# CIawevy/FreeFine

Hardware: AMD Instinct MI355X
Metric: edited images/sec/GPU @512px 50-step DDIM (higher is better)
Workload: dtype bf16x3

## Files before the change

freefine_amd/_lib.py:

```python
import ctypes as C
import os

_HERE = os.path.dirname(os.path.abspath(__file__))
LIB_PATH = os.environ.get("FREEFINE_HIP_LIB") or os.path.join(_HERE, "libfreefine_hip.so")

FFN_F32, FFN_BF16, FFN_BF16X3, FFN_FP8 = 0, 1, 2, 3
IG_OUT_SILU, IG_OUT_F32, IG_GEGLU, IG_OUT_TRANSPOSED, IG_OUT_PAIR, IG_OUT_GELU, IG_OUT_RELU, IG_OUT_KV64 = 1, 2, 4, 8, 16, 32, 64, 128
IG_OUT_QGELU = 256
ELT_RELU, ELT_ADD, ELT_GELU = 0, 1, 2
ATT_MAXP, ATT_MAXB = 4, 16
ATT_HEAD_RULE, ATT_UNIFORM_SEL1, ATT_UNIFORM_SEL0, ATT_CAUSAL = 1, 2, 4, 8
NORM_SILU, NORM_OUT_PAIR = 1, 2
IMGPREP_MAX_SIDE = 4096
IMGPREP_MAX_TAPS = 2 * 3 * IMGPREP_MAX_SIDE + 1
BOX_NMS_MAX = 16384
KEEP_NONE, KEEP_SUM_LT128, KEEP_GT128 = 0, 1, 2
CHAIN_MAXL, CHAIN_MAXW = 8, 1024
CONV_RELU = 1
POOL_MAX, POOL_AVG_VALID = 0, 1


class IgemmDesc(C.Structure):
    _fields_ = [
        ("A", C.c_void_p), ("W", C.c_void_p), ("out", C.c_void_p),
        ("bias", C.c_void_p), ("rowbias", C.c_void_p), ("residual", C.c_void_p),
        ("M", C.c_int), ("N", C.c_int), ("K", C.c_int), ("Kpad", C.c_int),
        ("lda", C.c_int), ("ldo", C.c_int), ("ldr", C.c_int), ("ldrb", C.c_int),
        ("rows_per_batch", C.c_int),
        ("Hin", C.c_int), ("Win", C.c_int), ("Cin", C.c_int), ("Hout", C.c_int), ("Wout", C.c_int),
        ("stride", C.c_int), ("pad", C.c_int), ("upsample", C.c_int),
        ("flags", C.c_int), ("alpha", C.c_float), ("conv", C.c_int),
        ("splitk", C.c_int), ("ws", C.c_void_p), ("ws_bytes", C.c_long),
        ("a_lo", C.c_int), ("x3", C.c_int), ("f8", C.c_int), ("kv64_from", C.c_int),
    ]


class AttnEntry(C.Structure):
    _fields_ = [
        ("q_row", C.c_int), ("kv_row", C.c_int),
        ("w_const", C.c_float), ("w_slope", C.c_float),
        ("wq", C.c_void_p), ("kmask", C.c_void_p), ("qsel", C.c_void_p),
        ("flags", C.c_int), ("hr_row", C.c_int),
    ]


class AttnDesc(C.Structure):
    _fields_ = [
        ("q", C.c_void_p), ("k", C.c_void_p), ("vt", C.c_void_p), ("out", C.c_void_p), ("w_dev", C.c_void_p),
        ("Bo", C.c_int), ("S", C.c_int), ("Sk", C.c_int), ("heads", C.c_int), ("D", C.c_int),
        ("ldq", C.c_int), ("ldk", C.c_int), ("ldvt", C.c_int), ("ldo", C.c_int),
        ("scale", C.c_float), ("npass", C.c_int), ("out_pair", C.c_int), ("kv_pair", C.c_int),
        ("e", AttnEntry * (ATT_MAXP * ATT_MAXB)),
    ]


class CtrlStepDesc(C.Structure):
    _fields_ = [
        ("eps", C.c_void_p), ("x", C.c_void_p), ("noise", C.c_void_p), ("m", C.c_void_p), ("om", C.c_void_p),
        ("x_prev", C.c_void_p), ("pred_x0", C.c_void_p),
        ("c_bt", C.c_float), ("c_at", C.c_float), ("c_ap", C.c_float), ("c_dir", C.c_float),
        ("c_dirm", C.c_float * 8), ("stdv", C.c_float * 8), ("row_masked", C.c_int * 8),
        ("rows", C.c_int), ("CHW", C.c_int), ("HW", C.c_int),
    ]


class SplatXform(C.Structure):
    _fields_ = [("center", C.c_float * 3), ("translate", C.c_float * 3), ("rotate", C.c_float * 9), ("scale", C.c_float * 3),
                ("tan_half_fov", C.c_float)]


class PackDesc(C.Structure):
    _fields_ = [
        ("src", C.c_void_p), ("dst", C.c_void_p), ("src_row", C.c_int * 16),
        ("B", C.c_int), ("Cl", C.c_int), ("CP", C.c_int), ("HW", C.c_int),
    ]


class DiftDesc(C.Structure):
    _fields_ = [
        ("src", C.c_void_p), ("tgt", C.c_void_p), ("kps", C.c_void_p), ("ws", C.c_void_p), ("out_rc", C.c_void_p), ("out_cos", C.c_void_p),
        ("ws_bytes", C.c_long), ("es", C.c_long),
        ("dtype", C.c_int), ("E", C.c_int), ("C", C.c_int), ("ld", C.c_int), ("h", C.c_int), ("w", C.c_int), ("H", C.c_int), ("W", C.c_int), ("K", C.c_int),
    ]


class ResizePilDesc(C.Structure):
    _fields_ = [
        ("src", C.c_void_p), ("dst", C.c_void_p), ("scratch", C.c_void_p), ("m1", C.c_void_p), ("m2", C.c_void_p),
        ("hbounds", C.c_void_p), ("hcoef", C.c_void_p), ("vbounds", C.c_void_p), ("vcoef", C.c_void_p),
        ("B", C.c_int), ("H", C.c_int), ("W", C.c_int), ("C", C.c_int), ("oh", C.c_int), ("ow", C.c_int), ("hksize", C.c_int), ("vksize", C.c_int),
        ("y0", C.c_int), ("x0", C.c_int), ("ch", C.c_int), ("cw", C.c_int), ("rule", C.c_int),
    ]


class CoarseEditDesc(C.Structure):
    _fields_ = [
        ("src_img", C.c_void_p), ("src_mask", C.c_void_p), ("bg", C.c_void_p), ("hole_img", C.c_void_p), ("hole_mask", C.c_void_p), ("inv", C.c_void_p),
        ("final_img", C.c_void_p), ("tmask", C.c_void_p), ("trans_hole", C.c_void_p),
        ("B", C.c_int), ("H", C.c_int), ("W", C.c_int), ("mask_c", C.c_int), ("hole_mask_c", C.c_int),
    ]


class Conv2dDesc(C.Structure):
    _fields_ = [
        ("x", C.c_void_p), ("w", C.c_void_p), ("bias", C.c_void_p), ("out", C.c_void_p),
        ("B", C.c_int), ("Hin", C.c_int), ("Win", C.c_int), ("Cin", C.c_int), ("N", C.c_int),
        ("KH", C.c_int), ("KW", C.c_int), ("stride", C.c_int), ("pad_h", C.c_int), ("pad_w", C.c_int),
        ("ldx", C.c_int), ("ldo", C.c_int), ("Kpad", C.c_int), ("flags", C.c_int),
    ]


_vp, _i, _f, _l = C.c_void_p, C.c_int, C.c_float, C.c_long
SYMBOLS = {
    "ffn_version": (_i, []),
    "ffn_last_error": (C.c_char_p, []),
    "ffn_device_info": (_i, [_i, C.c_char_p, _i]),
    "ffn_graph_launch": (_i, [_vp, _vp]),
    "ffn_igemm": (_i, [_vp, _i, C.POINTER(IgemmDesc)]),
    "ffn_conv3x3_n4": (_i, [_vp, _i, _vp, _vp, _vp, _vp, _i, _i, _i, _i]),
    "ffn_split_pair": (_i, [_vp, _vp, _vp, _l, _i, _i]),
    "ffn_groupnorm_f8": (_i, [_vp, _vp, _vp, _vp, _vp, _i, _i, _i, _i, _i, _f, _i, _f, _vp, _vp, _vp]),
    "ffn_attn": (_i, [_vp, _i, C.POINTER(AttnDesc)]),
    "ffn_attn_kernel_name": (_i, [_i, C.POINTER(AttnDesc), C.c_char_p, _i]),
    "ffn_igemm_tune": (_i, [_vp, _i, C.POINTER(IgemmDesc)]),
    "ffn_igemm_tune_entry_ints": (_i, []),
    "ffn_igemm_tune_export": (_i, [C.POINTER(C.c_int), _i]),
    "ffn_igemm_tune_import": (_i, [C.POINTER(C.c_int), _i]),
    "ffn_igemm_tune_stamp": (_i, []),
    "ffn_igemm_tune_clear": (_i, []),
    "ffn_igemm_tune_enable": (_i, [_i]),
    "ffn_igemm_num_configs": (_i, []),
    "ffn_igemm_force_config": (_i, [_i]),
    "ffn_igemm_kernel_name": (_i, [_i, C.POINTER(IgemmDesc), C.c_char_p, _i]),
    "ffn_attn_presplit": (_i, [_vp, _vp, _vp, _vp, _vp, _i, _i, _i, _i, _i]),
    "ffn_attn_variant": (_i, [_i, _i, C.POINTER(C.c_int), C.POINTER(C.c_int)]),
    "ffn_gn_nchunk": (_i, [_i]),
    "ffn_gn_fused": (_i, [_i, _i, _i, _i]),
    "ffn_gn_stats": (_i, [_vp, _i, _vp, _vp, _vp, _i, _i, _i, _i, _f, _vp, _vp, _vp]),
    "ffn_gn_apply": (_i, [_vp, _i, _vp, _vp, _vp, _vp, _i, _i, _i, _i]),
    "ffn_groupnorm": (_i, [_vp, _i, _vp, _vp, _vp, _vp, _i, _i, _i, _i, _f, _i, _vp, _vp, _vp]),
    "ffn_groupnorm_pair_raw": (_i, [_vp, _vp, _vp, _vp, _vp, _vp, _i, _i, _i, _i, _f, _i, _vp, _vp, _vp]),
    "ffn_layernorm": (_i, [_vp, _i, _vp, _vp, _vp, _vp, _i, _i, _f]),
    "ffn_layernorm_pair": (_i, [_vp, _vp, _vp, _vp, _vp, _i, _i, _f]),
    "ffn_softmax_rows": (_i, [_vp, _i, _vp, _vp, _l, _i, _f]),
    "ffn_pool_layernorm": (_i, [_vp, _i, _vp, _vp, _vp, _vp, _vp, _i, _i, _i, _f, _i]),
    "ffn_cosine_rows": (_i, [_vp, _vp, _vp, _vp, _i, _i, _i]),
    "ffn_cfg_masked": (_i, [_vp, _vp, _vp, _vp, _f, _vp, _l, _i]),
    "ffn_ddim_inv_step": (_i, [_vp, _vp, _vp, _f, _f, _f, _f, _vp, _vp, _l]),
    "ffn_ddim_ctrl_step": (_i, [_vp, C.POINTER(CtrlStepDesc)]),
    "ffn_pack_nchw": (_i, [_vp, _i, C.POINTER(PackDesc)]),
    "ffn_nhwc_to_nchw_f32": (_i, [_vp, _vp, _vp, _i, _i, _i, _i]),
    "ffn_concat": (_i, [_vp, _i, _vp, _vp, _vp, _l, _i, _i]),
    "ffn_timestep_embed": (_i, [_vp, _i, _vp, _vp, _vp, _i, _i, _i]),
    "ffn_transpose": (_i, [_vp, _i, _vp, _vp, _i, _i, _i, _i, _i]),
    "ffn_cast": (_i, [_vp, _i, _i, _vp, _vp, _l]),
    "ffn_eltwise": (_i, [_vp, _i, _i, _vp, _vp, _vp, _l]),
    "ffn_resize_bilinear": (_i, [_vp, _i, _vp, _vp, _i, _i, _i, _i, _i, _i, _i]),
    "ffn_splat_lift": (_i, [_vp, _vp, _vp, _vp, _i, _i, _i, _f, _f]),
    "ffn_splat_project": (_i, [_vp, _vp, _vp, _i, C.POINTER(SplatXform)]),
    "ffn_splat_bin": (_i, [_vp, _i, _vp, _i, _f, _i, _i, _vp, _vp, _vp]),
    "ffn_splat_render": (_i, [_vp, _vp, _vp, _vp, _vp, _f, _i, _i, _i, _vp, _vp, _vp]),
    "ffn_splat_ids": (_i, [_vp, _vp, _vp, _vp, _f, _i, _i, _i, _vp]),
    "ffn_splat_correspond": (_i, [_vp, _vp, _vp, _i, _i, _i, _vp, _i, _vp, _vp]),
    "ffn_geo_project": (_i, [_vp, _vp, C.POINTER(C.c_float), _f, _i, _i, _vp, _vp]),
    "ffn_splat_composite": (_i, [_vp, _vp, _vp, _vp, _vp, _f, _f, _i, _i, _i, _i, _i, _vp]),
    "ffn_mesh_cover": (_i, [_vp, _vp, _vp, _i, _i, _vp]),
    "ffn_embed_tokens": (_i, [_vp, _i, _vp, _vp, _vp, _vp, _l, _i, _i, _i]),
    "ffn_embed_tokens_ln": (_i, [_vp, _i, _vp, _vp, _vp, _vp, _vp, _vp, _l, _i, _i, _i, _f]),
    "ffn_affine_chain": (_i, [_vp, _vp, _vp, _vp, _i, _i, C.POINTER(C.c_int), _i, _f, _f]),
    "ffn_dift_match": (_i, [_vp, C.POINTER(DiftDesc)]),
    "ffn_dift_workspace_bytes": (_l, [_i, _i, _i, _i]),
    "ffn_sift_base": (_i, [_vp, _vp, _vp, _i, _i, _i]),
    "ffn_gauss_blur_f32": (_i, [_vp, _vp, _vp, _vp, _i, _i, _vp, _i]),
    "ffn_decimate2_f32": (_i, [_vp, _vp, _vp, _i, _i]),
    "ffn_sift_extrema": (_i, [_vp, _vp, _vp, _i, _i, _vp, _i, _vp, C.POINTER(C.c_int)]),
    "ffn_sift_refine_orient": (_i, [_vp, _vp, _vp, _i, _i, _i, _vp, _i, _vp]),
    "ffn_sift_describe": (_i, [_vp, _vp, _i, _i, _i, _vp, _i, _vp, _vp]),
    "ffn_knn2_u8": (_i, [_vp, _vp, _i, _vp, _i, _vp, _vp]),
    "ffn_resize_pil_bilinear_u8": (_i, [_vp, _vp, _vp, _vp, _i, _i, _i, _i, _i, _vp, _vp, _i, _vp, _vp, _i]),
    "ffn_resize_pil_u8": (_i, [_vp, C.POINTER(ResizePilDesc)]),
    "ffn_resize_taps8_u8": (_i, [_vp, _vp, _vp, _i, _i, _i, _i, _i, _i, _vp, _vp, _vp, _vp]),
    "ffn_resize_gather_u8": (_i, [_vp, _vp, _vp, _i, _i, _i, _i, _i, _i, _vp, _vp, _i]),
    "ffn_dilate_u8": (_i, [_vp, _vp, _vp, _vp, _i, _i, _i, _i, _i]),
    "ffn_mask_bbox_u8": (_i, [_vp, _vp, _vp, _i, _i, _i, _i]),
    "ffn_coarse_edit_2d": (_i, [_vp, C.POINTER(CoarseEditDesc)]),
    "ffn_vit_patch_rows": (_i, [_vp, _i, _vp, _vp, _vp, _i, _i, _i, _i, _i]),
    "ffn_vit_patch_rows_pair": (_i, [_vp, _vp, _vp, _vp, _i, _i, _i, _i, _i]),
    "ffn_sam_patch_rows": (_i, [_vp, _i, _vp, _vp, _i, _i, _i, _i, _i, _i, C.POINTER(C.c_float), C.POINTER(C.c_float)]),
    "ffn_sam_patch_rows_pair": (_i, [_vp, _vp, _vp, _i, _i, _i, _i, _i, _i, C.POINTER(C.c_float), C.POINTER(C.c_float)]),
    "ffn_hyper_masks": (_i, [_vp, _vp, _vp, _vp, _i, _i, _i, _i]),
    "ffn_upsample_bicubic": (_i, [_vp, _vp, _vp, _vp, _i, _i, _i, _i, _i]),
    "ffn_upsample_bicubic_stats": (_i, [_vp, _vp, _vp, _vp, _i, _i, _i, _i, _i, _f]),
    "ffn_box_nms": (_i, [_vp, _vp, _vp, _i, _f]),
    "ffn_image_to_nhwc": (_i, [_vp, _i, _vp, _vp, _l, _i]),
    "ffn_nhwc_to_image": (_i, [_vp, _i, _vp, _vp, _i, _i, _i]),
    "ffn_conv2d": (_i, [_vp, _i, C.POINTER(Conv2dDesc)]),
    "ffn_pool2d": (_i, [_vp, _i, _vp, _vp, _i, _i, _i, _i, _i, _i, _i, _i, _i]),
    "ffn_mean_hw": (_i, [_vp, _vp, _vp, _i, _i, _i, _i]),
    "ffn_fid_prep": (_i, [_vp, _vp, _vp, _vp, _i, _i, _i]),
}

_lib = None


class FreeFineHipError(RuntimeError):
    pass


def load():
    global _lib
    if _lib is None:
        if not os.path.exists(LIB_PATH):
            raise FreeFineHipError(
                f"{LIB_PATH} not found: build it with `python -c 'import __graft_entry__ as g; g.build()'` "
                "(hipcc --offload-arch=gfx950). There is no CPU fallback for the product path.")
        import torch
        lib = C.CDLL(LIB_PATH)
        for name, (res, args) in SYMBOLS.items():
            fn = getattr(lib, name)
            fn.restype = res
            fn.argtypes = args
        _lib = lib
    return _lib

# ... 6 lines not shown
```

freefine_amd/csrc/capi.hip:

```cpp
#include <stdlib.h>
#include <string.h>

#include "capi_common.h"
#include "conv_small.h"
#include "elementwise.h"
#include "norms.h"

__thread char g_err[512] = "";

extern "C" int ffn_version(void) { return 16; }
extern "C" const char* ffn_last_error(void) { return g_err; }
extern "C" int ffn_device_info(int device, char* name, int name_len) {
    hipDeviceProp_t prop;
    hipError_t e = hipGetDeviceProperties(&prop, device);
    if (e != hipSuccess) return fail(FFN_EHIP, "hipGetDeviceProperties: %s", hipGetErrorString(e));
    if (name && name_len > 0) {
        strncpy(name, prop.gcnArchName, name_len - 1);
        name[name_len - 1] = 0;
    }
    return prop.multiProcessorCount;
}

extern "C" int ffn_graph_launch(void* stream, void* graph_exec) {
    REQUIRE(graph_exec, "graph_launch: null graph");
    hipError_t e = hipGraphLaunch(reinterpret_cast<hipGraphExec_t>(graph_exec), reinterpret_cast<hipStream_t>(stream));
    if (e != hipSuccess) return fail(FFN_EHIP, "hipGraphLaunch: %s", hipGetErrorString(e));
    return FFN_OK;
}

extern "C" int ffn_split_pair(void* stream, const float* src, void* dst, long rows, int C, int ld_src) {
    REQUIRE(src && dst && rows > 0 && C > 0 && C % 4 == 0 && ld_src >= C && ld_src % 4 == 0, "split_pair: bad arguments (C=%d, ld_src=%d)", C, ld_src);
    REQUIRE(aligned16(src) && aligned16(dst), "split_pair: pointers must be 16-byte aligned");
    if (C % 8 == 0) LAUNCH(split_pair8_kernel, dim3(grid_for(rows * (C / 8))), dim3(256), 0, reinterpret_cast<hipStream_t>(stream), src, (bf16*)dst, rows, C, ld_src);
    else LAUNCH(split_pair_kernel, dim3(grid_for(rows * (C / 4))), dim3(256), 0, reinterpret_cast<hipStream_t>(stream), src, (bf16*)dst, rows, C, ld_src);
    return check_launch("split_pair");
}
extern "C" int ffn_conv3x3_n4(void* stream, int dtype, const void* x, const float* w, const float* bias, float* out, int B, int H, int W, int Cin) {
    REQUIRE(dtype == FFN_F32 || dtype == FFN_BF16, "conv3x3_n4: fp32 or bf16 activations");
    REQUIRE(x && w && out && aligned16(x) && aligned16(w) && aligned16(out) && (!bias || aligned16(bias)), "conv3x3_n4: null / unaligned pointer");
    REQUIRE(B > 0 && H > 0 && W > 0 && Cin > 0 && Cin % 16 == 0 && Cin <= 448, "conv3x3_n4: B=%d H=%d W=%d Cin=%d (Cin %% 16 == 0, <= 448)", B, H, W, Cin);
    hipStream_t s = reinterpret_cast<hipStream_t>(stream);
    const long npix = (long)B * H * W;
    const int lds = 36 * Cin * 4;
    dim3 grid((unsigned)((npix + 63) / 64));
    int rc;
    if (dtype == FFN_F32) {
        if ((rc = set_lds(conv3x3_n4_kernel<float>, lds))) return rc;
        LAUNCH(conv3x3_n4_kernel<float>, grid, dim3(256), lds, s, (const float*)x, w, bias, out, B, H, W, Cin);
    } else {
        if ((rc = set_lds(conv3x3_n4_kernel<bf16>, lds))) return rc;
        LAUNCH(conv3x3_n4_kernel<bf16>, grid, dim3(256), lds, s, (const bf16*)x, w, bias, out, B, H, W, Cin);
    }
    return check_launch("conv3x3_n4");
}

extern "C" int ffn_eltwise(void* stream, int dtype, int op, const void* a, const void* b, void* y, long n) {
    REQUIRE(dtype == FFN_F32 || dtype == FFN_BF16, "eltwise: bad dtype %d", dtype);
    REQUIRE(op == FFN_ELT_RELU || op == FFN_ELT_ADD || op == FFN_ELT_GELU, "eltwise: bad op %d", op);
    REQUIRE(a && y && (op != FFN_ELT_ADD || b), "eltwise: null operand");
    REQUIRE(n > 0 && n % 4 == 0, "eltwise: n=%ld must be a positive multiple of 4", n);
    hipStream_t s = reinterpret_cast<hipStream_t>(stream);
    const long n4 = n / 4;
    const int grid = grid_for(n4);
    if (dtype == FFN_F32) {
        if (op == FFN_ELT_RELU) LAUNCH((eltwise_kernel<float, FFN_ELT_RELU>), dim3(grid), dim3(256), 0, s, (const float*)a, (const float*)b, (float*)y, n4);
        else if (op == FFN_ELT_GELU) LAUNCH((eltwise_kernel<float, FFN_ELT_GELU>), dim3(grid), dim3(256), 0, s, (const float*)a, (const float*)b, (float*)y, n4);
        else LAUNCH((eltwise_kernel<float, FFN_ELT_ADD>), dim3(grid), dim3(256), 0, s, (const float*)a, (const float*)b, (float*)y, n4);
    } else {
        if (op == FFN_ELT_RELU) LAUNCH((eltwise_kernel<bf16, FFN_ELT_RELU>), dim3(grid), dim3(256), 0, s, (const bf16*)a, (const bf16*)b, (bf16*)y, n4);
        else if (op == FFN_ELT_GELU) LAUNCH((eltwise_kernel<bf16, FFN_ELT_GELU>), dim3(grid), dim3(256), 0, s, (const bf16*)a, (const bf16*)b, (bf16*)y, n4);
        else LAUNCH((eltwise_kernel<bf16, FFN_ELT_ADD>), dim3(grid), dim3(256), 0, s, (const bf16*)a, (const bf16*)b, (bf16*)y, n4);
    }
    return check_launch("eltwise");
}
extern "C" int ffn_resize_bilinear(void* stream, int dtype, const void* x, void* y, int B, int Hin, int Win, int Hout, int Wout, int C, int relu) {
    REQUIRE(dtype == FFN_F32 || dtype == FFN_BF16, "resize_bilinear: bad dtype %d", dtype);
    REQUIRE(x && y, "resize_bilinear: null operand");
    REQUIRE(B > 0 && Hin > 0 && Win > 0 && Hout > 0 && Wout > 0 && C > 0 && C % 4 == 0, "resize_bilinear: bad shape (C=%d must be a multiple of 4)", C);
    REQUIRE((long)B * Hout * Wout * C < (1l << 40) && (long)Hin * Win < (1l << 31), "resize_bilinear: problem too large");
    hipStream_t s = reinterpret_cast<hipStream_t>(stream);
    const long n4 = (long)B * Hout * Wout * (C / 4);
    const int grid = grid_for(n4);
    if (dtype == FFN_F32) {
        if (relu) LAUNCH((resize_bilinear_kernel<float, true>), dim3(grid), dim3(256), 0, s, (const float*)x, (float*)y, n4, Hin, Win, Hout, Wout, C);
        else LAUNCH((resize_bilinear_kernel<float, false>), dim3(grid), dim3(256), 0, s, (const float*)x, (float*)y, n4, Hin, Win, Hout, Wout, C);
    } else {
        if (relu) LAUNCH((resize_bilinear_kernel<bf16, true>), dim3(grid), dim3(256), 0, s, (const bf16*)x, (bf16*)y, n4, Hin, Win, Hout, Wout, C);
        else LAUNCH((resize_bilinear_kernel<bf16, false>), dim3(grid), dim3(256), 0, s, (const bf16*)x, (bf16*)y, n4, Hin, Win, Hout, Wout, C);
    }
    return check_launch("resize_bilinear");
}

extern "C" int ffn_gn_nchunk(int HW) {
    int n = HW / 128;
    if (n < 1) n = 1;
    if (n > 256) n = 256;
    return n;
}
extern "C" int ffn_gn_fused(int B, int HW, int C, int G) {
    const long slice = (long)HW * (C / (G > 0 ? G : 1));
    if (slice > 131072) return 0;
    if (HW <= 64) return 1;
    if (HW <= 256) return B <= 32 ? 1 : 0;
    return (HW <= 1024 && (long)B * HW * C <= 3000000l) ? 1 : 0;
}
extern "C" int ffn_groupnorm(void* stream, int dtype, const void* x, void* y, const float* gamma, const float* beta, int B, int HW, int C,
                             int G, float eps, int silu, float* partial_ws, float* scale, float* shift) {
    REQUIRE(dtype == FFN_F32 || dtype == FFN_BF16, "groupnorm: bad dtype");
    REQUIRE(x && y && gamma && beta && C % G == 0 && (C / G) % 2 == 0, "groupnorm: bad arguments (C=%d, G=%d)", C, G);
    hipStream_t s = reinterpret_cast<hipStream_t>(stream);
    const bool fused = ffn_gn_fused(B, HW, C, G) != 0;
    const bool pair = silu & FFN_NORM_OUT_PAIR;
    REQUIRE(!pair || (dtype == FFN_F32 && C % 4 == 0), "groupnorm: pair output needs fp32 input and C %% 4 == 0");
    silu &= FFN_NORM_SILU;
    if (fused && pair) {
        dim3 grid(G, B);
        if (silu) LAUNCH((gn_fused_kernel<float, true, true>), grid, dim3(1024), 0, s, (const float*)x, (float*)y, gamma, beta, HW, C, G, eps);
        else LAUNCH((gn_fused_kernel<float, false, true>), grid, dim3(1024), 0, s, (const float*)x, (float*)y, gamma, beta, HW, C, G, eps);
        return check_launch("gn_fused(pair)");
    }
    if (fused) {
        dim3 grid(G, B);
        if (dtype == FFN_F32) {
            if (silu) LAUNCH((gn_fused_kernel<float, true>), grid, dim3(1024), 0, s, (const float*)x, (float*)y, gamma, beta, HW, C, G, eps);
            else LAUNCH((gn_fused_kernel<float, false>), grid, dim3(1024), 0, s, (const float*)x, (float*)y, gamma, beta, HW, C, G, eps);
        } else {
            if (silu) LAUNCH((gn_fused_kernel<bf16, true>), grid, dim3(1024), 0, s, (const bf16*)x, (bf16*)y, gamma, beta, HW, C, G, eps);
            else LAUNCH((gn_fused_kernel<bf16, false>), grid, dim3(1024), 0, s, (const bf16*)x, (bf16*)y, gamma, beta, HW, C, G, eps);
        }
        return check_launch("gn_fused");
    }
    REQUIRE(partial_ws && scale && shift, "groupnorm: workspace required beyond 32x32 positions");
    int rc = ffn_gn_stats(stream, dtype, x, gamma, beta, B, HW, C, G, eps, partial_ws, scale, shift);
    if (rc) return rc;
    return ffn_gn_apply(stream, dtype, x, y, scale, shift, B, HW, C, silu | (pair ? FFN_NORM_OUT_PAIR : 0));
}
extern "C" int ffn_groupnorm_pair_raw(void* stream, const void* x, void* y, void* yraw, const float* gamma, const float* beta, int B, int HW, int C, int G,
                                      float eps, int silu, float* partial_ws, float* scale, float* shift) {
    REQUIRE(x && y && yraw && gamma && beta && partial_ws && scale && shift, "groupnorm_pair_raw: null pointer (the workspace is always needed)");
    REQUIRE(C % 8 == 0 && C % G == 0 && (C / G) % 2 == 0 && aligned16(x) && aligned16(y) && aligned16(yraw), "groupnorm_pair_raw: bad arguments (C=%d, G=%d)", C, G);
    REQUIRE(y != yraw && yraw != x && y != x, "groupnorm_pair_raw: x, y and yraw must be distinct buffers");
    int rc = ffn_gn_stats(stream, FFN_F32, x, gamma, beta, B, HW, C, G, eps, partial_ws, scale, shift);
    if (rc) return rc;
    hipStream_t s = reinterpret_cast<hipStream_t>(stream);
    const long n8 = (long)B * HW * (C / 8);
    if (silu & FFN_NORM_SILU) LAUNCH((gn_apply_pair8_kernel<true, true>), dim3(grid_for(n8)), dim3(256), 0, s, (const float*)x, (bf16*)y, scale, shift, n8, HW, C, (bf16*)yraw);
    else LAUNCH((gn_apply_pair8_kernel<false, true>), dim3(grid_for(n8)), dim3(256), 0, s, (const float*)x, (bf16*)y, scale, shift, n8, HW, C, (bf16*)yraw);
    return check_launch("gn_apply(pair + raw pair)");
}
extern "C" int ffn_groupnorm_f8(void* stream, const void* x, void* y, const float* gamma, const float* beta, int B, int HW, int C, int Cp, int G,
                                float eps, int silu, float qscale, float* partial_ws, float* scale, float* shift) {
    REQUIRE(x && y && gamma && beta && partial_ws && scale && shift, "groupnorm_f8: null pointer (the workspace is always needed)");
    REQUIRE(C % 16 == 0 && C % G == 0 && Cp >= C && Cp % 16 == 0 && aligned16(x) && aligned16(y) && qscale > 0.f, "groupnorm_f8: bad arguments (C=%d, Cp=%d)", C, Cp);
    int rc = ffn_gn_stats(stream, FFN_BF16, x, gamma, beta, B, HW, C, G, eps, partial_ws, scale, shift);
    if (rc) return rc;
    hipStream_t s = reinterpret_cast<hipStream_t>(stream);
    const long nch = (long)B * HW * (Cp / 16);
    if (silu & FFN_NORM_SILU) LAUNCH(gn_apply_f8_kernel<true>, dim3(grid_for(nch)), dim3(256), 0, s, (const bf16*)x, (uint8_t*)y, scale, shift, nch, HW, C, Cp, qscale);
    else LAUNCH(gn_apply_f8_kernel<false>, dim3(grid_for(nch)), dim3(256), 0, s, (const bf16*)x, (uint8_t*)y, scale, shift, nch, HW, C, Cp, qscale);
    return check_launch("gn_apply_f8");
}
extern "C" int ffn_gn_stats(void* stream, int dtype, const void* x, const float* gamma, const float* beta, int B, int HW, int C,
                            int G, float eps, float* partial_ws, float* scale, float* shift) {
    REQUIRE(dtype == FFN_F32 || dtype == FFN_BF16, "gn_stats: bad dtype");
    const int epc = dtype == FFN_F32 ? 4 : 8;
    REQUIRE(x && gamma && beta && partial_ws && scale && shift, "gn_stats: null pointer");
    REQUIRE(C % epc == 0 && C % G == 0 && aligned16(x), "gn_stats: C=%d must be a multiple of %d and of G=%d", C, epc, G);
    hipStream_t s = reinterpret_cast<hipStream_t>(stream);
    const int nchunk = ffn_gn_nchunk(HW);
    const int ppc = (HW + nchunk - 1) / nchunk;
    const int cols_ = C / epc < 256 ? C / epc : 256;
    const int lds = (256 / cols_ > 0 ? 256 / cols_ : 1) * cols_ * 2 * epc * (int)sizeof(float);
    if (dtype == FFN_F32)
        LAUNCH(gn_partial_kernel<float>, dim3(nchunk, B), dim3(256), lds, s, (const float*)x, partial_ws, HW, C, ppc);
    else
        LAUNCH(gn_partial_kernel<bf16>, dim3(nchunk, B), dim3(256), lds, s, (const bf16*)x, partial_ws, HW, C, ppc);
    if (int rc = check_launch("gn_partial")) return rc;
    LAUNCH(gn_finalize_kernel, dim3(G, B), dim3(64), 0, s, partial_ws, gamma, beta, scale, shift, HW, C, G, nchunk, ppc, eps);
    return check_launch("gn_stats");
}
extern "C" int ffn_gn_apply(void* stream, int dtype, const void* x, void* y, const float* scale, const float* shift, int B, int HW,
                            int C, int silu) {
    REQUIRE(dtype == FFN_F32 || dtype == FFN_BF16, "gn_apply: bad dtype");
    const int epc = dtype == FFN_F32 ? 4 : 8;
    REQUIRE(x && y && scale && shift && C % epc == 0 && aligned16(x) && aligned16(y), "gn_apply: bad arguments");
    hipStream_t s = reinterpret_cast<hipStream_t>(stream);
    const long nch = (long)B * HW * (C / epc);
    const int grid = grid_for(nch);
    if (silu & FFN_NORM_OUT_PAIR) {
        REQUIRE(dtype == FFN_F32, "gn_apply: pair output needs fp32 input");
        if (C % 8 == 0) {
            const long n8 = (long)B * HW * (C / 8);
            if (silu & FFN_NORM_SILU) LAUNCH(gn_apply_pair8_kernel<true>, dim3(grid_for(n8)), dim3(256), 0, s, (const float*)x, (bf16*)y, scale, shift, n8, HW, C);
            else LAUNCH(gn_apply_pair8_kernel<false>, dim3(grid_for(n8)), dim3(256), 0, s, (const float*)x, (bf16*)y, scale, shift, n8, HW, C);
            return check_launch("gn_apply(pair, 8 wide)");
        }
        if (silu & FFN_NORM_SILU) LAUNCH((gn_apply_kernel<float, true, true>), dim3(grid), dim3(256), 0, s, (const float*)x, (float*)y, scale, shift, nch, HW, C);
        else LAUNCH((gn_apply_kernel<float, false, true>), dim3(grid), dim3(256), 0, s, (const float*)x, (float*)y, scale, shift, nch, HW, C);
        return check_launch("gn_apply(pair)");
    }
    if (dtype == FFN_F32) {
        if (silu) LAUNCH((gn_apply_kernel<float, true>), dim3(grid), dim3(256), 0, s, (const float*)x, (float*)y, scale, shift, nch, HW, C);
        else LAUNCH((gn_apply_kernel<float, false>), dim3(grid), dim3(256), 0, s, (const float*)x, (float*)y, scale, shift, nch, HW, C);
    } else {
        if (silu) LAUNCH((gn_apply_kernel<bf16, true>), dim3(grid), dim3(256), 0, s, (const bf16*)x, (bf16*)y, scale, shift, nch, HW, C);
        else LAUNCH((gn_apply_kernel<bf16, false>), dim3(grid), dim3(256), 0, s, (const bf16*)x, (bf16*)y, scale, shift, nch, HW, C);
    }
    return check_launch("gn_apply");
}
extern "C" int ffn_layernorm(void* stream, int dtype, const void* x, void* y, const float* gamma, const float* beta, int M, int C,
                             float eps) {
    REQUIRE(dtype == FFN_F32 || dtype == FFN_BF16, "layernorm: bad dtype");
    const int epc = dtype == FFN_F32 ? 4 : 8;
    REQUIRE(x && y && gamma && beta && C % epc == 0 && aligned16(x) && aligned16(y), "layernorm: bad arguments");
    const int cch = C / epc;
    REQUIRE(cch <= 64 * 6, "layernorm: C=%d too large", C);
    hipStream_t s = reinterpret_cast<hipStream_t>(stream);
    const int grid = (M + 3) / 4;
    if (dtype == FFN_F32) {
        if (cch <= 128) LAUNCH((layernorm_kernel<float, 2>), dim3(grid), dim3(256), 0, s, (const float*)x, (float*)y, gamma, beta, M, C, eps);
        else LAUNCH((layernorm_kernel<float, 6>), dim3(grid), dim3(256), 0, s, (const float*)x, (float*)y, gamma, beta, M, C, eps);
    } else {
        if (cch <= 128) LAUNCH((layernorm_kernel<bf16, 2>), dim3(grid), dim3(256), 0, s, (const bf16*)x, (bf16*)y, gamma, beta, M, C, eps);
        else LAUNCH((layernorm_kernel<bf16, 6>), dim3(grid), dim3(256), 0, s, (const bf16*)x, (bf16*)y, gamma, beta, M, C, eps);
    }
    return check_launch("layernorm");
}
extern "C" int ffn_layernorm_pair(void* stream, const float* x, void* y, const float* gamma, const float* beta, int M, int C, float eps) {
    REQUIRE(x && y && gamma && beta && C % 4 == 0 && aligned16(x) && aligned16(y), "layernorm_pair: bad arguments");
    const int cch = C / 4;
    REQUIRE(cch <= 64 * 6, "layernorm_pair: C=%d too large", C);
    hipStream_t s = reinterpret_cast<hipStream_t>(stream);
    const int grid = (M + 3) / 4;
    if (cch <= 128) LAUNCH((layernorm_kernel<float, 2, true>), dim3(grid), dim3(256), 0, s, x, (float*)y, gamma, beta, M, C, eps);
    else LAUNCH((layernorm_kernel<float, 6, true>), dim3(grid), dim3(256), 0, s, x, (float*)y, gamma, beta, M, C, eps);
    return check_launch("layernorm(pair)");
}
extern "C" int ffn_softmax_rows(void* stream, int dtype, const void* x, void* y, long M, int N, float scale) {
    REQUIRE(dtype == FFN_F32 || dtype == FFN_BF16, "softmax_rows: bad dtype");
    REQUIRE(x && y && M > 0 && N > 0, "softmax_rows: bad arguments");
    hipStream_t s = reinterpret_cast<hipStream_t>(stream);
    if (dtype == FFN_F32) LAUNCH(softmax_rows_kernel<float>, dim3((unsigned)M), dim3(256), 0, s, (const float*)x, (float*)y, N, scale);
    else LAUNCH(softmax_rows_kernel<bf16>, dim3((unsigned)M), dim3(256), 0, s, (const bf16*)x, (bf16*)y, N, scale);
    return check_launch("softmax_rows");
}

extern "C" int ffn_cfg_masked(void* stream, const float* eps_u, const float* eps_c, const float* mask, float cfg, float* eps, long n,
                              int HW) {
    REQUIRE(eps_u && eps_c && eps && n > 0 && HW > 0, "cfg_masked: bad arguments");
    LAUNCH(cfg_masked_kernel, dim3(grid_for(n)), dim3(256), 0, reinterpret_cast<hipStream_t>(stream), eps_u, eps_c, mask, cfg, eps, n, HW);
    return check_launch("cfg_masked");
}
extern "C" int ffn_ddim_inv_step(void* stream, const float* eps, const float* x, float c_bt, float c_at, float c_an, float c_bn,
                                 float* x_next, float* pred_x0, long n) {
    REQUIRE(eps && x && x_next && n > 0, "ddim_inv_step: bad arguments");
    LAUNCH(ddim_inv_step_kernel, dim3(grid_for(n)), dim3(256), 0, reinterpret_cast<hipStream_t>(stream), eps, x, c_bt, c_at, c_an, c_bn, x_next, pred_x0, n);
    return check_launch("ddim_inv_step");
}
extern "C" int ffn_ddim_ctrl_step(void* stream, const ffn_ctrl_step_desc* d) {
    REQUIRE(d && d->eps && d->x && d->x_prev && d->m && d->om, "ddim_ctrl_step: null pointer");
    REQUIRE(d->rows > 0 && d->rows <= 8 && d->CHW > 0 && d->HW > 0 && d->CHW % d->HW == 0, "ddim_ctrl_step: bad shape");
    LAUNCH(ddim_ctrl_step_kernel, dim3(grid_for((long)d->rows * d->CHW)), dim3(256), 0, reinterpret_cast<hipStream_t>(stream), *d);
// ... 75 lines not shown
```

freefine_amd/csrc/capi_igemm.hip:

```cpp
#include <math.h>
#include <stdlib.h>
#include <string.h>
#include <initializer_list>

#include "capi_common.h"
#include "igemm.h"
#include "igemm_p8.h"

static bool can_split(const ffn_igemm_desc& d) {
    return d.ws && d.splitk != 1 && !(d.flags & (FFN_IG_GEGLU | FFN_IG_OUT_TRANSPOSED | FFN_IG_OUT_KV64));
}
static void igemm_rule_for(int dtype, const ffn_igemm_desc& d, int* bm, int* bn, int* splitk) {
    const long t128 = (long)((d.M + 127) / 128) * ((d.N + 127) / 128);
    const long t12864 = (long)((d.M + 127) / 128) * ((d.N + 63) / 64);
    *splitk = 1;
    if (!d.conv && !(d.flags & FFN_IG_GEGLU) && d.M >= 128 && (!can_split(d) || t12864 >= 128)) {
        *bm = 128; *bn = 64;
    } else if (d.N > 64 && (t128 >= 256 || (can_split(d) && d.M > 512 && d.N >= 128))) {
        *bm = 128; *bn = 128;
    } else if (t12864 >= 256 || d.M >= 4096 || (can_split(d) && d.M >= 96 && d.N >= 64)) {
        *bm = 128; *bn = 64;
    } else { *bm = 64; *bn = 64; }
    if (can_split(d)) {
        const int kstage = dtype == FFN_F32 ? 32 : 64;
        const int nk = (d.K + kstage - 1) / kstage;
        const long tiles = (long)((d.M + *bm - 1) / *bm) * ((d.N + *bn - 1) / *bn);
        int s = d.splitk > 1 ? d.splitk : (tiles >= 224 ? 1 : (int)((448 + tiles - 1) / tiles));
        if (d.splitk <= 1 && s > nk / 6) s = nk / 6;
        const long per = (long)d.M * d.N * 4;
        if ((long)s * per > d.ws_bytes) s = (int)(d.ws_bytes / per);
        if (s > nk) s = nk;
        if (s < 1) s = 1;
        *splitk = s;
    }
}

enum { CFG_64x64, CFG_128x64, CFG_128x128_8, CFG_128x128_16, CFG_256x128, CFG_256x256, CFG_128x320, CFG_128x160, CFG_192x320, CFG_H_128x320, CFG_H_256x128, CFG_H_256x256, CFG_H_128x128, CFG_PP_256x320, CFG_PP_256x256, CFG_PP_192x320, CFG_PP_192x256, CFG_PP_256x128, CFG_COUNT };
struct IgCfgInfo { int bm, bn, nwm, nwn; };
static const IgCfgInfo kCfg[CFG_COUNT] = {{64, 64, 2, 2}, {128, 64, 4, 2}, {128, 128, 2, 4}, {128, 128, 4, 4},
                                          {256, 128, 4, 4}, {256, 256, 4, 4}, {128, 320, 4, 4}, {128, 160, 4, 2}, {192, 320, 3, 4},
                                          {128, 320, 4, 4}, {256, 128, 4, 4}, {256, 256, 4, 4}, {128, 128, 4, 4},
                                          {256, 320, 2, 4}, {256, 256, 2, 4}, {192, 320, 2, 4}, {192, 256, 2, 4},
                                          {256, 128, 2, 4}};
struct IgChoice { int cfg, splitk; };
struct TunedEntry { IgChoice ch; bool validated; };

static bool is_halo_cfg(int cfg) { return cfg == CFG_H_128x320 || cfg == CFG_H_256x128 || cfg == CFG_H_256x256 || cfg == CFG_H_128x128; }
static bool is_pp_cfg(int cfg) { return cfg >= CFG_PP_256x320 && cfg <= CFG_PP_256x128; }
static bool pp_ok(const ffn_igemm_desc& d, int bm, int bn, int splitk = 1) {
    const long lim = (1l << 31) - 4096;
    const int nkt = d.x3 ? d.K / 96 : d.K / 64;
    if (bn == 128 && (bm != 256 || !d.x3 || d.conv != 1 || splitk > 1 || d.N % 256 == 0 || d.N % 320 == 0 || (d.flags & (FFN_IG_GEGLU | FFN_IG_OUT_PAIR | FFN_IG_OUT_KV64 | FFN_IG_OUT_TRANSPOSED)))) return false;
    if (d.x3) {
        if (d.x3 != 2 || d.K % 96 != 0 || d.a_lo != 32) return false;
    } else if (d.K % 64 != 0) return false;
    if (nkt < 2 || d.N % bn != 0 || d.M < bm) return false;
    const int osz = d.x3 ? 4 : 2;
    if (splitk > 1) {
        if (!can_split(d) || nkt % splitk != 0 || nkt / splitk < 2 || (long)splitk * d.M * d.N * 4 > d.ws_bytes || (long)splitk * d.M * d.N * 4 >= lim) return false;
    } else {
        const int act_ok = (!d.residual && !d.x3 && !d.f8 && !(d.flags & FFN_IG_GEGLU)) ? (FFN_IG_OUT_GELU | FFN_IG_OUT_RELU) : 0;
        if ((d.alpha != 1.0f && !d.f8) || (d.flags & ~(FFN_IG_GEGLU | act_ok | (d.x3 ? (FFN_IG_OUT_F32 | FFN_IG_OUT_PAIR | FFN_IG_OUT_KV64) : 0)))) return false;
        if (d.f8 && (!d.conv || (d.flags & FFN_IG_GEGLU))) return false;
        if (d.x3 && (d.flags & FFN_IG_GEGLU) && !(d.flags & FFN_IG_OUT_PAIR)) return false;
        if ((d.flags & FFN_IG_OUT_PAIR) && !(d.flags & FFN_IG_GEGLU) && (d.N % 32 != 0 || (d.ldo / 2) % 32 != 0 || (d.flags & FFN_IG_OUT_TRANSPOSED))) return false;
        if ((d.flags & FFN_IG_GEGLU) && bn != 256) return false;
        if (d.rowbias && d.rows_per_batch < 128) return false;
    }
    long a_bytes;
    if (d.conv) {
        const int pix = d.x3 ? d.lda : d.Cin;
        const int cpt = d.x3 ? d.Cin / 32 : d.Cin / 64;
        if (d.Cin % (d.x3 ? 32 : 64) != 0 || d.K != (d.conv == 2 ? 4 : 9) * (d.x3 ? 3 : 1) * d.Cin) return false;
        if (d.x3 && d.lda != 2 * d.Cin) return false;
        if (d.conv == 2 && (d.f8 || d.stride != 1 || d.upsample)) return false;
        if ((long)cpt * 9 * cpt >= 65536) return false;
        a_bytes = (long)(d.M / (d.Hout * d.Wout)) * d.Hin * d.Win * pix * 2;
        if (2 * d.Hin + 2 >= 32768 || 2 * d.Win + 2 >= 32768) return false;
        if (a_bytes + 256l * pix * 2 >= lim) return false;
    } else {
        a_bytes = (long)d.M * d.lda * 2;
        if (a_bytes + 256l * d.lda * 2 >= lim) return false;
    }
    if ((long)d.N * d.Kpad * 2 >= lim || (long)(d.M + 256) * d.ldo * ((d.flags & FFN_IG_OUT_PAIR) ? 2 : osz) >= lim) return false;
    if (d.residual && (long)(d.M + 256) * d.ldr * osz >= lim) return false;
    return true;
}
static int halo_bytes_for(const ffn_igemm_desc& d, int bm) {
    if (!d.conv || d.stride != 1 || d.upsample || d.pad != 1 || d.Hin != d.Hout || d.Win != d.Wout) return 0;
    if (d.Cin % 64 != 0 || d.Cin > 30000 || d.K != 9 * d.Cin || d.M % bm != 0) return 0;
    const int H = d.Hin, W = d.Win;
    int tw, tr;
    if (W <= bm) {
        if (bm % W != 0 || (H * W) % bm != 0) return 0;
        tw = W; tr = bm / W;
    } else {
        if (W % bm != 0) return 0;
        tw = bm; tr = 1;
    }
    const int nq = ((tr + 2) * (tw + 2) + 7) / 8;
    if (nq > 4 * 16) return 0;
    return nq * 8 * 128;
}
static bool x3_cfg(int cfg) { return cfg == CFG_64x64 || cfg == CFG_128x64 || cfg == CFG_128x128_8 || is_pp_cfg(cfg); }
static ffn_igemm_desc x3_view(const ffn_igemm_desc& d) {
    ffn_igemm_desc v = d;
    v.x3 = d.x3 == 2 ? 2 : 1;
    v.f8 = 0;
    v.K = 3 * d.K;
    v.flags |= FFN_IG_OUT_F32;
    return v;
}
static ffn_igemm_desc f8_view(const ffn_igemm_desc& d) {
    ffn_igemm_desc v = d;
    v.f8 = 1;
    v.x3 = 0;
    v.K = d.K / 2;
    v.Cin = d.Cin / 2;
    v.Kpad = d.Kpad / 2;
    v.lda = d.lda / 2;
    return v;
}
static ffn_igemm_desc igemm_view(int dtype, const ffn_igemm_desc& d) {
    if (dtype == FFN_BF16X3) return x3_view(d);
    if (dtype == FFN_FP8) return f8_view(d);
    ffn_igemm_desc v = d;
    v.x3 = v.f8 = 0;
    return v;
}
static int pp_tile_height(const ffn_igemm_desc& d, int bn, std::initializer_list<int> heights, int min_fill4, bool trans = false) {
    long best = -1;
    int bh = 0;
    for (int h : heights) {
        if (trans ? d.M < h : !pp_ok(d, h, bn)) continue;
        const long tiles = (long)((d.M + h - 1) / h) * (d.N / bn);
        if (tiles * 4 < (long)device_cus() * min_fill4) continue;
        const long cost = ((tiles + device_cus() - 1) / device_cus()) * h;
        if (best < 0 || cost < best) { best = cost; bh = h; }
    }
    return bh;
}
static int pp_cfg(int bm, int bn) {
    for (int cfg = CFG_PP_256x320; cfg <= CFG_PP_256x128; ++cfg)
        if (kCfg[cfg].bm == bm && kCfg[cfg].bn == bn) return cfg;
    return -1;
}
static bool conv2_tile(const ffn_igemm_desc& d, int* bm, int* bn) {
    for (int n : {320, 256})
        for (int h : {256, 192})
            if (pp_tile_height(d, n, {h}, 0)) { *bm = h; *bn = n; return true; }
    return false;
}
static bool pp_trans_tile(const ffn_igemm_desc& d, int* bm, int* bn) {
    const long lim = (1l << 31) - 4096;
    *bn = d.N % 320 == 0 ? 320 : (d.N % 256 == 0 ? 256 : 0);
    if (!*bn || d.alpha != 1.0f || d.rows_per_batch % 16 != 0 || d.M % 4 != 0) return false;
    if (d.x3) {
        if (d.x3 != 2 || d.K % 96 != 0 || d.K < 192 || d.a_lo != 32) return false;
    } else if (d.K % 64 != 0 || d.K < 128) return false;
    if ((long)(d.M + 256) * d.lda * 2 >= lim || (long)d.N * d.Kpad * 2 >= lim) return false;
    if ((long)((d.M + d.rows_per_batch - 1) / d.rows_per_batch) * d.N * d.ldo * (d.x3 ? 4 : 2) >= lim) return false;
    return (*bm = pp_tile_height(d, *bn, {256, 192}, 0, true)) != 0;
}
static IgChoice rule_choice(int dtype, const ffn_igemm_desc& d) {
    int bm, bn, sk;
    igemm_rule_for(dtype, d, &bm, &bn, &sk);
    const int kstage = dtype == FFN_F32 ? 32 : 64;
    const int nk = ((d.K + kstage - 1) / kstage + sk - 1) / sk;
    int cfg = CFG_64x64;
    if (bm == 128 && bn == 64) cfg = CFG_128x64;
    if (bm == 128 && bn == 128) cfg = (!d.conv && nk <= 24 && !d.x3 && !d.f8) ? CFG_128x128_16 : CFG_128x128_8;
    return IgChoice{cfg, sk};
}
static IgChoice heuristic_choice(const ffn_igemm_desc& d) {
    int bm, bn;
    if (d.conv == 2 && conv2_tile(d, &bm, &bn)) return IgChoice{pp_cfg(bm, bn), 1};
    if (d.splitk <= 1) {
        for (int n : {320, 256})
            if ((bm = pp_tile_height(d, n, {256, 192}, 3))) return IgChoice{pp_cfg(bm, n), 1};
        if (pp_tile_height(d, 128, {256}, 3)) return IgChoice{CFG_PP_256x128, 1};
    }
    return rule_choice(FFN_BF16, d);
}

struct TuneKey {
    int M, N, K, conv, Cin, Hin, Win, stride, upsample, flags, lda, splitk, ptrs, wslabs, rpb, alpha1, ldo, pad, Hout, Wout, Kpad, ldr, dtype;
    bool operator==(const TuneKey& o) const { return memcmp(this, &o, sizeof(TuneKey)) == 0; }
};
struct TuneKeyHash {
    size_t operator()(const TuneKey& k) const {
        const int* p = reinterpret_cast<const int*>(&k);
        size_t h = 1469598103934665603ull;
        for (size_t i = 0; i < sizeof(TuneKey) / sizeof(int); ++i) h = (h ^ (size_t)(unsigned)p[i]) * 1099511628211ull;
        return h;
    }
};
static TuneKey tune_key(const ffn_igemm_desc& d) {
    TuneKey k;
    memset(&k, 0, sizeof(k));
    k.M = d.M; k.N = d.N; k.K = d.K; k.conv = d.conv; k.flags = d.flags; k.lda = d.lda; k.splitk = d.splitk;
    if (d.conv) { k.Cin = d.Cin; k.Hin = d.Hin; k.Win = d.Win; k.stride = d.stride; k.upsample = d.upsample; k.pad = d.pad; k.Hout = d.Hout; k.Wout = d.Wout; }
    k.Kpad = d.Kpad;
    k.ldr = d.residual ? d.ldr : 0;
    k.dtype = d.x3 ? (FFN_BF16X3 | (d.x3 << 8)) : (d.f8 ? FFN_FP8 : FFN_BF16);
    k.ptrs = (d.bias ? 1 : 0) | (d.rowbias ? 2 : 0) | (d.residual ? 4 : 0) | (d.ws && d.ws_bytes > 0 ? 8 : 0);
    const long per = (long)d.M * d.N * 4;
    k.wslabs = d.ws ? (int)(d.ws_bytes / per > 1024 ? 1024 : d.ws_bytes / per) : 0;
    k.rpb = d.rows_per_batch;
    k.alpha1 = d.alpha == 1.0f;
    k.ldo = d.ldo;
    return k;
}
static std::mutex g_tune_mu;
static std::unordered_map<TuneKey, TunedEntry, TuneKeyHash> g_tuned;
static int g_tune_runtime = 1;
static bool tune_enabled() {
    static const bool on = [] { const char* e = getenv("FFN_IGEMM_TUNE"); return !(e && atoi(e) == 0); }();
    return on && g_tune_runtime;
}
static constexpr int kPpSplitBelow = 160;
static int candidates_for(const ffn_igemm_desc& d, IgChoice* out, int cap) {
    int n = 0;
    const IgChoice h = heuristic_choice(d);
    out[n++] = h;
    const int nk = (d.K + 63) / 64;
    const long per = (long)d.M * d.N * 4;
    for (int cfg = 0; cfg < CFG_COUNT; ++cfg) {
        const IgCfgInfo& c = kCfg[cfg];
        if ((d.x3 || d.f8) && !x3_cfg(cfg)) continue;
        if (d.conv == 2 && !is_pp_cfg(cfg)) continue;
        if ((cfg == CFG_128x320 || cfg == CFG_128x160 || cfg == CFG_192x320) && (d.flags & FFN_IG_GEGLU)) continue;
        if (is_halo_cfg(cfg)) {
            const int hb = halo_bytes_for(d, c.bm);
            if (hb <= 0 || d.splitk > 1 || 2 * hb + 2 * c.bn * 128 > 160 * 1024) continue;
            if ((cfg == CFG_H_128x320) && (d.flags & FFN_IG_GEGLU)) continue;
        }
        const bool halo = is_halo_cfg(cfg) || is_pp_cfg(cfg);
        if (is_pp_cfg(cfg)) {
            const long pt = (long)((d.M + c.bm - 1) / c.bm) * (d.N / (c.bn > 0 ? c.bn : 1));
            if (d.splitk <= 1 && pp_ok(d, c.bm, c.bn) && n < cap) out[n++] = IgChoice{cfg, 1};
            if (cfg != CFG_PP_256x128 && d.splitk != 1 && pt > 0 && pt < kPpSplitBelow && d.N % c.bn == 0) {
                const int nkt = d.x3 ? d.K / 96 : d.K / 64;
                int added = 0;
                for (int sgo = (int)((384 + pt - 1) / pt); sgo >= 2 && added < 2; --sgo) {
                    if (d.splitk > 1 && sgo != d.splitk) continue;
                    if (nkt % sgo != 0 || nkt / sgo < 2 || !pp_ok(d, c.bm, c.bn, sgo)) continue;
                    if (n < cap) out[n++] = IgChoice{cfg, sgo};
                    ++added;
                }
            }
            continue;
        }
        if (c.bm > 64 && c.bm >= 2 * d.M) continue;
        if (c.bn > 64 && c.bn >= 2 * d.N) continue;
        if (cfg == CFG_64x64 && (long)d.M * d.N > (1l << 22)) continue;
        const long tiles = (long)((d.M + c.bm - 1) / c.bm) * ((d.N + c.bn - 1) / c.bn);
        int splits[3] = {1, 0, 0};
        if (d.splitk > 1) {
            int sf = (can_split(d) && !halo) ? d.splitk : 1;
            if ((long)sf * per > d.ws_bytes) sf = (int)(d.ws_bytes / per);
            if (sf > nk) sf = nk;
            splits[0] = sf >= 2 ? sf : 1;
        } else if (can_split(d) && !halo) {
            for (int t = 0; t < 2; ++t) {
                int sgo = (int)(((t ? 512 : 256) + tiles / 2) / tiles);
                if (sgo > nk / 4) sgo = nk / 4;
                if ((long)sgo * per > d.ws_bytes) sgo = (int)(d.ws_bytes / per);
                if (sgo >= 2) splits[1 + t] = sgo;
            }
            if (splits[2] == splits[1]) splits[2] = 0;
        }
        for (int t = 0; t < 3 && n < cap; ++t) {
            if (!splits[t]) continue;
            bool dup = false;
            for (int j = 0; j < n; ++j) dup |= out[j].cfg == cfg && out[j].splitk == splits[t];
            if (!dup) out[n++] = IgChoice{cfg, splits[t]};
        }
    }
    return n;
}
static int g_force_cfg = -1;
extern "C" int ffn_igemm_num_configs(void) { return CFG_COUNT; }
extern "C" int ffn_igemm_force_config(int cfg) {
    const int prev = g_force_cfg;
    g_force_cfg = (cfg >= 0 && cfg < CFG_COUNT) ? cfg : -1;
    return prev;
}
static bool known_choice(const ffn_igemm_desc& d, IgChoice* ch) {
    IgChoice cand[40];
    if (g_force_cfg >= 0) {
        *ch = heuristic_choice(d);
        for (int i = candidates_for(d, cand, 40) - 1; i >= 0; --i)
            if (cand[i].cfg == g_force_cfg) *ch = cand[i];
        return true;
    }
    std::lock_guard<std::mutex> lk(g_tune_mu);
    auto it = g_tuned.find(tune_key(d));
    if (it == g_tuned.end()) return false;
    if (!it->second.validated) {
        const int nc = candidates_for(d, cand, 40);
        bool ok = false;
        for (int i = 0; i < nc; ++i) ok |= cand[i].cfg == it->second.ch.cfg && cand[i].splitk == it->second.ch.splitk;
        if (!ok) return g_tuned.erase(it), false;
        it->second.validated = true;
    }
    *ch = it->second.ch;
    return true;
}

enum IgKind { IG_RING, IG_HALO, IG_PP, IG_PP_TRANS };
struct IgemmPlan {
    IgKind kind;
    bool f32;
    int bm, bn, amode, nwm, nwn;
    bool swap, fastk, x3, f8;
    bool res, geglu, split;
    int splitk, halo_bytes, lds;
    bool reduce_f32;
    dim3 grid, block;
};
static int igemm_plan(int dtype, const ffn_igemm_desc& d, const IgChoice* ch, IgemmPlan* p) {
    *p = IgemmPlan{};
    p->f32 = dtype == FFN_F32;
    p->x3 = d.x3 != 0;
    p->f8 = d.f8 != 0;
    p->amode = d.conv ? AMODE_CONV3 : AMODE_DENSE;
    p->swap = !(d.flags & FFN_IG_OUT_TRANSPOSED);
    p->reduce_f32 = p->f32 || p->x3;
    p->splitk = 1;
    p->block = dim3(512);
    const bool tuned = ch != nullptr;
    IgChoice rule;
    if (!tuned && !p->f32 && pp_trans_tile(d, &p->bm, &p->bn)) {
        p->kind = IG_PP_TRANS;
    } else {
        if (!tuned) ch = &(rule = rule_choice(p->f32 ? FFN_F32 : FFN_BF16, d));
        REQUIRE(ch->cfg >= 0 && ch->cfg < CFG_COUNT, "igemm: bad configuration %d", ch->cfg);
        REQUIRE(!(p->x3 || p->f8) || x3_cfg(ch->cfg), "igemm: configuration %d is not built for split-bf16 / fp8 problems", ch->cfg);
        const IgCfgInfo& c = kCfg[ch->cfg];
        p->kind = is_halo_cfg(ch->cfg) ? IG_HALO : (is_pp_cfg(ch->cfg) ? IG_PP : IG_RING);
        p->bm = c.bm; p->bn = c.bn; p->nwm = c.nwm; p->nwn = c.nwn;
        p->splitk = ch->splitk;
        p->block = dim3(64 * c.nwm * c.nwn);
        if (!tuned && p->x3) p->nwm = p->nwn = 2, p->block = dim3(256);
    }
    const int ntm = (d.M + p->bm - 1) / p->bm, ntn = (d.N + p->bn - 1) / p->bn;
    switch (p->kind) {
    case IG_RING: {
        p->fastk = tuned && !p->x3 && !p->f8 && (d.conv ? d.Cin % 64 == 0 : d.K % 64 == 0) && (long)d.K * 2 + 256 <= (long)sizeof(g_zero_page);
        p->lds = 2 * (p->bm + p->bn) * 128;
        int gx = ntm * ntn;
        if (tuned || p->x3) {
            int per_cu = (160 * 1024) / p->lds;
            if (per_cu > 2048 / (int)p->block.x) per_cu = 2048 / (int)p->block.x;
            const int cap = (device_cus() * per_cu) / p->splitk;
            if (gx > cap && cap >= 8) gx = cap;
        }
        p->grid = dim3(gx, p->splitk);
        break;
    }
    case IG_HALO:
        p->halo_bytes = halo_bytes_for(d, p->bm);
        REQUIRE(p->halo_bytes > 0 && p->splitk == 1 && !p->x3 && !p->f8, "igemm: halo kernel not applicable");
        p->lds = 2 * p->halo_bytes + 2 * p->bn * 128;
        p->grid = dim3((d.M / p->bm) * ntn);
        break;
    case IG_PP:
        REQUIRE(pp_ok(d, p->bm, p->bn, p->splitk), "igemm: ping-pong kernel not applicable");
        p->split = p->splitk > 1;
        p->res = !p->split && d.residual;
        p->geglu = !p->split && !d.conv && (d.flags & FFN_IG_GEGLU);
        [[fallthrough]];
    case IG_PP_TRANS: {
        p->lds = 2 * (p->bm + p->bn) * 128 + 12288;
        const int nt = ntm * (d.N / p->bn) * p->splitk;
        p->grid = dim3(nt < device_cus() ? nt : device_cus());
        break;
    }
    }
    return FFN_OK;
}
template <typename K, typename... A>
static int igemm_launch(const IgemmPlan& p, K kern, hipStream_t s, A... args) {
    static const char* const what[] = {"igemm", "igemm(halo)", "igemm(ping-pong)", "igemm(ping-pong, transposed)"};
    if (int rc = set_lds(kern, p.lds)) return rc;
    LAUNCH(kern, p.grid, p.block, p.lds, s, args...);
    return check_launch(what[p.kind]);
}
template <typename T, int AMODE, bool SWAP, bool FASTK = false, bool X3 = false, bool F8 = false>
static int launch_ring(const IgemmPlan& p, hipStream_t s, const ffn_igemm_desc& d) {
#define FFN_RING(BM_, BN_, WM_, WN_) \
    if (p.bm == BM_ && p.bn == BN_ && p.nwm == WM_ && p.nwn == WN_) return igemm_launch(p, igemm_glds_kernel<T, BM_, BN_, AMODE, SWAP, 2, WM_, WN_, FASTK, X3, F8>, s, d)
    if constexpr (X3 && !SWAP) {
        FFN_RING(64, 64, 2, 2);
        FFN_RING(128, 64, 2, 2);
        FFN_RING(128, 128, 2, 2);
    } else {
        FFN_RING(64, 64, 2, 2);
        FFN_RING(128, 64, 4, 2);
        FFN_RING(128, 128, 2, 4);
        if constexpr (!X3 && !F8) FFN_RING(128, 128, 4, 4);
        if constexpr (sizeof(T) == 2 && SWAP && !X3 && !F8) {
            FFN_RING(256, 128, 4, 4);
            FFN_RING(256, 256, 4, 4);
            FFN_RING(128, 320, 4, 4);
            FFN_RING(128, 160, 4, 2);
            FFN_RING(192, 320, 3, 4);
        }
    }
#undef FFN_RING
    return fail(FFN_EINVAL, "igemm: no %d x %d tile on %d x %d waves for this problem", p.bm, p.bn, p.nwm, p.nwn);
}
template <int AMODE, bool X3 = false, bool F8 = false>
static int launch_pp(const IgemmPlan& p, hipStream_t s, const ffn_igemm_desc& d) {
    const bool trans = p.kind == IG_PP_TRANS;
#define FFN_PP(BM_, BN_, RES_, GEGLU_, SPLIT_, TRANS_)                                                                       \
    if (p.bm == BM_ && p.bn == BN_ && p.res == RES_ && p.geglu == GEGLU_ && p.split == SPLIT_ && trans == TRANS_) \
        return igemm_launch(p, igemm_pp_kernel<BM_, BN_, AMODE, RES_, GEGLU_, SPLIT_, TRANS_, X3, F8>, s, d, p.splitk)
#define FFN_PP_TILE(BM_, BN_)                                                                   \
    FFN_PP(BM_, BN_, false, false, false, false);                                               \
    FFN_PP(BM_, BN_, true, false, false, false);                                                \
    FFN_PP(BM_, BN_, false, false, true, false);                                                \
    if constexpr (AMODE == AMODE_DENSE && !F8) {                                                \
        FFN_PP(BM_, BN_, false, false, false, true);                                            \
        if constexpr (BN_ == 256) FFN_PP(BM_, BN_, false, true, false, false);                  \
    }
    FFN_PP_TILE(256, 320)
    FFN_PP_TILE(256, 256)
    FFN_PP_TILE(192, 320)
    FFN_PP_TILE(192, 256)
    if constexpr (X3 && AMODE == AMODE_CONV3) {
        FFN_PP(256, 128, false, false, false, false);
        FFN_PP(256, 128, true, false, false, false);
    }
#undef FFN_PP_TILE
#undef FFN_PP
    return fail(FFN_EINVAL, "igemm: no %d x %d ping-pong tile of this form", p.bm, p.bn);
}
static int igemm_run(hipStream_t s, int dtype, const ffn_igemm_desc& d, const IgChoice* ch) {
    IgemmPlan p;
    int rc = igemm_plan(dtype, d, ch, &p);
    if (rc) return rc;
    const bool conv = p.amode == AMODE_CONV3;
    switch (p.kind) {
    case IG_RING:
        if (p.f32) rc = conv ? launch_ring<float, AMODE_CONV3, true>(p, s, d) : (p.swap ? launch_ring<float, AMODE_DENSE, true>(p, s, d) : launch_ring<float, AMODE_DENSE, false>(p, s, d));
        else if (!p.swap) rc = p.x3 ? launch_ring<bf16, AMODE_DENSE, false, false, true>(p, s, d) : launch_ring<bf16, AMODE_DENSE, false>(p, s, d);
        else if (p.x3) rc = conv ? launch_ring<bf16, AMODE_CONV3, true, false, true>(p, s, d) : launch_ring<bf16, AMODE_DENSE, true, false, true>(p, s, d);
        else if (p.f8) rc = launch_ring<bf16, AMODE_CONV3, true, false, false, true>(p, s, d);
        else if (p.fastk) rc = conv ? launch_ring<bf16, AMODE_CONV3, true, true>(p, s, d) : launch_ring<bf16, AMODE_DENSE, true, true>(p, s, d);
        else rc = conv ? launch_ring<bf16, AMODE_CONV3, true>(p, s, d) : launch_ring<bf16, AMODE_DENSE, true>(p, s, d);
        break;
    case IG_HALO:
#define FFN_HALO(BM_, BN_) \
    if (p.bm == BM_ && p.bn == BN_) rc = igemm_launch(p, igemm_halo_kernel<bf16, BM_, BN_, 4, 4>, s, d, p.halo_bytes)
        FFN_HALO(128, 320);
        FFN_HALO(256, 128);
        FFN_HALO(256, 256);
        FFN_HALO(128, 128);
#undef FFN_HALO
        break;
    case IG_PP:
    case IG_PP_TRANS:
        if (p.x3) rc = conv ? launch_pp<AMODE_CONV3, true>(p, s, d) : launch_pp<AMODE_DENSE, true>(p, s, d);
        else if (p.f8) rc = launch_pp<AMODE_CONV3, false, true>(p, s, d);
        else rc = conv ? launch_pp<AMODE_CONV3>(p, s, d) : launch_pp<AMODE_DENSE>(p, s, d);
        break;
    }
    if (rc || p.splitk == 1) return rc;
    const dim3 grid(grid_for((long)d.M * (d.N / 4)));
    if (p.reduce_f32) LAUNCH(igemm_splitk_reduce_kernel<float>, grid, dim3(256), 0, s, d, p.splitk);
    else LAUNCH(igemm_splitk_reduce_kernel<bf16>, grid, dim3(256), 0, s, d, p.splitk);
    return check_launch("igemm_splitk_reduce");
}
static int igemm_tune_now(hipStream_t s, int dtype, const ffn_igemm_desc& d) {
    std::lock_guard<std::mutex> lk(g_tune_mu);
    IgChoice cand[40];
    const int nc = candidates_for(d, cand, 40);
    hipEvent_t e0, e1;
    if (hipEventCreate(&e0) != hipSuccess || hipEventCreate(&e1) != hipSuccess) return igemm_run(s, dtype, d, &cand[0]);
    IgChoice best = cand[0];
    float best_ms = 1e30f;
    const int reps = 3;
    for (int i = 0; i < nc; ++i) {
        int rc = igemm_run(s, dtype, d, &cand[i]);
        if (rc) continue;
        float ms = 1e30f;
        for (int round = 0; round < 2 && !rc; ++round) {
            (void)hipEventRecord(e0, s);
            for (int r = 0; r < reps && !rc; ++r) rc = igemm_run(s, dtype, d, &cand[i]);
            (void)hipEventRecord(e1, s);
            if (rc || hipEventSynchronize(e1) != hipSuccess) { rc = rc ? rc : FFN_EHIP; break; }
            float t = 0.f;
            (void)hipEventElapsedTime(&t, e0, e1);
            if (t < ms) ms = t;
        }
        if (rc) continue;
        if (ms < best_ms) { best_ms = ms; best = cand[i]; }
// ... 30 lines not shown
        if (buf && n < max_entries) {
            int* e = buf + (long)n * kTuneEntryInts;
            e[0] = kTuneStamp;
            memcpy(e + 1, &kv.first, sizeof(TuneKey));
            e[kTuneEntryInts - 2] = kv.second.ch.cfg;
            e[kTuneEntryInts - 1] = kv.second.ch.splitk;
        }
        ++n;
    }
    return n;
}
extern "C" int ffn_igemm_tune_import(const int* buf, int n_entries) {
    REQUIRE(buf || n_entries == 0, "igemm_tune_import: null buffer");
    std::lock_guard<std::mutex> lk(g_tune_mu);
    int n = 0;
    for (int i = 0; i < n_entries; ++i) {
        const int* e = buf + (long)i * kTuneEntryInts;
        if (e[0] != kTuneStamp) continue;
        TuneKey k;
        memcpy(&k, e + 1, sizeof(TuneKey));
        const IgChoice ch{e[kTuneEntryInts - 2], e[kTuneEntryInts - 1]};
        if (ch.cfg < 0 || ch.cfg >= CFG_COUNT || ch.splitk < 1) continue;
        g_tuned[k] = TunedEntry{ch, false};
        ++n;
    }
    return n;
}
static int igemm_validate(int dtype, const ffn_igemm_desc& d) {
    REQUIRE(dtype == FFN_F32 || dtype == FFN_BF16 || dtype == FFN_BF16X3 || dtype == FFN_FP8, "igemm: bad dtype %d", dtype);
    if (dtype == FFN_FP8) {
        REQUIRE(d.conv && d.Cin > 0 && d.Cin % 16 == 0 && d.K == 9 * d.Cin && d.Kpad >= d.K && d.Kpad % 16 == 0 && d.lda == d.Cin,
                "igemm(fp8): 3x3 convolutions with Cin %% 16 == 0 only (Cin=%d, K=%d, Kpad=%d, lda=%d)", d.Cin, d.K, d.Kpad, d.lda);
        REQUIRE(d.M > 0 && d.N > 0 && d.N % 4 == 0 && d.ldo % 4 == 0 && d.rows_per_batch > 0 && d.M % (d.Hout * d.Wout) == 0, "igemm(fp8): bad shape");
        REQUIRE(!(d.flags & (FFN_IG_GEGLU | FFN_IG_OUT_TRANSPOSED | FFN_IG_OUT_PAIR | FFN_IG_OUT_F32)), "igemm(fp8): plain / SiLU / residual epilogues only");
        REQUIRE(d.stride == 1 || d.stride == 2, "igemm(fp8): stride %d", d.stride);
        int ex = 0;
        REQUIRE(d.alpha > 0.f && frexpf(d.alpha, &ex) == 0.5f, "igemm(fp8): alpha must be a power of two (the un-scaling of two power-of-two operand scales)");
        if (d.residual) REQUIRE(d.ldr % 4 == 0 && d.ldr >= d.N, "igemm(fp8): ldr=%d must be a multiple of 4 and >= N=%d", d.ldr, d.N);
        REQUIRE(d.ldo >= d.N, "igemm(fp8): ldo=%d must be >= N=%d", d.ldo, d.N);
        return FFN_OK;
    }
    const int epc = dtype == FFN_F32 ? 4 : 8;
    const int kmul = dtype == FFN_BF16X3 ? (d.x3 == 2 ? 2 : 3) : 1;
    REQUIRE(d.M > 0 && d.N > 0 && d.K > 0, "igemm: empty problem M=%d N=%d K=%d", d.M, d.N, d.K);
    REQUIRE(d.Kpad >= kmul * d.K && d.Kpad % epc == 0, "igemm: Kpad=%d (row stride of W) must be >= %d x K=%d and a multiple of %d", d.Kpad, kmul, d.K, epc);
    if (dtype == FFN_BF16X3) {
        const int plane = d.conv ? d.Cin : d.K;
        if (d.x3 == 2) {
            REQUIRE(plane % 32 == 0 && d.a_lo == 32 && d.lda >= 2 * plane, "igemm: blocked split-bf16 operands need K (conv: Cin) %% 32 == 0, a_lo = 32, lda >= 2 x that (%d, a_lo=%d, lda=%d)", plane, d.a_lo, d.lda);
        } else {
            REQUIRE(d.a_lo % 8 == 0 && d.a_lo >= plane && d.a_lo + plane <= d.lda, "igemm: split-bf16 A needs planes of %d elements: a_lo=%d, lda=%d", plane, d.a_lo, d.lda);
        }
        REQUIRE(d.lda % 8 == 0, "igemm: lda=%d must be a multiple of 8", d.lda);
        REQUIRE(d.alpha == 1.0f, "igemm: split-bf16 problems take alpha = 1");
    }
    REQUIRE(d.K % epc == 0, "igemm: K=%d must be a multiple of %d", d.K, epc);
    REQUIRE(d.rows_per_batch > 0, "igemm: rows_per_batch must be > 0");
    if (d.conv) {
        REQUIRE(d.Cin % epc == 0, "igemm: Cin=%d must be a multiple of %d", d.Cin, epc);
        if (d.conv == 2) {
            REQUIRE((dtype == FFN_BF16 || dtype == FFN_BF16X3) && d.K == 4 * d.Cin && d.stride == 1 && d.upsample == 0 && d.pad >= 0 && d.pad <= 3 && d.splitk <= 1,
                    "igemm: 2x2 convolution needs FFN_BF16 / FFN_BF16X3, K = 4*Cin, stride 1, no upsample, pad in 0..3, no forced split");
            int bm, bn;
            REQUIRE(conv2_tile(igemm_view(dtype, d), &bm, &bn), "igemm: 2x2 convolution M=%d N=%d Cin=%d fits no ping-pong tile (Cin %% 64 (split-bf16: 32), N %% 256 / 320, M >= 192)", d.M, d.N, d.Cin);
        } else {
            REQUIRE(d.conv == 1, "igemm: conv=%d", d.conv);
            REQUIRE(d.K == 9 * d.Cin, "igemm: conv K=%d != 9*Cin=%d", d.K, 9 * d.Cin);
        }
        REQUIRE(d.stride == 1 || d.stride == 2, "igemm: stride %d", d.stride);
        REQUIRE(d.upsample == 0 || d.upsample == 1, "igemm: upsample %d", d.upsample);
        REQUIRE(d.M % (d.Hout * d.Wout) == 0, "igemm: M=%d not a multiple of Hout*Wout", d.M);
    } else {
        REQUIRE(d.lda % epc == 0, "igemm: lda=%d must be a multiple of %d", d.lda, epc);
    }
    if (d.flags & FFN_IG_OUT_KV64) {
        REQUIRE(dtype == FFN_BF16X3 && !d.conv && !d.residual && !d.rowbias && d.splitk <= 1 &&
                    !(d.flags & (FFN_IG_GEGLU | FFN_IG_OUT_PAIR | FFN_IG_OUT_SILU | FFN_IG_OUT_GELU | FFN_IG_OUT_RELU | FFN_IG_OUT_QGELU)),
                "igemm: FFN_IG_OUT_KV64 needs FFN_BF16X3, dense A, the plain epilogue and no forced split-K");
        if (d.flags & FFN_IG_OUT_TRANSPOSED) REQUIRE(d.rows_per_batch % 64 == 0 && d.M % d.rows_per_batch == 0 && d.ldo >= d.rows_per_batch && d.ldo % 64 == 0,
                                                     "igemm: KV64 transposed output needs rows_per_batch %% 64 == 0, whole batches, ldo %% 64 == 0 (rows_per_batch=%d, ldo=%d)", d.rows_per_batch, d.ldo);
        else REQUIRE(d.kv64_from >= 0 && d.kv64_from < d.N && d.kv64_from % 64 == 0 && d.N % 64 == 0 && d.ldo % 4 == 0,
                     "igemm: KV64 output needs kv64_from and N %% 64 == 0 (kv64_from=%d, N=%d)", d.kv64_from, d.N);
    }
    if (d.flags & FFN_IG_OUT_TRANSPOSED) {
        REQUIRE(!d.conv, "igemm: transposed output is only supported for dense A");
        REQUIRE(d.ldo % 4 == 0, "igemm: transposed ldo=%d must be a multiple of 4", d.ldo);
        REQUIRE(!(d.flags & (FFN_IG_GEGLU | FFN_IG_OUT_F32 | FFN_IG_OUT_SILU | FFN_IG_OUT_GELU | FFN_IG_OUT_RELU | FFN_IG_OUT_QGELU)) && !d.residual && !d.rowbias,
                "igemm: transposed output supports bias only");
    } else {
        REQUIRE(d.N % 4 == 0 && d.ldo % 4 == 0, "igemm: N=%d and ldo=%d must be multiples of 4", d.N, d.ldo);
        if (d.residual) REQUIRE(d.ldr % 4 == 0, "igemm: ldr=%d must be a multiple of 4", d.ldr);
        if (d.flags & FFN_IG_OUT_PAIR) {
            const int nout = (d.flags & FFN_IG_GEGLU) ? d.N / 2 : d.N;
            REQUIRE(dtype == FFN_BF16X3 && d.ldo % 16 == 0 && d.ldo / 2 >= nout, "igemm: pair output needs FFN_BF16X3, ldo %% 16 == 0, ldo/2 >= columns");
            REQUIRE(d.residual != d.out, "igemm: pair output cannot overwrite its fp32 residual");
            REQUIRE((d.ldo / 2) % 32 != 0 || nout % 32 == 0 || nout == d.ldo / 2, "igemm: blocked pair output (ldo/2 %% 32 == 0) needs whole 32-column blocks");
            REQUIRE(nout == d.ldo / 2 || (d.ldo / 2) % 32 == 0, "igemm: pair output into a wider row needs ldo/2 %% 32 == 0 (ldo=%d, columns=%d)", d.ldo, nout);
        }
        if (d.flags & FFN_IG_GEGLU) {
            REQUIRE(d.N % 64 == 0, "igemm: GEGLU needs N %% 64 == 0 (N=%d)", d.N);
            REQUIRE(!d.residual && !d.rowbias && !(d.flags & (FFN_IG_OUT_F32 | FFN_IG_OUT_SILU | FFN_IG_OUT_GELU | FFN_IG_OUT_RELU | FFN_IG_OUT_QGELU)), "igemm: GEGLU epilogue is exclusive");
        }
    }
    const int act = d.flags & (FFN_IG_OUT_SILU | FFN_IG_OUT_GELU | FFN_IG_OUT_RELU | FFN_IG_OUT_QGELU);
    REQUIRE((act & (act - 1)) == 0, "igemm: SILU / GELU / QGELU / RELU are mutually exclusive");
    REQUIRE(d.splitk >= 0, "igemm: splitk must be >= 0");
    if (!d.conv && dtype != FFN_BF16X3) REQUIRE(d.lda >= d.K, "igemm: lda=%d must be >= K=%d", d.lda, d.K);
    if (d.flags & FFN_IG_OUT_TRANSPOSED) {
        const int cols = d.rows_per_batch < d.M ? d.rows_per_batch : d.M;
        REQUIRE(d.ldo >= cols, "igemm: transposed ldo=%d must be >= the %d rows of a batch", d.ldo, cols);
    } else if (!(d.flags & FFN_IG_OUT_PAIR)) {
        const int nout = (d.flags & FFN_IG_GEGLU) ? d.N / 2 : d.N;
        REQUIRE(d.ldo >= nout, "igemm: ldo=%d must be >= the %d output columns", d.ldo, nout);
    }
    if (d.residual) REQUIRE(d.ldr >= d.N, "igemm: ldr=%d must be >= N=%d", d.ldr, d.N);
    return FFN_OK;
}
static bool tuned_family(int dtype, const ffn_igemm_desc& d) { return dtype != FFN_F32 && !(d.flags & FFN_IG_OUT_TRANSPOSED); }
extern "C" int ffn_igemm_kernel_name(int dtype, const ffn_igemm_desc* d0, char* buf, int len) {
    REQUIRE(d0 && buf && len > 0, "igemm_kernel_name: null argument");
    if (int rc = igemm_validate(dtype, *d0)) return rc;
    const ffn_igemm_desc d = igemm_view(dtype, *d0);
    const bool tuned = tuned_family(dtype, d);
    IgChoice ch;
    if (tuned && !known_choice(d, &ch)) ch = heuristic_choice(d);
    IgemmPlan p;
    if (int rc = igemm_plan(dtype, d, tuned ? &ch : nullptr, &p)) return rc;
    auto b = [](bool v) { return v ? "true" : "false"; };
    switch (p.kind) {
    case IG_RING:
        snprintf(buf, len, "void igemm_glds_kernel<%s, %d, %d, %d, %s, 2, %d, %d, %s, %s, %s>(ffn_igemm_desc)", p.f32 ? "float" : "bf16", p.bm, p.bn, p.amode,
                 b(p.swap), p.nwm, p.nwn, b(p.fastk), b(p.x3), b(p.f8));
        break;
    case IG_HALO: snprintf(buf, len, "void igemm_halo_kernel<bf16, %d, %d, %d, %d>(ffn_igemm_desc, int)", p.bm, p.bn, p.nwm, p.nwn); break;
    case IG_PP:
    case IG_PP_TRANS:
        snprintf(buf, len, "void igemm_pp_kernel<%d, %d, %d, %s, %s, %s, %s, %s, %s>(ffn_igemm_desc, int)", p.bm, p.bn, p.amode, b(p.res), b(p.geglu), b(p.split),
                 b(p.kind == IG_PP_TRANS), b(p.x3), b(p.f8));
        break;
    }
    return FFN_OK;
}
extern "C" int ffn_igemm(void* stream, int dtype, const ffn_igemm_desc* d0) {
    REQUIRE(d0, "igemm: null descriptor");
    if (int rc = igemm_validate(dtype, *d0)) return rc;
    if (dtype == FFN_FP8) {
        REQUIRE(d0->A && d0->W && d0->out && aligned16(d0->A) && aligned16(d0->W) && aligned16(d0->out), "igemm(fp8): A/W/out must be non-null and 16-byte aligned");
    } else {
        REQUIRE(d0->A && d0->W && d0->out, "igemm: null A/W/out");
        REQUIRE(aligned16(d0->A) && aligned16(d0->W) && aligned16(d0->out), "igemm: A/W/out must be 16-byte aligned");
    }
    if ((dtype == FFN_BF16X3 || dtype == FFN_F32) && d0->residual) REQUIRE(aligned16(d0->residual), "igemm: fp32 residual must be 16-byte aligned");
    if ((dtype == FFN_BF16 || dtype == FFN_FP8) && d0->residual)
        REQUIRE((reinterpret_cast<uintptr_t>(d0->residual) & 7) == 0, "igemm%s: bf16 residual must be 8-byte aligned", dtype == FFN_FP8 ? "(fp8)" : "");
    if (d0->ws) REQUIRE(aligned16(d0->ws) && d0->ws_bytes >= 0, "igemm%s: workspace must be 16-byte aligned", dtype == FFN_FP8 ? "(fp8)" : "");
    hipStream_t s = reinterpret_cast<hipStream_t>(stream);
    const ffn_igemm_desc d = igemm_view(dtype, *d0);
    if (!tuned_family(dtype, d)) return igemm_run(s, dtype, d, nullptr);
    IgChoice ch;
    if (!known_choice(d, &ch)) {
        hipStreamCaptureStatus cap = hipStreamCaptureStatusNone;
        (void)hipStreamIsCapturing(s, &cap);
        if (tune_enabled() && cap == hipStreamCaptureStatusNone && d.residual != d.out) return igemm_tune_now(s, dtype, d);
        ch = heuristic_choice(d);
    }
    return igemm_run(s, dtype, d, &ch);
}

extern "C" int ffn_igemm_tune(void* stream, int dtype, const ffn_igemm_desc* d) { return ffn_igemm(stream, dtype, d); }
```

freefine_amd/csrc/igemm_p8.h:

```cpp
#pragma once
#include <type_traits>
#include "igemm.h"

#ifndef PP_ABL
#define PP_ABL 0
#endif
#ifdef PP_STAMP
__device__ unsigned long long pp_stamp_out[8 * 64];
#define PP_STAMP_AT(k_) do { if (blockIdx.x == 7 && s >= 24 && s < 28) { const unsigned long long t_ = __builtin_amdgcn_s_memtime(); \
    if (lane == 0) *reinterpret_cast<unsigned long long*>(smem + CV + 12288 + (wave * 64 + (s - 24) * 16 + (k_)) * 8) = t_; } } while (0)
#else
#define PP_STAMP_AT(k_) do {} while (0)
#endif
#define X3_NBE(FN_, NA_) ((FN_) + 2 - ((FN_) + (NA_) + 1) / 2)
template <int N>
__device__ __forceinline__ void pp_wait_vmcnt() {
    if (PP_ABL != 2) asm volatile("s_waitcnt vmcnt(%0)" ::"n"(N) : "memory");
}
__device__ __forceinline__ void pp_barrier() {
    asm volatile("" ::: "memory");
    __builtin_amdgcn_s_barrier();
    asm volatile("" ::: "memory");
}

#ifdef PP_TRACE
__device__ unsigned long long pp_trace[256 * 64];
#endif
template <int BM, int BN, int AMODE, bool RES, bool GEGLU, bool SPLIT = false, bool TRANS = false, bool X3 = false, bool F8 = false>
__global__ __launch_bounds__(512) void igemm_pp_kernel(const IgemmParams p, int splitk = 1) {
    typedef bf16 T;
    constexpr int HM = BM / 2;
    constexpr int FM = HM / 16;
    constexpr int FH = FM / 2;
    constexpr int NA = BM / 64;
    constexpr int FN = BN / 64;
    constexpr int WN = BN / 4;
    constexpr int ABYTES = BM * 128, BBYTES = BN * 128, BUF = ABYTES + BBYTES;
    constexpr int CV = 2 * BUF;
    constexpr int NB1 = (FN + 1) / 2;
    constexpr int NST = (SPLIT || TRANS || X3) ? FH * FN : (GEGLU ? FH * FN / 2 : FH * ((FN + 1) / 2));
    constexpr int OSZ = (X3 && !GEGLU) ? 4 : 2;
    constexpr int OOB = (int)0x80000000;
    static_assert((BM == 256 || BM == 192) && (BN == 256 || BN == 320 || (BN == 128 && BM == 256 && X3 && AMODE == AMODE_CONV3 && !GEGLU && !SPLIT && !TRANS)), "tiles built for this kernel");
    static_assert(!GEGLU || FN % 2 == 0, "GEGLU pairs hidden / gate column blocks inside a wave");

    extern __shared__ __attribute__((aligned(16))) char smem[];

    const int tid = threadIdx.x;
    const int lane = tid & 63, wave = __builtin_amdgcn_readfirstlane(tid >> 6);
    const int wr = wave >> 2, wc = wave & 3;
    const int l15 = lane & 15, g = lane >> 4;
    const int lrow = lane >> 3, csrc = (lane & 7) ^ lrow;

    static_assert(!SPLIT || (!RES && !GEGLU), "split-K slabs carry raw accumulators: the epilogue runs in the reduce kernel");
    static_assert(!TRANS || (!RES && !GEGLU && !SPLIT && AMODE == AMODE_DENSE), "transposed output: dense A, bias only");
    static_assert(!F8 || (!X3 && !TRANS && !GEGLU), "fp8 operands: plain / residual / split-K epilogues");
    const int ntn = p.N / BN;
    const int ntm = (p.M + BM - 1) / BM;
    const int nsl = SPLIT ? splitk : 1;
    const int ntiles = ntm * ntn * nsl;
    const int G = gridDim.x;
    const int nk = (X3 ? p.K / 96 : p.K / 64) / nsl;
    const int first = __builtin_amdgcn_readfirstlane(xcd_remap(blockIdx.x, G));
    const int my_tiles = (ntiles - first + G - 1) / G;
    const int S = my_tiles * nk;

    const int PIX = X3 ? p.lda * 2 : p.Cin * 2;
    const long a_bytes = AMODE == AMODE_DENSE ? (long)p.M * p.lda * 2 : (long)(p.M / (p.Hout * p.Wout)) * p.Hin * p.Win * PIX;
    const __amdgpu_buffer_rsrc_t rsrcA = __builtin_amdgcn_make_buffer_rsrc(const_cast<void*>(p.A), 0, (int)a_bytes, 0x00020000);
    const __amdgpu_buffer_rsrc_t rsrcB = __builtin_amdgcn_make_buffer_rsrc(const_cast<void*>(p.W), 0, (int)((long)p.N * p.Kpad * 2), 0x00020000);
    const __amdgpu_buffer_rsrc_t rsrcBias = __builtin_amdgcn_make_buffer_rsrc(const_cast<float*>(p.bias), 0, p.bias ? p.N * 4 : 0, 0x00020000);
    const int nbatch = (p.M + p.rows_per_batch - 1) / p.rows_per_batch;
    const __amdgpu_buffer_rsrc_t rsrcRb =
        __builtin_amdgcn_make_buffer_rsrc(const_cast<float*>(p.rowbias), 0, p.rowbias ? ((nbatch - 1) * p.ldrb + p.N) * 4 : 0, 0x00020000);
    const long o_bytes = TRANS ? (long)((p.M + p.rows_per_batch - 1) / p.rows_per_batch) * p.N * p.ldo * OSZ : (long)p.M * p.ldo * OSZ;
    const __amdgpu_buffer_rsrc_t rsrcO = __builtin_amdgcn_make_buffer_rsrc(p.out, 0, (int)o_bytes, 0x00020000);
    const __amdgpu_buffer_rsrc_t rsrcR = __builtin_amdgcn_make_buffer_rsrc(const_cast<void*>(p.residual), 0, RES ? (int)((long)p.M * p.ldr * OSZ) : 0, 0x00020000);

    int l_tile = first, l_kt = 0;
    int l_k0 = 0;
    int a_off[NA];
    int a_yx[NA];
    int b_voff;
    const int b_step = 64 * p.Kpad * 2;
    int apiece[NA];
    if constexpr (BM == 256) {
        apiece[0] = wave; apiece[1] = 16 + wave; apiece[2] = 8 + wave; apiece[3] = 24 + wave;
    } else {
        apiece[0] = wave < 6 ? wave : wave + 6;
        apiece[1] = wave < 4 ? 14 + wave : 2 + wave;
        apiece[2] = wave < 2 ? 10 + wave : 16 + wave;
    }
    const int cpt = AMODE == AMODE_DENSE ? 1 : (X3 ? p.Cin / 32 : p.Cin / 64);
    const int cpt_rcp = (65536 + cpt - 1) / cpt;
    constexpr bool TAPIN = X3 && AMODE != AMODE_DENSE;
    const int ntap = p.conv == 2 ? 4 : 9;
    auto kt_split = [&](int kt, int& tap, int& c) {
        if (TAPIN) {
            c = p.conv == 2 ? (kt >> 2) : ((kt * 7282) >> 16);
            tap = kt - c * ntap;
        } else {
            tap = (kt * cpt_rcp) >> 16;
            c = kt - tap * cpt;
        }
    };
    int ka = 0, tap_ky = 0, tap_kx = 0, tap_off = 0;
    auto k_position = [&]() {
        const int kt = l_k0 + l_kt;
        if (AMODE == AMODE_DENSE) {
            ka = kt * 128;
        } else {
            int tap, c;
// ... 191 lines not shown
                            acc[i][j][3] = fmaf(__uint_as_float(w1 & 0xffff0000u), f8_inv, c[3]);
                        } else {
                        acc[i][j][0] = c[0] + __uint_as_float(w0 << 16);
                        acc[i][j][1] = c[1] + __uint_as_float(w0 & 0xffff0000u);
                        acc[i][j][2] = c[2] + __uint_as_float(w1 << 16);
                        acc[i][j][3] = c[3] + __uint_as_float(w1 & 0xffff0000u);
                        }
                    } else {
                        acc[i][j] = c;
                    }
                }
            }
        }
    };
    const __amdgpu_buffer_rsrc_t rsrcWs = __builtin_amdgcn_make_buffer_rsrc(p.ws, 0, SPLIT ? (int)((long)nsl * p.M * p.N * 4) : 0, 0x00020000);
    auto store_rows = [&](int wtile, auto I0) {
        constexpr int i0 = decltype(I0)::value;
        const int tile = wtile / nsl;
        const int m0 = (tile / ntn) * BM + wr * HM, n0 = (tile % ntn) * BN + wc * WN;
        int ln = lane;
        asm volatile("" : "+v"(ln));
        const int pr = ln >> 2, pg = ln & 3;
        const int paddr = (pr + 16 * pg) * 4;
        auto perm = [&](unsigned v) { return (unsigned)__builtin_amdgcn_ds_bpermute(paddr, (int)v); };
        if constexpr (SPLIT) {
            const int slice = wtile - tile * nsl;
            const int voff = (pr * p.N + 4 * pg) * 4;
#pragma unroll
            for (int i = i0; i < i0 + FH; ++i) {
                const int vo = m0 + i * 16 + pr < p.M ? voff : OOB;
#pragma unroll
                for (int j = 0; j < FN; ++j) {
                    u32x4 w = __builtin_bit_cast(u32x4, acc[i][j]);
                    w[0] = perm(w[0]); w[1] = perm(w[1]); w[2] = perm(w[2]); w[3] = perm(w[3]);
                    __builtin_amdgcn_raw_buffer_store_b128(w, rsrcWs, vo, ((slice * p.M + m0 + i * 16) * p.N + n0 + j * 16) * 4, 0);
                }
            }
            return;
        }
        if constexpr (TRANS) {
            const int voff = (pr * p.ldo + 4 * pg) * OSZ;
#pragma unroll
            for (int i = i0; i < i0 + FH; ++i) {
                const int mb = m0 + i * 16;
                const int bb = mb / p.rows_per_batch, sb = mb - bb * p.rows_per_batch;
#pragma unroll
                for (int j = 0; j < FN; ++j) {
                    if constexpr (X3) {
                        u32x4 w4 = __builtin_bit_cast(u32x4, acc[i][j]);
                        w4[0] = perm(w4[0]); w4[1] = perm(w4[1]); w4[2] = perm(w4[2]); w4[3] = perm(w4[3]);
                        if (p.flags & FFN_IG_OUT_KV64) {
                            const float f0 = __uint_as_float(w4[0]), f1 = __uint_as_float(w4[1]), f2 = __uint_as_float(w4[2]), f3 = __uint_as_float(w4[3]);
                            u32x2 hi, lo;
                            hi[0] = pack_bf16x2(f0, f1);
                            hi[1] = pack_bf16x2(f2, f3);
                            lo[0] = pack_bf16x2(f0 - __uint_as_float(hi[0] << 16), f1 - __uint_as_float(hi[0] & 0xffff0000u));
                            lo[1] = pack_bf16x2(f2 - __uint_as_float(hi[1] << 16), f3 - __uint_as_float(hi[1] & 0xffff0000u));
                            const int vo2 = mb + 4 * pg < p.M ? (pr * p.ldo * 4 + 4 * pg * 2) : OOB;
                            const int so2 = (bb * p.N + n0 + j * 16) * p.ldo * 4 + (sb >> 6) * 256 + (sb & 63) * 2;
                            __builtin_amdgcn_raw_buffer_store_b64(hi, rsrcO, vo2, so2, 0);
                            __builtin_amdgcn_raw_buffer_store_b64(lo, rsrcO, vo2, so2 + 128, 0);
                            continue;
                        }
                        __builtin_amdgcn_raw_buffer_store_b128(w4, rsrcO, mb + 4 * pg < p.M ? voff : OOB, ((bb * p.N + n0 + j * 16) * p.ldo + sb) * 4, 0);
                        continue;
                    }
                    u32x2 w;
                    w[0] = perm(pack_bf16x2(acc[i][j][0], acc[i][j][1]));
                    w[1] = perm(pack_bf16x2(acc[i][j][2], acc[i][j][3]));
                    __builtin_amdgcn_raw_buffer_store_b64(w, rsrcO, mb + 4 * pg < p.M ? voff : OOB, ((bb * p.N + n0 + j * 16) * p.ldo + sb) * 2, 0);
                }
            }
            return;
        }
        if (PP_ABL == 4) {
#pragma unroll
            for (int i = i0; i < i0 + FH; ++i)
#pragma unroll
                for (int j = 0; j < FN; ++j) asm volatile("" ::"v"(acc[i][j]));
            return;
        }
        if constexpr (X3) {
            const int voff = (pr * p.ldo + 4 * pg) * 4;
#pragma unroll
            for (int i = i0; i < i0 + FH; ++i) {
                const int vo = m0 + i * 16 + pr < p.M ? voff : OOB;
                if constexpr (GEGLU) {
                    const int vo2 = m0 + i * 16 + pr < p.M ? (pr * p.ldo + 4 * pg) * 2 : OOB;
#pragma unroll
                    for (int j = 0; j + 1 < FN; j += 2) {
                        const f32x2_t g01 = (PP_ABL == 3 ? f32x2_t{acc[i][j + 1][0], acc[i][j + 1][1]} : gelu_erf26_2(f32x2_t{acc[i][j + 1][0], acc[i][j + 1][1]})) * f32x2_t{acc[i][j][0], acc[i][j][1]};
                        const f32x2_t g23 = (PP_ABL == 3 ? f32x2_t{acc[i][j + 1][2], acc[i][j + 1][3]} : gelu_erf26_2(f32x2_t{acc[i][j + 1][2], acc[i][j + 1][3]})) * f32x2_t{acc[i][j][2], acc[i][j][3]};
                        const float v[4] = {g01[0], g01[1], g23[0], g23[1]};
                        u32x2 hi, lo;
                        hi[0] = pack_bf16x2(v[0], v[1]);
                        hi[1] = pack_bf16x2(v[2], v[3]);
                        lo[0] = pack_bf16x2(v[0] - __uint_as_float(hi[0] << 16), v[1] - __uint_as_float(hi[0] & 0xffff0000u));
                        lo[1] = pack_bf16x2(v[2] - __uint_as_float(hi[1] << 16), v[3] - __uint_as_float(hi[1] & 0xffff0000u));
                        hi[0] = perm(hi[0]); hi[1] = perm(hi[1]); lo[0] = perm(lo[0]); lo[1] = perm(lo[1]);
                        const int so = ((m0 + i * 16) * p.ldo + n0 + (j / 2) * 16) * 2;
                        __builtin_amdgcn_raw_buffer_store_b64(hi, rsrcO, vo2, so, 0);
                        __builtin_amdgcn_raw_buffer_store_b64(lo, rsrcO, vo2, so + 64, 0);
                    }
                } else {
#pragma unroll
                    for (int j = 0; j < FN; ++j) {
                        u32x4 w = __builtin_bit_cast(u32x4, acc[i][j]);
                        w[0] = perm(w[0]); w[1] = perm(w[1]); w[2] = perm(w[2]); w[3] = perm(w[3]);
                        const int nf = n0 + j * 16;
                        if (p.flags & FFN_IG_OUT_PAIR) {
                            const float f0 = __uint_as_float(w[0]), f1 = __uint_as_float(w[1]), f2 = __uint_as_float(w[2]), f3 = __uint_as_float(w[3]);
                            u32x2 hi, lo;
                            hi[0] = pack_bf16x2(f0, f1);
                            hi[1] = pack_bf16x2(f2, f3);
                            lo[0] = pack_bf16x2(f0 - __uint_as_float(hi[0] << 16), f1 - __uint_as_float(hi[0] & 0xffff0000u));
                            lo[1] = pack_bf16x2(f2 - __uint_as_float(hi[1] << 16), f3 - __uint_as_float(hi[1] & 0xffff0000u));
                            const int vo2 = m0 + i * 16 + pr < p.M ? (pr * p.ldo + 4 * pg) * 2 : OOB;
                            const int so2 = (m0 + i * 16) * p.ldo * 2 + (nf >> 5) * 128 + (nf & 31) * 2;
                            __builtin_amdgcn_raw_buffer_store_b64(hi, rsrcO, vo2, so2, 0);
                            __builtin_amdgcn_raw_buffer_store_b64(lo, rsrcO, vo2, so2 + 64, 0);
                            continue;
                        }
                        if ((p.flags & FFN_IG_OUT_KV64) && nf >= p.kv64_from) {
                            const float f0 = __uint_as_float(w[0]), f1 = __uint_as_float(w[1]), f2 = __uint_as_float(w[2]), f3 = __uint_as_float(w[3]);
                            u32x2 hi, lo;
                            hi[0] = pack_bf16x2(f0, f1);
                            hi[1] = pack_bf16x2(f2, f3);
                            lo[0] = pack_bf16x2(f0 - __uint_as_float(hi[0] << 16), f1 - __uint_as_float(hi[0] & 0xffff0000u));
                            lo[1] = pack_bf16x2(f2 - __uint_as_float(hi[1] << 16), f3 - __uint_as_float(hi[1] & 0xffff0000u));
                            const int crel = nf - p.kv64_from;
                            const int vo2 = m0 + i * 16 + pr < p.M ? (pr * p.ldo * 4 + 4 * pg * 2) : OOB;
                            const int so2 = ((m0 + i * 16) * p.ldo + p.kv64_from) * 4 + (crel >> 6) * 256 + (crel & 63) * 2;
                            __builtin_amdgcn_raw_buffer_store_b64(hi, rsrcO, vo2, so2, 0);
                            __builtin_amdgcn_raw_buffer_store_b64(lo, rsrcO, vo2, so2 + 128, 0);
                            continue;
                        }
                        __builtin_amdgcn_raw_buffer_store_b128(w, rsrcO, vo, ((m0 + i * 16) * p.ldo + n0 + j * 16) * 4, 0);
                    }
                }
            }
            return;
        }
        if constexpr (GEGLU) {
            const int voff = (l15 * p.ldo + 4 * g) * 2;
#pragma unroll
            for (int i = i0; i < i0 + FH; ++i)
#pragma unroll
                for (int j = 0; j + 1 < FN; j += 2) {
                    const f32x2_t g01 = (PP_ABL == 3 ? f32x2_t{acc[i][j + 1][0], acc[i][j + 1][1]} : gelu_erf_fast2(f32x2_t{acc[i][j + 1][0], acc[i][j + 1][1]})) * f32x2_t{acc[i][j][0], acc[i][j][1]};
                    const f32x2_t g23 = (PP_ABL == 3 ? f32x2_t{acc[i][j + 1][2], acc[i][j + 1][3]} : gelu_erf_fast2(f32x2_t{acc[i][j + 1][2], acc[i][j + 1][3]})) * f32x2_t{acc[i][j][2], acc[i][j][3]};
                    u32x2 w;
                    w[0] = pack_bf16x2(g01[0], g01[1]);
                    w[1] = pack_bf16x2(g23[0], g23[1]);
                    __builtin_amdgcn_raw_buffer_store_b64(w, rsrcO, voff, ((m0 + i * 16) * p.ldo + n0 / 2 + (j / 2) * 16) * 2, 0);
                }
            return;
        }
        if constexpr (F8) {
#pragma unroll
            for (int i = i0; i < i0 + FH; ++i)
#pragma unroll
                for (int j = 0; j < FN; ++j) {
                    acc[i][j] *= p.alpha;
                    asm volatile("" : "+v"(acc[i][j]));
                }
            __builtin_amdgcn_sched_barrier(0);
// ... 234 lines not shown
                read_a(ra, a_rd0, 0);
                read_b(rb, b_rd0);
            } else if (needB) {
#pragma unroll
                for (int i = 0; i < NB1; ++i) issue_b(i, lb);
                pp_wait_vmcnt<NB1>();
            } else {
                pp_wait_vmcnt<0>();
            }
            __builtin_amdgcn_sched_barrier(0);
            pp_barrier();
            mfma_rows(I0_t{});
            __builtin_amdgcn_sched_barrier(0);
            pp_barrier();

            read_a(ra, a_rd0, FH);
            if (needB) {
#pragma unroll
                for (int i = NB1; i < FN; ++i) issue_b(i, lb);
            }
            if (p_tile >= 0) {
                init_rows(c_tile, I4_t{});
                p_tile = -1;
            }
            __builtin_amdgcn_sched_barrier(0);
            pp_barrier();
            mfma_rows(I4_t{});
            __builtin_amdgcn_sched_barrier(0);
            pp_barrier();

            read_a(ra, a_rd1, 0);
            read_b(rb, b_rd1);
            if (needA) {
                k_position();
                issue_a(0, la);
                issue_a(1, la);
            }
            __builtin_amdgcn_sched_barrier(0);
            pp_barrier();
            mfma_rows(I0_t{});
            __builtin_amdgcn_sched_barrier(0);
            pp_barrier();

            read_a(ra, a_rd1, FH);
            if (more) {
                if (needA) {
#pragma unroll
                    for (int i = 2; i < NA; ++i) issue_a(i, la);
                }
                advance();
                if (PP_ABL == 9 && c_kt < 2) {}
                else if (switched) pp_wait_vmcnt<NA - 2 + (SPLIT ? 0 : 6)>();
                else pp_wait_vmcnt<NA - 2>();
            }
            if (c_kt == nk - 1) {
#ifdef PP_TRACE
                if (tid == 0) pp_trace[blockIdx.x * 64 + 2 * ((c_tile - first) / G & 31)] = __builtin_amdgcn_s_memrealtime();
#endif
                store_rows(c_tile, I0_t{});
#ifdef PP_TRACE
                if (tid == 0) pp_trace[blockIdx.x * 64 + 2 * ((c_tile - first) / G & 31) + 1] = __builtin_amdgcn_s_memrealtime();
#endif
            }
            __builtin_amdgcn_sched_barrier(0);
            pp_barrier();
            mfma_rows(I4_t{});
            __builtin_amdgcn_sched_barrier(0);
            pp_barrier();

            buf = nb;
            if (++c_kt == nk) {
                p_tile = c_tile;
                c_kt = 0;
                c_tile += G;
            }
        }
    }
    if (p_tile >= 0) store_rows(p_tile, I4_t{});
    if (wr == 0) pp_barrier();
#ifdef PP_STAMP
    if (blockIdx.x == 7) pp_stamp_out[tid] = *reinterpret_cast<const unsigned long long*>(smem + CV + 12288 + tid * 8);
#endif
}
```

freefine_amd/csrc/norms.h:

```cpp
#pragma once
#include "common.h"
#include "layernorm_row.h"

__device__ __forceinline__ int gn_row_count(int p0, int p1, int row, int ppi) {
    return p0 + row < p1 ? (p1 - p0 - row + ppi - 1) / ppi : 0;
}
template <typename T>
__global__ __launch_bounds__(256) void gn_partial_kernel(const T* __restrict__ x, float* __restrict__ partial, int HW,
                                                         int C, int pix_per_chunk) {
    constexpr int EPC = DT<T>::EPC;
    extern __shared__ __attribute__((aligned(16))) char smem[];
    float* ls = reinterpret_cast<float*>(smem);
    const int b = blockIdx.y, chunk = blockIdx.x, nchunk = gridDim.x;
    const int cch = C / EPC;
    const int tid = threadIdx.x;
    const int p0 = chunk * pix_per_chunk;
    const int p1 = min(HW, p0 + pix_per_chunk);
    float* dst = partial + ((long)b * nchunk + chunk) * 2 * C;
    for (int cbase = 0; cbase < cch; cbase += 256) {
        const int cols = min(cch - cbase, 256);
        const int ppi = max(1, 256 / cols);
        const int cc = cbase + tid % cols, pp = tid / cols;
        const bool active = pp < ppi;
        if (active) {
// ... 2 lines not shown
            for (int e = 0; e < EPC; ++e) s[e] = ss[e] = pv[e] = 0.f;
            const T* src = x + ((long)b * HW) * C + cc * EPC;
            int px = p0 + pp;
            const int cnt = gn_row_count(p0, p1, pp, ppi), first = px;
            for (; px + 7 * ppi < p1; px += 8 * ppi) {
                u32x4 v[8];
#pragma unroll
                for (int u = 0; u < 8; ++u) v[u] = *reinterpret_cast<const u32x4*>(src + (long)(px + u * ppi) * C);
                __builtin_amdgcn_sched_barrier(0);
                if (px == first) DT<T>::unpack(v[0], pv);
#pragma unroll
                for (int u = 0; u < 8; ++u) {
                    float f[EPC];
                    DT<T>::unpack(v[u], f);
#pragma unroll
                    for (int e = 0; e < EPC; ++e) {
                        const float d = f[e] - pv[e];
                        s[e] += d;
                        ss[e] += d * d;
                    }
                }
            }
            for (; px < p1; px += ppi) {
                const u32x4 v = *reinterpret_cast<const u32x4*>(src + (long)px * C);
                float f[EPC];
                DT<T>::unpack(v, f);
                if (px == first) DT<T>::unpack(v, pv);
#pragma unroll
                for (int e = 0; e < EPC; ++e) {
                    const float d = f[e] - pv[e];
                    s[e] += d;
                    ss[e] += d * d;
                }
            }
            const float inv = cnt > 0 ? 1.0f / (float)cnt : 0.f;
#pragma unroll
            for (int e = 0; e < EPC; ++e) {
                const float m = s[e] * inv;
                ls[(pp * cols + (cc - cbase)) * 2 * EPC + 2 * e] = pv[e] + m;
                ls[(pp * cols + (cc - cbase)) * 2 * EPC + 2 * e + 1] = fmaxf(ss[e] - s[e] * m, 0.f);
            }
        }
        __syncthreads();
        const int n = max(p1 - p0, 0);
        for (int i = tid; i < cols * EPC; i += 256) {
            double sm = 0.0, sq = 0.0;
            for (int r = 0; r < ppi; ++r) {
                const double nr = (double)gn_row_count(p0, p1, r, ppi), mr = (double)ls[(r * cols * EPC + i) * 2];
                sm += nr * mr;
                sq += (double)ls[(r * cols * EPC + i) * 2 + 1] + nr * mr * mr;
            }
            const double mean = n > 0 ? sm / (double)n : 0.0;
            const double m2 = fmax(sq - sm * mean, 0.0);
            dst[(cbase * EPC + i) * 2] = (float)mean;
            dst[(cbase * EPC + i) * 2 + 1] = (float)m2;
        }
        __syncthreads();
    }
}

__global__ __launch_bounds__(64) void gn_finalize_kernel(const float* __restrict__ partial, const float* __restrict__ gamma,
                                                         const float* __restrict__ beta, float* __restrict__ scale,
                                                         float* __restrict__ shift, int HW, int C, int G, int nchunk,
                                                         int pix_per_chunk, float eps) {
    const int g = blockIdx.x, b = blockIdx.y, lane = threadIdx.x;
    const int cg = C / G;
    const double n = (double)HW * cg;
    double s = 0.0, sq = 0.0;
    for (int i = lane; i < nchunk * cg; i += 64) {
        const int ch = i / cg, c = g * cg + (i - ch * cg);
        const double ni = (double)max(min(HW, (ch + 1) * pix_per_chunk) - ch * pix_per_chunk, 0);
        const float* src = partial + (((long)b * nchunk + ch) * C + c) * 2;
        const double mi = (double)src[0];
        s += ni * mi;
        sq += (double)src[1] + ni * mi * mi;
    }
    for (int off = 32; off > 0; off >>= 1) {
        s += __shfl_xor(s, off);
        sq += __shfl_xor(sq, off);
    }
    const double mean = s / n;
    const double m2 = fmax(sq - s * mean, 0.0);
    const float rstd = (float)(1.0 / sqrt(m2 / n + (double)eps));
    for (int i = lane; i < cg; i += 64) {
        const int c = g * cg + i;
        const float sc = rstd * gamma[c];
        scale[(long)b * C + c] = sc;
        shift[(long)b * C + c] = (float)((double)beta[c] - mean * (double)sc);
    }
}

template <typename T, bool SILU, bool PAIR = false>
__global__ __launch_bounds__(256) void gn_apply_kernel(const T* __restrict__ x, T* __restrict__ y,
                                                       const float* __restrict__ scale, const float* __restrict__ shift,
                                                       long nchunks_total, int HW, int C) {
    constexpr int EPC = DT<T>::EPC;
    const int cch = C / EPC;
    for (long i = (long)blockIdx.x * 256 + threadIdx.x; i < nchunks_total; i += (long)gridDim.x * 256) {
        const long pix = i / cch;
        const int cc = (int)(i - pix * cch);
        const int b = (int)(pix / HW);
        const u32x4 v = *reinterpret_cast<const u32x4*>(x + i * EPC);
        float f[EPC];
        DT<T>::unpack(v, f);
        const float* sc = scale + (long)b * C + cc * EPC;
        const float* sh = shift + (long)b * C + cc * EPC;
#pragma unroll
        for (int e = 0; e < EPC; ++e) {
            float t = f[e] * sc[e] + sh[e];
            if (SILU) t = silu_for<T>(t);
            f[e] = t;
        }
        if constexpr (PAIR) store_pair4(reinterpret_cast<bf16*>(y), pix, C, cc * EPC, f);
        else *reinterpret_cast<u32x4*>(y + i * EPC) = DT<T>::pack(f);
    }
}

template <bool SILU, bool RAW = false>
__global__ __launch_bounds__(256) void gn_apply_pair8_kernel(const float* __restrict__ x, bf16* __restrict__ y, const float* __restrict__ scale,
                                                             const float* __restrict__ shift, long n8_total, int HW, int C, bf16* __restrict__ yraw = nullptr) {
    const int cch = C / 8;
    const int lo_off = pair_lo(C);
    for (long i = (long)blockIdx.x * 256 + threadIdx.x; i < n8_total; i += (long)gridDim.x * 256) {
        const long pix = i / cch;
        const int c = (int)(i - pix * cch) * 8;
        const int b = (int)(pix / HW);
        const f32x4 v0 = *reinterpret_cast<const f32x4*>(x + pix * C + c), v1 = *reinterpret_cast<const f32x4*>(x + pix * C + c + 4);
        const f32x4 s0 = *reinterpret_cast<const f32x4*>(scale + (long)b * C + c), s1 = *reinterpret_cast<const f32x4*>(scale + (long)b * C + c + 4);
        const f32x4 h0 = *reinterpret_cast<const f32x4*>(shift + (long)b * C + c), h1 = *reinterpret_cast<const f32x4*>(shift + (long)b * C + c + 4);
        float f[8];
#pragma unroll
        for (int e = 0; e < 4; ++e) {
            f[e] = v0[e] * s0[e] + h0[e];
            f[4 + e] = v1[e] * s1[e] + h1[e];
        }
        if (SILU) {
#pragma unroll
            for (int e = 0; e < 8; ++e) f[e] = silu_fast(f[e]);
        }
        u32x4 hi, lo;
#pragma unroll
        for (int w = 0; w < 4; ++w) {
            hi[w] = pack_bf16x2(f[2 * w], f[2 * w + 1]);
            lo[w] = pack_bf16x2(f[2 * w] - __uint_as_float(hi[w] << 16), f[2 * w + 1] - __uint_as_float(hi[w] & 0xffff0000u));
        }
        bf16* q = y + pix * 2 * C + pair_pos(c, C);
        *reinterpret_cast<u32x4*>(q) = hi;
        *reinterpret_cast<u32x4*>(q + lo_off) = lo;
        if (RAW) {
            const float r[8] = {v0[0], v0[1], v0[2], v0[3], v1[0], v1[1], v1[2], v1[3]};
#pragma unroll
            for (int w = 0; w < 4; ++w) {
                hi[w] = pack_bf16x2(r[2 * w], r[2 * w + 1]);
                lo[w] = pack_bf16x2(r[2 * w] - __uint_as_float(hi[w] << 16), r[2 * w + 1] - __uint_as_float(hi[w] & 0xffff0000u));
            }
            bf16* qr = yraw + pix * 2 * C + pair_pos(c, C);
            *reinterpret_cast<u32x4*>(qr) = hi;
            *reinterpret_cast<u32x4*>(qr + lo_off) = lo;
        }
    }
}

template <bool SILU>
__global__ __launch_bounds__(256) void gn_apply_f8_kernel(const bf16* __restrict__ x, uint8_t* __restrict__ y, const float* __restrict__ scale,
                                                          const float* __restrict__ shift, long nchunks_total, int HW, int C, int Cp, float qs) {
    const int cch = Cp / 16;
// ... 131 lines not shown
```

freefine_amd/ops.py:

```python
import ctypes as CT
import math

import os
import threading

import torch

from . import _lib as L


def _dt(t):
    if t.dtype == torch.float32:
        return L.FFN_F32
    if t.dtype == torch.bfloat16:
        return L.FFN_BF16
    raise TypeError(f"unsupported dtype {t.dtype}")


def epc(dtype):
    return 4 if dtype == torch.float32 else 8


def kstage(dtype):
    return 8 * epc(dtype)
# ... 183 lines not shown
                           lambda: lib.ffn_igemm(_stream(), dcode, CT.byref(d))), "ffn_igemm(conv 2x2)")
    if out is None:
        out = torch.empty(B, 4 * Hin * Win, cout, dtype=odt, device=x.device)
    out.view(B, Hin, 2, Win, 2, cout).copy_(y.view(B, Hin, Win, 2, 2, cout).permute(0, 1, 3, 2, 4, 5))
    return out


F8_ACT_SCALE = 16.0


def pack_conv3x3_f8(w, cin_pad=None):
    cout, cin = w.shape[:2]
    cp = cin_pad or (cin + 127) // 128 * 128
    w2 = torch.zeros(cout, 3, 3, cp, dtype=torch.float32, device=w.device)
    w2[..., :cin] = w.permute(0, 2, 3, 1).float()
    amax = float(w2.abs().max())
    k = math.floor(math.log2(448.0 / amax)) if amax > 0 else 0
    ws = 2.0 ** k
    q = (w2 * ws).clamp(-448.0, 448.0).to(torch.float8_e4m3fn).reshape(cout, 9 * cp).contiguous().view(torch.uint8)
    q._ffn_f8 = (cp, 1.0 / (ws * F8_ACT_SCALE))
    return q


def is_f8(w):
    return getattr(w, "_ffn_f8", None) is not None


def groupnorm_f8(x, gamma, beta, G, eps, Cp, silu=False, ws=None):
    lib = L.load()
    B, HW, Cc = x.shape
    assert x.dtype == torch.bfloat16
    out = torch.empty(B, HW, Cp, dtype=torch.uint8, device=x.device)
    out._ffn_f8_act = Cc
    partial, scale, shift = ws if ws is not None else gn_workspace(B, HW, Cc, x.device)
    call = lambda: lib.ffn_groupnorm_f8(_stream(), x.data_ptr(), out.data_ptr(), gamma.data_ptr(), beta.data_ptr(), B, HW, Cc, Cp, G, eps,
                                        L.NORM_SILU if silu else 0, F8_ACT_SCALE, partial.data_ptr(), scale.data_ptr(), shift.data_ptr())
    L.check(_timed("gn_partial+gn_finalize+gn_apply_f8", 0.0, x.numel() * 2.0 + out.numel(), call), "ffn_groupnorm_f8")
    return out


def pack_geglu(w, b, dtype, x3=False):
    f2, k = w.shape
    f = f2 // 2
    assert f % 16 == 0
    idx = torch.arange(f, device=w.device).reshape(f // 16, 16)
    order = torch.stack([idx, idx + f], dim=1).reshape(-1)
    wp = pack_linear(w[order], dtype, x3)
    bp = None if b is None else b[order].float().contiguous()
    return wp, bp


def _mark_pair(t, C):
    t._ffn_pair = C
    return t


def pair_width(x):
    return getattr(x, "_ffn_pair", None)


def split_pair(x, K=None):
    lib = L.load()
    assert x.dtype == torch.float32 and x.stride(-1) == 1
    K = K if K is not None else x.shape[-1]
    rows = x.numel() // x.shape[-1]
    ld = x.stride(-2) if x.ndim > 1 else x.shape[-1]
    out = torch.empty(*x.shape[:-1], 2 * K, dtype=torch.bfloat16, device=x.device)
    L.check(_timed("split_pair_kernel", 0.0, 8.0 * rows * K, lambda: lib.ffn_split_pair(_stream(), x.data_ptr(), out.data_ptr(), rows, K, ld)),
            "ffn_split_pair")
    return _mark_pair(out, K)


_WS = {}
WS_BYTES = 96 << 20


def _workspace(device):
    key = (device, torch.cuda.current_stream().cuda_stream)
    ws = _WS.get(key)
    if ws is None:
        ws = _WS[key] = torch.empty(WS_BYTES // 4, dtype=torch.float32, device=device)
    return ws

_TLS = threading.local()


def _invariant():
    return getattr(_TLS, "batch_invariant", False)


class batch_invariant:

    def __enter__(self):
        self.prev, _TLS.batch_invariant = _invariant(), True

    def __exit__(self, *exc):
        _TLS.batch_invariant = self.prev


def linear(x, w, bias=None, *, K=None, out=None, residual=None, rowbias=None, rows_per_batch=None, silu=False,
           geglu=False, out_f32=False, transposed_ld=None, alpha=1.0, splitk=0, out_pair=False, gelu=False, relu=False, kv64_from=None, qgelu=False):
    lib = L.load()
    K = K if K is not None else x.shape[-1]
    M = x.numel() // x.shape[-1]
    N = w.shape[0]
    d = L.IgemmDesc()
    x3 = is_x3(w)
    if x3 and pair_width(x) is not None:
        K = pair_width(x)
        M = x.numel() // x.shape[-1]
        xa = x
    else:
        xa = split_pair(x, K) if x3 else x
    dcode = L.FFN_BF16X3 if x3 else _dt(x)
    d.A, d.W = xa.data_ptr(), w.data_ptr()
    d.bias, d.rowbias, d.residual = _p(bias), _p(rowbias), _p(residual)
    d.M, d.N, d.K, d.Kpad = M, N, K, w.stride(0)
    d.lda = xa.stride(-2) if xa.ndim > 1 else xa.shape[-1]
    d.x3 = int(w._ffn_x3) if x3 else 0
    d.a_lo = (32 if d.x3 == 2 else K) if x3 else 0
    odt = torch.float32 if x3 else x.dtype
    d.rows_per_batch = rows_per_batch or M
    d.ldrb = rowbias.stride(0) if rowbias is not None else 0
    flags = 0
    n_out = N
    if silu:
        flags |= L.IG_OUT_SILU
    if gelu:
        flags |= L.IG_OUT_GELU
    if relu:
        flags |= L.IG_OUT_RELU
    if qgelu:
        flags |= L.IG_OUT_QGELU
    if geglu:
        flags |= L.IG_GEGLU
        n_out = N // 2
    if out_f32:
        flags |= L.IG_OUT_F32
    if transposed_ld is not None:
        flags |= L.IG_OUT_TRANSPOSED
        nb = M // d.rows_per_batch
        if out is None:
            alloc = torch.zeros if transposed_ld > d.rows_per_batch else torch.empty
            out = alloc(nb, N, transposed_ld, dtype=odt, device=x.device)
        d.ldo = transposed_ld
    elif out_pair:
        assert x3 and out is None
        flags |= L.IG_OUT_PAIR
        out = _mark_pair(torch.empty(*x.shape[:-1], 2 * n_out, dtype=torch.bfloat16, device=x.device), n_out)
        d.ldo = 2 * n_out
    else:
        if out is None:
            out = torch.empty(*x.shape[:-1], n_out, dtype=torch.float32 if out_f32 else odt, device=x.device)
        d.ldo = out.stride(-2) if out.ndim > 1 else n_out
    assert xa.stride(-1) == 1 and out.stride(-1) == 1 and (residual is None or residual.stride(-1) == 1), "linear: x, out and residual need contiguous columns"
    d.ldr = (residual.stride(-2) if residual.ndim > 1 else residual.shape[-1]) if residual is not None else 0
    d.out = out.data_ptr()
    if kv64_from is not None:
        assert x3 and residual is None and rowbias is None and not (silu or gelu or relu or qgelu or geglu or out_pair)
        flags |= L.IG_OUT_KV64
        d.kv64_from = int(kv64_from)
        splitk = 1
    d.flags, d.alpha, d.conv = flags, alpha, 0
    if splitk == 0 and _invariant():
        splitk = 1
    d.splitk, d.ws, d.ws_bytes = splitk, _workspace(x.device).data_ptr(), WS_BYTES
    if _PROF is None:
        L.check(lib.ffn_igemm(_stream(), dcode, CT.byref(d)), "ffn_igemm")
    else:
        esz = x.element_size()
        L.check(_timed(_igemm_name(lib, dcode, d), 2.0 * M * N * K, esz * (M * K + N * K + M * n_out),
                       lambda: lib.ffn_igemm(_stream(), dcode, CT.byref(d))), "ffn_igemm")
    return out


def conv3x3(x, w, bias, B, Hin, Win, Cin, *, stride=1, pad=1, upsample=False, out=None, residual=None, rowbias=None,
            rowbias_ld=None, out_f32=False, Hout=None, Wout=None, splitk=0, relu=False):
    lib = L.load()
    He, We = (Hin * 2, Win * 2) if upsample else (Hin, Win)
    if Hout is None:
        Hout = (He + 2 * pad - 3) // stride + 1
        Wout = (We + 2 * pad - 3) // stride + 1
    N = w.shape[0]
    d = L.IgemmDesc()
    x3 = is_x3(w)
    f8 = is_f8(w)
    if f8:
        assert x.dtype == torch.uint8 and x.shape[-1] == w._ffn_f8[0] and out_f32 is False
        Cin = x.shape[-1]
        xa = x
    elif x3 and pair_width(x) is not None:
        assert pair_width(x) == Cin
        xa = x
    else:
        xa = split_pair(x, Cin) if x3 else x
    dcode = L.FFN_FP8 if f8 else (L.FFN_BF16X3 if x3 else _dt(x))
    odt = torch.float32 if x3 else (torch.bfloat16 if f8 else x.dtype)
    d.A, d.W = xa.data_ptr(), w.data_ptr()
    d.bias, d.rowbias, d.residual = _p(bias), _p(rowbias), _p(residual)
    d.M, d.N, d.K, d.Kpad = B * Hout * Wout, N, 9 * Cin, w.shape[1]
    d.lda = 2 * Cin if x3 else Cin
    d.x3 = int(w._ffn_x3) if x3 else 0
    d.a_lo = (32 if d.x3 == 2 else Cin) if x3 else 0
    d.rows_per_batch = Hout * Wout
    d.ldrb = (rowbias_ld or rowbias.stride(0)) if rowbias is not None else 0
    if out is None:
        out = torch.empty(B, Hout * Wout, N, dtype=torch.float32 if out_f32 else odt, device=x.device)
    assert xa.is_contiguous(), "conv3x3: x must be contiguous (a column view of a wider buffer has no pixel stride the kernels could follow)"
    assert out.stride(-1) == 1 and (residual is None or residual.stride(-1) == 1), "conv3x3: out and residual need contiguous columns"
    d.out, d.ldo = out.data_ptr(), out.stride(-2)
    d.ldr = residual.stride(-2) if residual is not None else 0
    d.Hin, d.Win, d.Cin, d.Hout, d.Wout = Hin, Win, Cin, Hout, Wout
    d.stride, d.pad, d.upsample = stride, pad, 1 if upsample else 0
    d.flags, d.alpha, d.conv = (L.IG_OUT_F32 if out_f32 else 0) | (L.IG_OUT_RELU if relu else 0), (w._ffn_f8[1] if f8 else 1.0), 1
    if splitk == 0 and _invariant():
        splitk = 1
    d.splitk, d.ws, d.ws_bytes = splitk, _workspace(x.device).data_ptr(), WS_BYTES
    if _PROF is None:
        L.check(lib.ffn_igemm(_stream(), dcode, CT.byref(d)), "ffn_igemm(conv)")
    else:
        esz = x.element_size()
        k_real = 9 * getattr(x, "_ffn_f8_act", Cin)
        L.check(_timed(_igemm_name(lib, dcode, d), 2.0 * d.M * N * k_real, esz * (x.numel() + N * d.K + d.M * N),
                       lambda: lib.ffn_igemm(_stream(), dcode, CT.byref(d))), "ffn_igemm(conv)")
    return out


class AttnEntrySpec:
    __slots__ = ("q_row", "kv_row", "w_const", "w_slope", "wq", "kmask", "qsel", "flags", "hr_row")

    def __init__(self, q_row, kv_row, w_const=1.0, w_slope=0.0, wq=None, kmask=None, qsel=None, flags=0, hr_row=None):
        self.q_row, self.kv_row, self.w_const, self.w_slope = q_row, kv_row, w_const, w_slope
        self.wq, self.kmask, self.qsel, self.flags, self.hr_row = wq, kmask, qsel, flags, hr_row

    def remap(self, row_map, logical_row):
        return AttnEntrySpec(row_map[self.q_row], row_map[self.kv_row], self.w_const, self.w_slope, self.wq, self.kmask, self.qsel,
                             self.flags, logical_row if self.hr_row is None else self.hr_row)

    def pinned(self, logical_row):
        return self if self.hr_row is not None else AttnEntrySpec(self.q_row, self.kv_row, self.w_const, self.w_slope, self.wq, self.kmask, self.qsel,
                                                                  self.flags, logical_row)

    def renumber(self, ren, kv_ren=None):
        kv_ren = ren if kv_ren is None else kv_ren
        if self.q_row not in ren or self.kv_row not in kv_ren:
            raise ValueError(f"attention term (q row {self.q_row}, kv row {self.kv_row}) reaches outside the rows of this phase {sorted(ren)} / {sorted(kv_ren)}")
        return AttnEntrySpec(ren[self.q_row], kv_ren[self.kv_row], self.w_const, self.w_slope, self.wq, self.kmask, self.qsel, self.flags, self.hr_row)

    def shifted(self, base, logical_row, kv_base=None):
        return AttnEntrySpec(self.q_row + base, self.kv_row + (base if kv_base is None else kv_base), self.w_const, self.w_slope, self.wq,
                             self.kmask, self.qsel, self.flags, logical_row if self.hr_row is None else self.hr_row)


def _set_entries(d, passes, b0, nb, ptr=_p):
    for p, rows in enumerate(passes):
        for b in range(nb):
            sp = rows[b0 + b]
            e = d.e[p * L.ATT_MAXB + b]
            if sp is None:
                e.w_const = e.w_slope = 0.0
                continue
            e.q_row, e.kv_row, e.w_const, e.w_slope = sp.q_row, sp.kv_row, sp.w_const, sp.w_slope
            e.wq, e.kmask, e.qsel, e.flags = ptr(sp.wq), ptr(sp.kmask), ptr(sp.qsel), sp.flags
            hr = sp.hr_row if sp.hr_row is not None else (b0 + b if b0 else None)
            e.hr_row = 0 if hr is None else hr + 1


def _takes_kv_images(lib, d):
    probe = L.AttnDesc.from_buffer_copy(d)
    probe.kv_pair = 1
    return lib.ffn_attn_kernel_name(L.FFN_BF16X3, CT.byref(probe), CT.create_string_buffer(160), 160) == 0


def kv_images_ok(Dh, S, Sk, passes=None, nbytes=0):
    if not (_ATTN_PRESPLIT and nbytes < 2 ** 31 - 65536):
        return False
    lib = L.load()
    passes = passes or [[AttnEntrySpec(0, 0)]]
    Bo = len(passes[0])
    for b0 in range(0, Bo, L.ATT_MAXB):
        nb = min(L.ATT_MAXB, Bo - b0)
        d = L.AttnDesc()
        d.Bo, d.S, d.Sk, d.heads, d.D, d.npass = nb, S, Sk, 1, Dh, len(passes)
        d.ldq = d.ldk = d.ldo = Dh
        d.ldvt = Sk
        d.w_dev = 1
        _set_entries(d, passes, b0, nb, lambda t: 0 if t is None else 1)
        if not _takes_kv_images(lib, d):
            return False
    return True


_CUS = {}


def attn_row_split(Bo, wg_per_row, maxb, cus):
    best_n, best = min(maxb, Bo), None
    for n in range(min(maxb, Bo), 0, -1):
        full, rest = divmod(Bo, n)
        rounds = full * -(-n * wg_per_row // cus) + (-(-rest * wg_per_row // cus) if rest else 0)
        if best is None or rounds < best:
            best_n, best = n, rounds
    return best_n


def attention(q, k, vt, heads, scale, passes=None, *, Sk=None, out=None, w_dev=None, Bo=None, C=None, x3=False, out_pair=False, kv_images=False, causal=False):
    lib = L.load()
    Bq, S, _ = q.shape
    Cq = C if C is not None else q.shape[2]
    Sk = Sk if Sk is not None else k.shape[1]
    Dh = Cq // heads
    if passes is None:
        passes = [[AttnEntrySpec(b, b) for b in range(Bq)]]
    if causal:
        passes = [[None if sp is None else AttnEntrySpec(sp.q_row, sp.kv_row, sp.w_const, sp.w_slope, sp.wq, sp.kmask, sp.qsel, sp.flags | L.ATT_CAUSAL, sp.hr_row)
                   for sp in rows] for rows in passes]
    Bo = Bo if Bo is not None else len(passes[0])
    out_pair = bool(out_pair and x3 and q.dtype == torch.float32 and Dh <= 64 and out is None and Cq % 8 == 0)
    if out_pair:
        out = _mark_pair(torch.empty(Bo, S, 2 * Cq, dtype=torch.bfloat16, device=q.device), Cq)
    if out is None:
        out = torch.empty(Bo, S, Cq, dtype=q.dtype, device=q.device)
    for rows in passes:
        assert len(rows) == Bo
    esz = q.element_size()
    dcode = L.FFN_BF16X3 if (x3 and q.dtype == torch.float32) else _dt(q)
    descs = []
    chunk = L.ATT_MAXB
    if Bo > 1 and Dh == 64 and S >= 128 and Sk % 64 == 0 and q.is_cuda:
        di = q.device.index if q.device.index is not None else torch.cuda.current_device()
        if di not in _CUS:
            _CUS[di] = torch.cuda.get_device_properties(di).multi_processor_count
        chunk = attn_row_split(Bo, heads * -(-S // 256), L.ATT_MAXB, _CUS[di])
    for b0 in range(0, Bo, chunk):
        nb = min(chunk, Bo - b0)
        d = L.AttnDesc()
        d.q, d.k, d.vt, d.w_dev = q.data_ptr(), k.data_ptr(), vt.data_ptr(), _p(w_dev)
        d.out = out.data_ptr() + b0 * S * Cq * esz
        d.Bo, d.S, d.Sk, d.heads, d.D = nb, S, Sk, heads, Dh
        d.ldq, d.ldk, d.ldvt, d.ldo = q.stride(1), k.stride(1), vt.stride(1), (2 * Cq if out_pair else Cq)
        d.out_pair = 1 if out_pair else 0
        d.scale, d.npass = scale, len(passes)
        d.kv_pair = 1 if kv_images else 0
        _set_entries(d, passes, b0, nb)
        descs.append((b0, nb, d))
    if kv_images:
        assert dcode == L.FFN_BF16X3 and kv_images_ok(Dh, S, Sk)
    elif dcode == L.FFN_BF16X3 and _ATTN_PRESPLIT and k.stride(2) == 1 and vt.stride(2) == 1 and k.stride(0) == Sk * k.stride(1) \
            and vt.stride(0) == heads * Dh * vt.stride(1) and k.shape[0] * Sk * heads * Dh * 4 < 2 ** 31 - 65536:
        if all(_takes_kv_images(lib, d) for _, _, d in descs):
            Bk = k.shape[0]
            kp = torch.empty(Bk, Sk, 2 * heads * Dh, dtype=torch.bfloat16, device=q.device)
            vp = torch.empty(Bk, heads * Dh, 2 * Sk, dtype=torch.bfloat16, device=q.device)
            L.check(_timed("attn_presplit_kernel", 0.0, 16.0 * Bk * Sk * heads * Dh,
                           lambda: lib.ffn_attn_presplit(_stream(), k.data_ptr(), vt.data_ptr(), kp.data_ptr(), vp.data_ptr(), Bk, Sk, heads, k.stride(1), vt.stride(1))),
                    "ffn_attn_presplit")
            for _, _, d in descs:
                d.k, d.vt, d.kv_pair = kp.data_ptr(), vp.data_ptr(), 1
                d.ldk, d.ldvt = heads * Dh, Sk
    for b0, nb, d in descs:
        if _PROF is None:
            L.check(lib.ffn_attn(_stream(), dcode, CT.byref(d)), "ffn_attn")
        else:
            nterms = sum(1 for rows in passes for sp in rows[b0:b0 + nb] if sp is not None and (sp.w_const != 0.0 or sp.w_slope != 0.0))
            nbuf = CT.create_string_buffer(160)
            lib.ffn_attn_kernel_name(dcode, CT.byref(d), nbuf, 160)
            L.check(_timed(nbuf.value.decode(), 4.0 * nterms * S * Sk * Cq,
                           esz * nterms * (S * Cq + 2 * Sk * Cq) + esz * nb * S * Cq,
                           lambda: lib.ffn_attn(_stream(), dcode, CT.byref(d))), "ffn_attn")
    return out


def gn_workspace(B, HW, C, device):
    lib = L.load()
    nchunk = lib.ffn_gn_nchunk(HW)
    return (torch.empty(B * nchunk * 2 * C, dtype=torch.float32, device=device),
            torch.empty(B, C, dtype=torch.float32, device=device), torch.empty(B, C, dtype=torch.float32, device=device))


def groupnorm(x, gamma, beta, G, eps, silu=False, out=None, ws=None, pair=False):
    lib = L.load()
    B, HW, Cc = x.shape
    if pair:
        assert x.dtype == torch.float32 and out is None
        out = _mark_pair(torch.empty(B, HW, 2 * Cc, dtype=torch.bfloat16, device=x.device), Cc)
    if out is None:
        out = torch.empty_like(x)
    nb = B
    if _invariant() and lib.ffn_gn_fused(1, HW, Cc, G) and not lib.ffn_gn_fused(B, HW, Cc, G):
        while not lib.ffn_gn_fused(nb, HW, Cc, G):
            nb = (nb + 1) // 2
    if lib.ffn_gn_fused(nb, HW, Cc, G):
        partial = scale = shift = None
    else:
        partial, scale, shift = ws if ws is not None else gn_workspace(B, HW, Cc, x.device)
    fl = (L.NORM_SILU if silu else 0) | (L.NORM_OUT_PAIR if pair else 0)
    def call():
        rc = 0
        for b0 in range(0, B, nb):
            n = min(nb, B - b0)
            rc = lib.ffn_groupnorm(_stream(), _dt(x), x.data_ptr() + b0 * HW * Cc * x.element_size(), out.data_ptr() + b0 * HW * out.shape[-1] * out.element_size(),
                                   gamma.data_ptr(), beta.data_ptr(), n, HW, Cc, G, eps, fl, _p(partial), _p(scale), _p(shift))
            if rc:
                break
        return rc
    if _PROF is None:
        L.check(call(), "ffn_groupnorm")
    else:
        name = f"gn_fused_kernel<{_tname(x)}>" if partial is None else f"gn_partial+gn_finalize+gn_apply<{_tname(x)}>"
        L.check(_timed(name, 0.0, 2.0 * x.numel() * x.element_size(), call), "ffn_groupnorm")
    return out


def groupnorm_pair_raw(x, gamma, beta, G, eps, silu=False, ws=None):
    lib = L.load()
    B, HW, Cc = x.shape
    if Cc % 8 != 0 or lib.ffn_gn_fused(1 if _invariant() else B, HW, Cc, G) or not x.is_contiguous():
        return groupnorm(x, gamma, beta, G, eps, silu=silu, pair=True, ws=ws), split_pair(x, Cc)
    assert x.dtype == torch.float32
    y = _mark_pair(torch.empty(B, HW, 2 * Cc, dtype=torch.bfloat16, device=x.device), Cc)
    yr = _mark_pair(torch.empty(B, HW, 2 * Cc, dtype=torch.bfloat16, device=x.device), Cc)
    partial, scale, shift = ws if ws is not None else gn_workspace(B, HW, Cc, x.device)
    call = lambda: lib.ffn_groupnorm_pair_raw(_stream(), x.data_ptr(), y.data_ptr(), yr.data_ptr(), gamma.data_ptr(), beta.data_ptr(), B, HW, Cc, G, eps,
                                              L.NORM_SILU if silu else 0, _p(partial), _p(scale), _p(shift))
    if _PROF is None:
        L.check(call(), "ffn_groupnorm_pair_raw")
    else:
        L.check(_timed("gn_partial+gn_finalize+gn_apply<float> (+ raw pair)", 0.0, 3.0 * x.numel() * x.element_size(), call), "ffn_groupnorm_pair_raw")
    return y, yr


def layernorm(x, gamma, beta, eps=1e-5, out=None, pair=False):
    lib = L.load()
    Cc = x.shape[-1]
    M = x.numel() // Cc
    if pair:
        assert x.dtype == torch.float32 and out is None
        out = _mark_pair(torch.empty(*x.shape[:-1], 2 * Cc, dtype=torch.bfloat16, device=x.device), Cc)
        call = lambda: lib.ffn_layernorm_pair(_stream(), x.data_ptr(), out.data_ptr(), gamma.data_ptr(), beta.data_ptr(), M, Cc, eps)
    else:
        if out is None:
            out = torch.empty_like(x)
        call = lambda: lib.ffn_layernorm(_stream(), _dt(x), x.data_ptr(), out.data_ptr(), gamma.data_ptr(), beta.data_ptr(), M, Cc, eps)
    if _PROF is None:
        L.check(call(), "ffn_layernorm")
    else:
        L.check(_timed(f"layernorm_kernel<{_tname(x)}>", 0.0, 2.0 * x.numel() * x.element_size(), call), "ffn_layernorm")
    return out


def pool_layernorm(x, ids, gamma, beta, eps=1e-5, out=None, pair=False):
    lib = L.load()
    assert x.ndim == 3 and x.is_contiguous()
    N, S, Cc = x.shape
    if ids is not None:
        assert ids.dtype == torch.int32 and tuple(ids.shape) == (N, S) and ids.is_contiguous() and ids.device == x.device
    if pair:
        assert x.dtype == torch.float32
        if out is None:
            out = torch.empty(N, 2 * Cc, dtype=torch.bfloat16, device=x.device)
        assert out.dtype == torch.bfloat16 and tuple(out.shape) == (N, 2 * Cc) and out.is_contiguous()
        out = _mark_pair(out, Cc)
    elif out is None:
        out = torch.empty(N, Cc, dtype=x.dtype, device=x.device)
    else:
        assert out.dtype == x.dtype and tuple(out.shape) == (N, Cc) and out.is_contiguous()
    L.check(_timed(f"pool_layernorm_kernel<{_tname(x)}>", 0.0, 2.0 * N * Cc * x.element_size(),
                   lambda: lib.ffn_pool_layernorm(_stream(), _dt(x), x.data_ptr(), _p(ids), out.data_ptr(), gamma.data_ptr(), beta.data_ptr(), N, S, Cc, eps,
                                                  int(pair))), "ffn_pool_layernorm")
    return out


def cosine_rows(a, b, out=None):
    lib = L.load()
    assert a.dtype == b.dtype == torch.float32 and a.ndim == b.ndim == 2 and a.is_contiguous() and b.is_contiguous() and a.device == b.device
    B, P = a.shape
    assert b.shape[1] == P
    if out is None:
        out = torch.empty(B, dtype=torch.float32, device=a.device)
    else:
        assert out.dtype == torch.float32 and tuple(out.shape) == (B,) and out.is_contiguous()
    L.check(_timed("cosine_rows_kernel", 6.0 * B * P, 4.0 * (B * P + b.shape[0] * P + B),
                   lambda: lib.ffn_cosine_rows(_stream(), a.data_ptr(), b.data_ptr(), out.data_ptr(), B, P, b.shape[0])), "ffn_cosine_rows")
    return out


def softmax_rows(x, scale=1.0, out=None):
    lib = L.load()
    N = x.shape[-1]
    M = x.numel() // N
    if out is None:
        out = torch.empty_like(x)
    L.check(_timed(f"softmax_rows_kernel<{_tname(x)}>", 0.0, 2.0 * x.numel() * x.element_size(),
                   lambda: lib.ffn_softmax_rows(_stream(), _dt(x), x.data_ptr(), out.data_ptr(), M, N, scale)), "ffn_softmax_rows")
    return out


def cfg_masked(eps_u, eps_c, mask_f, cfg, out=None):
    lib = L.load()
    if out is None:
        out = torch.empty_like(eps_u)
    HW = eps_u.shape[-1] * eps_u.shape[-2]
    L.check(_timed("cfg_masked_kernel", 0.0, 12.0 * eps_u.numel(),
                   lambda: lib.ffn_cfg_masked(_stream(), eps_u.data_ptr(), eps_c.data_ptr(), _p(mask_f), float(cfg), out.data_ptr(),
# ... 864 lines not shown
```

freefine_amd/unet.py:

```python
import ctypes as CT
import weakref

import torch

from . import _lib as L
from . import ops
from .config import UNetConfig


class _Res:
    pass


class HipUNet:
    def __init__(self, cfg: UNetConfig, state, dtype=torch.bfloat16, device="cuda:0", x3=False, fp8_conv=False):
        assert not x3 or dtype == torch.float32, "split-bf16 mode keeps fp32 activations"
        assert not fp8_conv or dtype == torch.bfloat16, "fp8 convolutions are an option of the bf16 fast mode"
        self.x3 = bool(x3)
        self.fp8_conv = bool(fp8_conv)
        self.cfg, self.dtype, self.device = cfg, dtype, torch.device(device)
        self.in_channels = cfg.in_channels
        self.hook, self.controller = "edit", None
        self._graphs = {}
        self._capture_stream = None
# ... 409 lines not shown
                if c.cur_att_layer != 0:
                    for _ in range(self.num_attention_calls):
                        c._tick()
            return hit
        fp = self._plan_all_slow(B, H, W)
        if len(self._plan_cache) > 64:
            self._plan_cache.clear()
        self._plan_cache[key] = fp
        return fp

    def _plan_all_slow(self, B, H, W):
        fps = []
        ru = self._reuse
        join_tb = self.join_block_tb(ru["join"]) if (ru is not None and ru["mode"] == "replay") else -1
        kv_from = ru["kv_from"] if (ru is not None and ru["mode"] == "replay_kv") else None
        calls = self._call_list(H, W)
        drop = ru is not None and ru["mode"] == "replay" and bool(ru.get("drop_tail"))
        for ci, (is_cross, place, S, heads) in enumerate(calls):
            self._in_phase_a = ci // 2 < join_tb
            self._kv_ext = kv_from is not None and not is_cross and ci // 2 >= kv_from
            if drop and ci == len(calls) - 1:
                self._in_phase_a = True
            plan = self._plan(is_cross, place, B, S, heads)
            if drop and ci == len(calls) - 2:
                plan = self._without_ref_queries(plan, B)
            if plan["passes"] is None:
                fps.append(0)
                continue
            rows = tuple(tuple(None if e is None else (e.q_row, e.kv_row, e.w_const, e.w_slope, e.flags, e.hr_row,
                                                       0 if e.wq is None else e.wq.data_ptr(),
                                                       0 if e.kmask is None else e.kmask.data_ptr(),
                                                       0 if e.qsel is None else e.qsel.data_ptr()) for e in r) for r in plan["passes"])
            fps.append((plan["kind"], plan["needs_cg"], rows))
        self._in_phase_a = self._kv_ext = False
        return (self.hook, tuple(fps))

    def join_block_tb(self, join):
        tb = len([t for blk in self.down if blk.attn for t in blk.attn]) + 1
        for blk in self.up[:join]:
            tb += len(blk.attn) if blk.attn else 0
        return tb

    def _capture(self, sample, text_kv, sig):
        ctrls = self._ctrls()
        state = [(c.cur_att_layer, c.cur_step) for c in ctrls]
        x_static = sample.clone()
        ru = self._reuse
        ref_in = None
        if ru is not None and ru["mode"] == "replay":
            ref_in = [t.clone() for t in ru["state"]]
            ru["state_run"] = ref_in
        if ru is not None and ru["mode"] == "replay_kv":
            ref_in = ru["static"] = []
            ru["static_bufs"] = []
        self._run(x_static, text_kv)
        if ru is not None and ru["mode"] == "replay_kv":
            ru["static_ready"] = True
        for c, st in zip(ctrls, state):
            c.cur_att_layer, c.cur_step = st
        torch.cuda.synchronize()
        graph = torch.cuda.CUDAGraph()
        if self._capture_stream is None:
            self._capture_stream = torch.cuda.Stream(device=x_static.device)
        with torch.cuda.graph(graph, stream=self._capture_stream):
            out = self._run(x_static, text_kv)
        rec = ru is not None and ru["mode"] == "record"
        g = dict(graph=graph, x=x_static, out=out, ref_in=ref_in, ref_bufs=ru.get("static_bufs") if ru is not None else None,
                 boundary=self.last_boundary if rec else None, kv=self.last_kv if rec else None, device=x_static.device.index)
        if ru is not None:
            for k in ("state_run", "static", "static_bufs", "static_ready"):
                ru.pop(k, None)
        self._graphs[sig] = g
        return g

    def _gn(self, x, gb, eps, silu):
        B, HW, C = x.shape
        return ops.groupnorm(x, gb[0], gb[1], self.cfg.norm_num_groups, eps, silu=silu, pair=self.x3)

    def _gn_conv_in(self, x, gb, w):
        if ops.is_f8(w):
            return ops.groupnorm_f8(x, gb[0], gb[1], self.cfg.norm_num_groups, self.cfg.norm_eps, w._ffn_f8[0], silu=True)
        return self._gn(x, gb, self.cfg.norm_eps, True)

    def _resblock(self, r, x, B, H, W, temb_all, out=None):
        cin = x.shape[-1]
        if r.sc is not None and self.x3 and not ops.is_f8(r.c1[0]) and ops.pair_width(x) is None and x.dtype == torch.float32:
            h, x = ops.groupnorm_pair_raw(x, r.n1[0], r.n1[1], self.cfg.norm_num_groups, self.cfg.norm_eps, silu=True)
        else:
            h = self._gn_conv_in(x, r.n1, r.c1[0])
        rb = temb_all[:, r.temb_off:r.temb_off + r.cout]
        h = ops.conv3x3(h, r.c1[0], r.c1[1], B, H, W, cin, rowbias=rb, rowbias_ld=temb_all.shape[1])
        h = self._gn_conv_in(h, r.n2, r.c2[0])
        if r.sc is not None:
            x = ops.linear(x, r.sc[0], r.sc[1], K=cin)
        return ops.conv3x3(h, r.c2[0], r.c2[1], B, H, W, r.cout, residual=x, out=out)

    def _without_ref_queries(self, plan, B):
        keep = self._reuse["idx_a_list"]
        passes = plan["passes"] if plan["passes"] is not None else [[ops.AttnEntrySpec(b, b) for b in range(B)]]
        pin = lambda e, r: e if (e is None or e.hr_row is not None) else ops.AttnEntrySpec(e.q_row, e.kv_row, e.w_const, e.w_slope, e.wq, e.kmask, e.qsel, e.flags, r)
        out = dict(plan)
        out["passes"] = [[pin(rows[r], r) for r in keep] for rows in passes]
        return out

    def _self_plan(self, t, place, B, S, drop_ref_queries=False):
        if self.controller is None:
            return dict(kind="plain", needs_cg=False, passes=[[ops.AttnEntrySpec(r, r, hr_row=r) for r in self._reuse["idx_a_list"]]]) if drop_ref_queries else None
        plan = self._plan(False, place, B, S, t.heads)
        if drop_ref_queries:
            assert plan["kind"] != "shared_kv"
            plan = self._without_ref_queries(plan, B)
        return plan

    def _attention(self, t, is_cross, place, q, k, vt, ldq_view, B, S, Sk, plan=None, kv_images=False):
        D = t.C // t.heads
        scale = D ** -0.5
        if is_cross and self.controller is not None:
            plan = self._plan(is_cross, place, B, S, t.heads)
        if plan is None:
            return ops.attention(q, k, vt, t.heads, scale, None, Sk=Sk, C=t.C, x3=self.x3, out_pair=self.x3, kv_images=kv_images)
        if plan["kind"] == "shared_kv":
            assert not kv_images
            rr = plan["ref_rows"]
            kc = k[..., :t.C] if k.shape[-1] != t.C else k
            k2 = torch.cat([kc, kc[rr]], dim=1).contiguous()
            vt2 = torch.cat([vt[..., :Sk], vt[rr][..., :Sk]], dim=2).contiguous()
            return ops.attention(q, k2, vt2, t.heads, scale, plan["passes"], Sk=2 * Sk, C=t.C, x3=self.x3, out_pair=self.x3)
        return ops.attention(q, k, vt, t.heads, scale, plan["passes"], Sk=Sk, C=t.C, w_dev=self.cg_dev if plan["needs_cg"] else None, x3=self.x3,
                             out_pair=self.x3, kv_images=kv_images)

    def _kv_buffers(self, B, S, C, ldv):
        ru = self._reuse
        i = ru["cursor"]
        ru["cursor"] = i + 1
        if ru.get("static_ready"):
            return ru["static_bufs"][i]
        k_ref, vt_ref = ru["state"][2 * i], ru["state"][2 * i + 1]
        nr = k_ref.shape[0]
        assert tuple(k_ref.shape) == (nr, S, C) and tuple(vt_ref.shape) == (nr, C, ldv), (tuple(k_ref.shape), tuple(vt_ref.shape), (S, C, ldv))
        qk = torch.empty(B + nr, S, 2 * C, dtype=self.dtype, device=self.device)
        vt = torch.empty(B + nr, C, ldv, dtype=self.dtype, device=self.device)
        qk[B:, :, C:].copy_(k_ref)
        vt[B:].copy_(vt_ref)
        if ru.get("static") is not None:
            ru["static_bufs"].append((qk, vt))
            ru["static"] += [qk[B:, :, C:], vt[B:]]
        return qk, vt

    def _transformer_block(self, t, x, B, H, W, place, kv_text, out=None, drop=None, tb=0):
        S, C = H * W, t.C
        res0 = x
        ru = self._reuse
        h = self._gn(x, t.norm, 1e-6, False)
        h = ops.linear(h, t.proj_in[0], t.proj_in[1], K=C)
        y = ops.layernorm(h, *t.ln[0], pair=self.x3)
        ldv = (S + 7) // 8 * 8
        if ru is not None and ru["mode"] == "replay_kv" and tb >= ru["kv_from"]:
            qk, vt = self._kv_buffers(B, S, C, ldv)
            ops.linear(y, t.w_qk1, None, K=C, out=qk[:B])
            ops.linear(y, t.w_v1, None, K=C, rows_per_batch=S, transposed_ld=ldv, out=vt[:B])
            self._kv_ext = True
            a = self._attention(t, False, place, qk[:B], qk[..., C:], vt, 2 * C, B, S, S, plan=self._self_plan(t, place, B, S))
            self._kv_ext = False
        else:
            plan = self._self_plan(t, place, B, S, drop_ref_queries=drop is not None)
            rec = ru is not None and ru["mode"] == "record" and ru.get("kv_from") is not None and tb >= ru["kv_from"]
            img = self.x3 and not rec and (plan is None or plan["kind"] != "shared_kv") and \
                ops.kv_images_ok(C // t.heads, S, S, None if plan is None else plan["passes"], B * max(S * 2 * C, C * ldv) * 4)
            qk = ops.linear(y, t.w_qk1, None, K=C, kv64_from=C if img else None)
            vt = ops.linear(y, t.w_v1, None, K=C, rows_per_batch=S, transposed_ld=ldv, kv64_from=0 if img else None)
            if rec:
                self.last_kv.append((qk[..., C:], vt))
            a = self._attention(t, False, place, qk, qk[..., C:], vt, 2 * C, B, S, S, plan=plan, kv_images=img)
        if drop is not None:
            idx, kv_text = drop
            h, res0, B = h.index_select(0, idx), res0.index_select(0, idx), idx.shape[0]
            self._in_phase_a = True
        h = ops.linear(a, t.o1[0], t.o1[1], K=C, residual=h)
        y = ops.layernorm(h, *t.ln[1], pair=self.x3)
        q = ops.linear(y, t.w_q2, None, K=C)
        k2, vt2 = kv_text
        a = self._attention(t, True, place, q, k2, vt2, C, B, S, k2.shape[1])
        h = ops.linear(a, t.o2[0], t.o2[1], K=C, residual=h)
        y = ops.layernorm(h, *t.ln[2], pair=self.x3)
        y = ops.linear(y, t.ff1[0], t.ff1[1], K=C, geglu=True, out_pair=self.x3)
        h = ops.linear(y, t.ff2[0], t.ff2[1], K=4 * C, residual=h, out_pair=self.x3 and C % 32 == 0)
        return ops.linear(h, t.proj_out[0], t.proj_out[1], K=C, residual=res0, out=out)

    def _run(self, sample, text_kv, stop_up=None):
        cfg = self.cfg
        B, _, H, W = sample.shape
        dt = self.dtype
        ru = self._reuse
        replay = ru is not None and ru["mode"] == "replay"
        record = ru is not None and ru["mode"] == "record"
        replay_kv = ru is not None and ru["mode"] == "replay_kv"
        BB = B
        if replay:
            sample = sample.index_select(0, ru["idx_a"])
            B = sample.shape[0]
            text_kv = list(ru["text_kv_a"][:self.join_block_tb(ru["join"])]) + list(text_kv[self.join_block_tb(ru["join"]):])
        if replay_kv:
            sample = sample.index_select(0, ru["idx_a"])
            B = sample.shape[0]
            text_kv = ru["text_kv_a"]
            ru["cursor"] = 0
        if record and ru.get("kv_from") is not None:
            self.last_kv = []
        self._in_phase_a = replay
        ti = iter(text_kv)
        tb = 0
        te = ops.timestep_embed(self.t_dev, self.freq, BB, dt, flip=cfg.flip_sin_to_cos)
        e1 = ops.linear(te, self.te1[0], self.te1[1], K=self.te1[2], silu=True)
        e2 = ops.linear(e1, self.te2[0], self.te2[1], K=self.te2[2], silu=True)
        temb_all = ops.linear(e2, self.temb_w, self.temb_b, K=self.te2[0].shape[0], out_f32=True)
        temb_full = temb_all
        temb_all = temb_all[:B]
        x = ops.pack_nchw(sample, list(range(B)), self.cin_pad, dt)
        x = ops.conv3x3(x, self.conv_in[0], self.conv_in[1], B, H, W, self.cin_pad)
        skips = [(x, H, W)]
        n = len(self.down)
        for i, blk in enumerate(self.down):
            for j, r in enumerate(blk.res):
                x = self._resblock(r, x, B, H, W, temb_all)
                if blk.attn:
                    x = self._transformer_block(blk.attn[j], x, B, H, W, "down", next(ti), tb=tb)
                    tb += 1
                skips.append((x, H, W))
            if blk.down is not None:
                C = x.shape[-1]
                x = ops.conv3x3(x, blk.down[0], blk.down[1], B, H, W, C, stride=2)
                H, W = (H + 1) // 2, (W + 1) // 2
                skips.append((x, H, W))
        x = self._resblock(self.mid.res[0], x, B, H, W, temb_all)
        x = self._transformer_block(self.mid.attn[0], x, B, H, W, "mid", next(ti), tb=tb)
        tb += 1
        def cat_dst(C1, HW):
            return ops.cat_dst((B, HW), C1, skips[-1][0].shape[-1], dt, x.device) if skips else None
        x = self._resblock(self.mid.res[1], x, B, H, W, temb_all, out=cat_dst(self.mid.res[1].cout, H * W))
        for i, blk in enumerate(self.up):
            if ru is not None and ru.get("join") is not None and i == ru["join"]:
                if record:
                    self.last_boundary = [x] + [s for s, _, _ in reversed(skips)]
                if replay:
                    state = ru.get("state_run") or ru["state"]
                    assert len(state) == 1 + len(skips), (len(state), len(skips))
                    merge = lambda a, r: torch.cat([a, r.to(a.dtype)], 0).index_select(0, ru["perm"])
                    x = merge(x, state[0])
                    skips = [(merge(s, st), sh, sw) for (s, sh, sw), st in zip(skips, reversed(state[1:]))]
                    B, temb_all = BB, temb_full
                    self._in_phase_a = False
            for j, r in enumerate(blk.res):
                s, sh, sw = skips.pop()
                assert (sh, sw) == (H, W)
                x = ops.concat(x, s)
                dst = cat_dst(r.cout, H * W) if j + 1 < len(blk.res) else None
                x = self._resblock(r, x, B, H, W, temb_all, out=None if blk.attn else dst)
                if blk.attn:
                    last = replay and bool(ru.get("drop_tail")) and blk.attn[j] is self.transformers[-1]
                    drop = (ru["idx_a"], ru["text_kv_a"][-1]) if last else None
                    x = self._transformer_block(blk.attn[j], x, B, H, W, "up", next(ti), out=dst, drop=drop, tb=tb)
                    tb += 1
                    if last:
                        assert dst is None and i == len(self.up) - 1 and j == len(blk.res) - 1, "the last transformer block closes the network"
                        B, temb_all = x.shape[0], temb_full[:x.shape[0]]
            if blk.up is not None:
                C = x.shape[-1]
                if blk.up2 is not None and stop_up is None and ops.up2x_eligible(C, C, B * H * W):
                    x = ops.conv3x3_up2x(x, blk.up2, blk.up[1], B, H, W, C, out=cat_dst(C, 4 * H * W))
                else:
                    x = ops.conv3x3(x, blk.up[0], blk.up[1], B, H, W, C, upsample=True, out=cat_dst(C, 4 * H * W))
                H, W = 2 * H, 2 * W
            if stop_up is not None and i == stop_up:
                return x, H, W
        C = x.shape[-1]
        if self.conv_out_n4 is not None:
            x = ops.groupnorm(x, self.norm_out[0], self.norm_out[1], cfg.norm_num_groups, cfg.norm_eps, silu=True)
            eps = ops.conv3x3_n4(x, self.conv_out_n4, self.conv_out[1], B, H, W, C)
        else:
            x = self._gn(x, self.norm_out, cfg.norm_eps, True)
            eps = ops.conv3x3(x, self.conv_out[0], self.conv_out[1], B, H, W, C, out_f32=True)
        eps = ops.nhwc_to_nchw_f32(eps, cfg.out_channels, H, W)
        self._in_phase_a = False
        if B != BB:
            eps = torch.zeros(BB, *eps.shape[1:], dtype=eps.dtype, device=eps.device).index_copy_(0, ru["idx_a"], eps)
        return eps
```

include/freefine_hip.h:

```cpp
#ifndef FREEFINE_HIP_H
#define FREEFINE_HIP_H
#include <stdint.h>
#ifdef __cplusplus
extern "C" {
#endif

enum { FFN_F32 = 0, FFN_BF16 = 1, FFN_BF16X3 = 2 ,
       FFN_FP8 = 3  };
enum { FFN_OK = 0, FFN_EINVAL = -22, FFN_ENOSYS = -38, FFN_EHIP = -5, FFN_ENOSPC = -28 };

int ffn_version(void);
const char* ffn_last_error(void);
int ffn_device_info(int device, char* name, int name_len);
int ffn_graph_launch(void* stream, void* graph_exec);

enum {
    FFN_IG_OUT_SILU = 1 << 0,
    FFN_IG_OUT_F32 = 1 << 1,
    FFN_IG_GEGLU = 1 << 2,
    FFN_IG_OUT_TRANSPOSED = 1 << 3,
    FFN_IG_OUT_PAIR = 1 << 4,
    FFN_IG_OUT_GELU = 1 << 5,
    FFN_IG_OUT_KV64 = 1 << 7,
    FFN_IG_OUT_RELU = 1 << 6,
    FFN_IG_OUT_QGELU = 1 << 8
};
typedef struct ffn_igemm_desc {
    const void* A;
    const void* W;
    void* out;
    const float* bias;
    const float* rowbias;
    const void* residual;
    int M, N, K, Kpad;
    int lda, ldo, ldr, ldrb;
    int rows_per_batch;
    int Hin, Win, Cin, Hout, Wout, stride, pad, upsample;
    int flags;
    float alpha;
    int conv;
    int splitk;
    void* ws;
    long ws_bytes;
    int a_lo;
    int x3;
    int f8;
    int kv64_from;
} ffn_igemm_desc;
int ffn_igemm(void* stream, int dtype, const ffn_igemm_desc* d);
int ffn_split_pair(void* stream, const float* src, void* dst, long rows, int C, int ld_src);
int ffn_conv3x3_n4(void* stream, int dtype, const void* x, const float* w, const float* bias, float* out, int B, int H, int W, int Cin);
int ffn_groupnorm_f8(void* stream, const void* x_bf16, void* y_e4m3, const float* gamma, const float* beta, int B, int HW, int C, int Cp,
                     int G, float eps, int silu, float qscale, float* partial_ws, float* scale, float* shift);
int ffn_igemm_tune(void* stream, int dtype, const ffn_igemm_desc* d);
int ffn_igemm_tune_entry_ints(void);
int ffn_igemm_tune_export(int* buf, int max_entries);
int ffn_igemm_tune_import(const int* buf, int n_entries);
int ffn_igemm_tune_clear(void);
int ffn_igemm_tune_enable(int on);
int ffn_igemm_tune_stamp(void);
int ffn_igemm_num_configs(void);
int ffn_igemm_force_config(int cfg);
int ffn_igemm_kernel_name(int dtype, const ffn_igemm_desc* d, char* buf, int len);

#define FFN_ATT_MAXP 4
#define FFN_ATT_MAXB 16
enum { FFN_ATT_HEAD_RULE = 1, FFN_ATT_UNIFORM_SEL1 = 2, FFN_ATT_UNIFORM_SEL0 = 4,
       FFN_ATT_CAUSAL = 8  };
typedef struct ffn_attn_entry {
    int q_row, kv_row;
    float w_const, w_slope;
    const float* wq;
    const uint8_t* kmask;
    const uint8_t* qsel;
    int flags;
    int hr_row;
} ffn_attn_entry;
typedef struct ffn_attn_desc {
    const void* q;
    const void* k;
    const void* vt;
    void* out;
    const float* w_dev;
    int Bo, S, Sk, heads, D;
    int ldq, ldk, ldvt, ldo;
    float scale;
    int npass;
    int out_pair;
    int kv_pair;
    ffn_attn_entry e[FFN_ATT_MAXP * FFN_ATT_MAXB];
} ffn_attn_desc;
int ffn_attn(void* stream, int dtype, const ffn_attn_desc* d);
int ffn_attn_presplit(void* stream, const float* k, const float* vt, void* k_pair, void* vt_pair, int rows, int Sk, int heads, int ldk, int ldvt);
int ffn_attn_variant(int dtype, int D, int* dp, int* qf);
int ffn_attn_kernel_name(int dtype, const ffn_attn_desc* d, char* buf, int len);

enum { FFN_ELT_RELU = 0, FFN_ELT_ADD = 1, FFN_ELT_GELU = 2 };
int ffn_eltwise(void* stream, int dtype, int op, const void* a, const void* b, void* y, long n);
int ffn_resize_bilinear(void* stream, int dtype, const void* x, void* y, int B, int Hin, int Win, int Hout, int Wout, int C, int relu);

typedef struct ffn_splat_xform {
    float center[3], translate[3], rotate[9] , scale[3];
    float tan_half_fov;
} ffn_splat_xform;
int ffn_splat_lift(void* stream, const float* depth, const int* idx, float* pts, int n, int W, int H, float fx, float fy);
int ffn_splat_project(void* stream, const float* pts, float* proj, int n, const ffn_splat_xform* x);
int ffn_splat_bin(void* stream, int fill, const float* proj, int n, float radius, int W, int H, int* counts, const int* offs, int* list);
int ffn_splat_render(void* stream, const float* proj, const float* rgb, const int* offs, const int* list, float radius, int K, int W, int H,
                     float* image, int* idx_sum, uint8_t* covered);
int ffn_splat_ids(void* stream, const float* proj, const int* offs, const int* list, float radius, int K, int W, int H, int* ids);
int ffn_splat_correspond(void* stream, const float* proj, const int* idx, int n, int W, int H, const int* ids, int K, float* map, uint8_t* visible);

int ffn_geo_project(void* stream, const float* depth, const float* pose, float focal, int H, int W, float* tcoords, float* proj);
int ffn_splat_composite(void* stream, const float* proj, const float* feat, const int* offs, const int* list, float radius, float tau, int K,
                        int C, int H, int W, int round_half, float* out);
int ffn_mesh_cover(void* stream, const float* tcoords, const uint8_t* mask, int H, int W, uint8_t* cover);

enum { FFN_NORM_SILU = 1, FFN_NORM_OUT_PAIR = 2 };
int ffn_gn_nchunk(int HW);
int ffn_gn_fused(int B, int HW, int C, int G);
int ffn_gn_stats(void* stream, int dtype, const void* x, const float* gamma, const float* beta, int B, int HW, int C, int G,
                 float eps, float* partial_ws, float* scale, float* shift);
int ffn_gn_apply(void* stream, int dtype, const void* x, void* y, const float* scale, const float* shift, int B, int HW,
                 int C, int silu);
int ffn_groupnorm(void* stream, int dtype, const void* x, void* y, const float* gamma, const float* beta, int B, int HW, int C, int G,
                  float eps, int silu, float* partial_ws, float* scale, float* shift);
int ffn_groupnorm_pair_raw(void* stream, const void* x, void* y_pair, void* yraw_pair, const float* gamma, const float* beta, int B, int HW, int C, int G,
                           float eps, int silu, float* partial_ws, float* scale, float* shift);
int ffn_layernorm(void* stream, int dtype, const void* x, void* y, const float* gamma, const float* beta, int M, int C,
                  float eps);
int ffn_layernorm_pair(void* stream, const float* x, void* y, const float* gamma, const float* beta, int M, int C, float eps);
int ffn_softmax_rows(void* stream, int dtype, const void* x, void* y, long M, int N, float scale);
int ffn_pool_layernorm(void* stream, int dtype, const void* x, const int* ids, void* y, const float* gamma, const float* beta, int N, int S, int C, float eps,
                       int pair);
int ffn_cosine_rows(void* stream, const float* a, const float* b, float* out, int B, int P, int b_rows);

int ffn_cfg_masked(void* stream, const float* eps_u, const float* eps_c, const float* mask, float cfg, float* eps, long n,
                   int HW);
int ffn_ddim_inv_step(void* stream, const float* eps, const float* x, float c_bt, float c_at, float c_an, float c_bn,
                      float* x_next, float* pred_x0, long n);
typedef struct ffn_ctrl_step_desc {
    const float* eps;
    const float* x;
    const float* noise;
    const float* m;
    const float* om;
    float* x_prev;
    float* pred_x0;
    float c_bt, c_at, c_ap, c_dir;
    float c_dirm[8], stdv[8];
    int row_masked[8];
    int rows, CHW, HW;
} ffn_ctrl_step_desc;
int ffn_ddim_ctrl_step(void* stream, const ffn_ctrl_step_desc* d);

typedef struct ffn_pack_desc {
    const float* src;
    void* dst;
    int src_row[16];
    int B, Cl, CP, HW;
} ffn_pack_desc;
int ffn_pack_nchw(void* stream, int dtype, const ffn_pack_desc* d);
int ffn_nhwc_to_nchw_f32(void* stream, const float* src, float* dst, int B, int HW, int C, int ld);
int ffn_concat(void* stream, int dtype, const void* a, const void* b, void* out, long rows, int C1, int C2);
int ffn_timestep_embed(void* stream, int dtype, const float* t_dev, const float* freq, void* out, int B, int half, int flip);
int ffn_transpose(void* stream, int dtype, const void* src, void* dst, int B, int R, int C, int ld_src, int ld_dst);
int ffn_cast(void* stream, int src_dtype, int dst_dtype, const void* src, void* dst, long n);
int ffn_embed_tokens(void* stream, int dtype, const int* ids, const float* table, const float* pos, void* out, long M, int S, int C, int V);
int ffn_embed_tokens_ln(void* stream, int dtype, const int* ids, const float* table, const float* pos, void* out, const float* gamma, const float* beta, long M,
                        int S, int C, int V, float eps);
#define FFN_CHAIN_MAXL 8
#define FFN_CHAIN_MAXW 1024
int ffn_affine_chain(void* stream, const float* x, const float* params, float* out, int B, int ldx, const int* dims, int L, float shift, float scale);
int ffn_image_to_nhwc(void* stream, int dtype, const uint8_t* img, void* dst, long npix, int CP);
int ffn_nhwc_to_image(void* stream, int dtype, const void* src, float* dst, int B, int HW, int ld);

typedef struct ffn_dift_desc {
    const void* src;
    const void* tgt;
    const int* kps;
    void* ws;
    int* out_rc;
    float* out_cos;
    long ws_bytes;
    long es;
    int dtype, E, C, ld, h, w, H, W, K;
} ffn_dift_desc;
int ffn_dift_match(void* stream, const ffn_dift_desc* d);
long ffn_dift_workspace_bytes(int C, int h, int w, int K);

#define FFN_SIFT_MAX_SIDE 16384
#define FFN_SIFT_MAX_TAPS 63
int ffn_sift_base(void* stream, const uint8_t* img, float* out, int H, int W, int C);
int ffn_gauss_blur_f32(void* stream, const float* src, float* dst, float* tmp, int H, int W, const float* taps, int T);
int ffn_decimate2_f32(void* stream, const float* src, float* dst, int H, int W);
int ffn_sift_extrema(void* stream, const float* gauss, float* dog, int h, int w, int* cand, int cap, int* counter, int* count);
int ffn_sift_refine_orient(void* stream, const float* dog, const float* gauss, int h, int w, int octave, const int* cand, int n, float* out);
int ffn_sift_describe(void* stream, const float* gauss, int h, int w, int octave, const float* kp, int n, uint8_t* desc, float* raw);
int ffn_knn2_u8(void* stream, const uint8_t* des1, int n1, const uint8_t* des2, int n2, int* idx, int* dist);

#define FFN_IMGPREP_MAX_SIDE 4096
int ffn_resize_pil_bilinear_u8(void* stream, const uint8_t* src, uint8_t* dst, uint8_t* scratch, int B, int H, int W, int oh, int ow, const int* hbounds,
                               const int* hcoef, int hksize, const int* vbounds, const int* vcoef, int vksize);
int ffn_vit_patch_rows(void* stream, int dtype, const uint8_t* src, const float* lut, void* out, int B, int H, int W, int patch, int ldo);
int ffn_vit_patch_rows_pair(void* stream, const uint8_t* src, const float* lut, void* out, int B, int H, int W, int patch, int K);

#define FFN_IMGPREP_MAX_TAPS (2 * 3 * FFN_IMGPREP_MAX_SIDE + 1)
enum { FFN_KEEP_NONE = 0, FFN_KEEP_SUM_LT128 = 1, FFN_KEEP_GT128 = 2 };
typedef struct {
    const uint8_t* src;
    uint8_t* dst;
// ... 62 lines not shown
```

Baseline: 2.022.

## Fuse GroupNorm statistics into the bf16x3 GEMM epilogue of producing convs

Adds a GNSTATS epilogue flag to the ping-pong bf16x3 implicit GEMM. Each tile writes per-column mean and M2 partials, which are reduced with DPP and bpermute, into a workspace. A new finalize kernel merges the tile partials into the GroupNorm scale and shift tables, so the following GroupNorm skips its separate statistics pass over the activation. The UNet marks the producers whose output feeds a GroupNorm. This removes one full read of each normalised activation, at the cost of extra epilogue work and register pressure, and it forbids split-K and the 128-wide tiles for those GEMMs.

Result: no change. 2.037, median of 4 (+0.8%).

```diff
diff --git a/freefine_amd/_lib.py b/freefine_amd/_lib.py
--- a/freefine_amd/_lib.py
+++ b/freefine_amd/_lib.py
@@ -7,6 +7,7 @@
 FFN_F32, FFN_BF16, FFN_BF16X3, FFN_FP8 = 0, 1, 2, 3
 IG_OUT_SILU, IG_OUT_F32, IG_GEGLU, IG_OUT_TRANSPOSED, IG_OUT_PAIR, IG_OUT_GELU, IG_OUT_RELU, IG_OUT_KV64 = 1, 2, 4, 8, 16, 32, 64, 128
 IG_OUT_QGELU = 256
+IG_OUT_GNSTATS = 512
 ELT_RELU, ELT_ADD, ELT_GELU = 0, 1, 2
 ATT_MAXP, ATT_MAXB = 4, 16
 ATT_HEAD_RULE, ATT_UNIFORM_SEL1, ATT_UNIFORM_SEL0, ATT_CAUSAL = 1, 2, 4, 8
@@ -32,6 +33,7 @@
         ("flags", C.c_int), ("alpha", C.c_float), ("conv", C.c_int),
         ("splitk", C.c_int), ("ws", C.c_void_p), ("ws_bytes", C.c_long),
         ("a_lo", C.c_int), ("x3", C.c_int), ("f8", C.c_int), ("kv64_from", C.c_int),
+        ("gn_ws", C.c_void_p), ("gn_ws_floats", C.c_long),
     ]
 
 
@@ -122,6 +124,7 @@
     "ffn_groupnorm_f8": (_i, [_vp, _vp, _vp, _vp, _vp, _i, _i, _i, _i, _i, _f, _i, _f, _vp, _vp, _vp]),
     "ffn_attn": (_i, [_vp, _i, C.POINTER(AttnDesc)]),
     "ffn_attn_kernel_name": (_i, [_i, C.POINTER(AttnDesc), C.c_char_p, _i]),
+    "ffn_igemm_gnstats_floats": (_l, [_i, C.POINTER(IgemmDesc), _i]),
     "ffn_igemm_tune": (_i, [_vp, _i, C.POINTER(IgemmDesc)]),
     "ffn_igemm_tune_entry_ints": (_i, []),
     "ffn_igemm_tune_export": (_i, [C.POINTER(C.c_int), _i]),
@@ -140,6 +143,8 @@
     "ffn_gn_apply": (_i, [_vp, _i, _vp, _vp, _vp, _vp, _i, _i, _i, _i]),
     "ffn_groupnorm": (_i, [_vp, _i, _vp, _vp, _vp, _vp, _i, _i, _i, _i, _f, _i, _vp, _vp, _vp]),
     "ffn_groupnorm_pair_raw": (_i, [_vp, _vp, _vp, _vp, _vp, _vp, _i, _i, _i, _i, _f, _i, _vp, _vp, _vp]),
+    "ffn_gn_apply_pair_raw": (_i, [_vp, _vp, _vp, _vp, _vp, _vp, _i, _i, _i, _i]),
+    "ffn_gn_finalize_tiles": (_i, [_vp, _vp, _i, _vp, _i, _vp, _vp, _i, _i, _i, _f, _vp, _vp]),
     "ffn_layernorm": (_i, [_vp, _i, _vp, _vp, _vp, _vp, _i, _i, _f]),
     "ffn_layernorm_pair": (_i, [_vp, _vp, _vp, _vp, _vp, _i, _i, _f]),
     "ffn_softmax_rows": (_i, [_vp, _i, _vp, _vp, _l, _i, _f]),
diff --git a/freefine_amd/csrc/capi.hip b/freefine_amd/csrc/capi.hip
--- a/freefine_amd/csrc/capi.hip
+++ b/freefine_amd/csrc/capi.hip
@@ -8,7 +8,7 @@
 
 __thread char g_err[512] = "";
 
-extern "C" int ffn_version(void) { return 16; }
+extern "C" int ffn_version(void) { return 17; }
 extern "C" const char* ffn_last_error(void) { return g_err; }
 extern "C" int ffn_device_info(int device, char* name, int name_len) {
     hipDeviceProp_t prop;
@@ -142,6 +142,11 @@
     REQUIRE(y != yraw && yraw != x && y != x, "groupnorm_pair_raw: x, y and yraw must be distinct buffers");
     int rc = ffn_gn_stats(stream, FFN_F32, x, gamma, beta, B, HW, C, G, eps, partial_ws, scale, shift);
     if (rc) return rc;
+    return ffn_gn_apply_pair_raw(stream, x, y, yraw, scale, shift, B, HW, C, silu);
+}
+extern "C" int ffn_gn_apply_pair_raw(void* stream, const void* x, void* y, void* yraw, const float* scale, const float* shift, int B, int HW, int C, int silu) {
+    REQUIRE(x && y && yraw && scale && shift && C % 8 == 0 && aligned16(x) && aligned16(y) && aligned16(yraw), "gn_apply_pair_raw: bad arguments (C=%d)", C);
+    REQUIRE(y != yraw && yraw != x && y != x, "gn_apply_pair_raw: x, y and yraw must be distinct buffers");
     hipStream_t s = reinterpret_cast<hipStream_t>(stream);
     const long n8 = (long)B * HW * (C / 8);
     if (silu & FFN_NORM_SILU) LAUNCH((gn_apply_pair8_kernel<true, true>), dim3(grid_for(n8)), dim3(256), 0, s, (const float*)x, (bf16*)y, scale, shift, n8, HW, C, (bf16*)yraw);
@@ -178,6 +183,14 @@
     if (int rc = check_launch("gn_partial")) return rc;
     LAUNCH(gn_finalize_kernel, dim3(G, B), dim3(64), 0, s, partial_ws, gamma, beta, scale, shift, HW, C, G, nchunk, ppc, eps);
     return check_launch("gn_stats");
+}
+extern "C" int ffn_gn_finalize_tiles(void* stream, const float* ws_a, int Ca, const float* ws_b, int Cb, const float* gamma, const float* beta, int B, int HW, int G,
+                                     float eps, float* scale, float* shift) {
+    REQUIRE(ws_a && gamma && beta && scale && shift && aligned16(ws_a), "gn_finalize_tiles: null pointer");
+    REQUIRE(B > 0 && HW >= 128 && G > 0 && Ca > 0 && Cb >= 0 && (Cb == 0) == (ws_b == nullptr) && (Ca + Cb) % G == 0 && (long)B * HW < (1l << 31),
+            "gn_finalize_tiles: bad shape (B=%d, HW=%d, Ca=%d, Cb=%d, G=%d; HW >= 128: the producer's rows_per_batch)", B, HW, Ca, Cb, G);
+    LAUNCH(gn_finalize_tiles_kernel, dim3(G, B), dim3(64), 0, reinterpret_cast<hipStream_t>(stream), ws_a, Ca, ws_b, Cb, gamma, beta, scale, shift, B, HW, G, eps);
+    return check_launch("gn_finalize_tiles");
 }
 extern "C" int ffn_gn_apply(void* stream, int dtype, const void* x, void* y, const float* scale, const float* shift, int B, int HW,
                             int C, int silu) {
diff --git a/freefine_amd/csrc/capi_igemm.hip b/freefine_amd/csrc/capi_igemm.hip
--- a/freefine_amd/csrc/capi_igemm.hip
+++ b/freefine_amd/csrc/capi_igemm.hip
@@ -8,7 +8,7 @@
 #include "igemm_p8.h"
 
 static bool can_split(const ffn_igemm_desc& d) {
-    return d.ws && d.splitk != 1 && !(d.flags & (FFN_IG_GEGLU | FFN_IG_OUT_TRANSPOSED | FFN_IG_OUT_KV64));
+    return d.ws && d.splitk != 1 && !(d.flags & (FFN_IG_GEGLU | FFN_IG_OUT_TRANSPOSED | FFN_IG_OUT_KV64 | FFN_IG_OUT_GNSTATS));
 }
 static void igemm_rule_for(int dtype, const ffn_igemm_desc& d, int* bm, int* bn, int* splitk) {
     const long t128 = (long)((d.M + 127) / 128) * ((d.N + 127) / 128);
@@ -50,7 +50,7 @@
 static bool pp_ok(const ffn_igemm_desc& d, int bm, int bn, int splitk = 1) {
     const long lim = (1l << 31) - 4096;
     const int nkt = d.x3 ? d.K / 96 : d.K / 64;
-    if (bn == 128 && (bm != 256 || !d.x3 || d.conv != 1 || splitk > 1 || d.N % 256 == 0 || d.N % 320 == 0 || (d.flags & (FFN_IG_GEGLU | FFN_IG_OUT_PAIR | FFN_IG_OUT_KV64 | FFN_IG_OUT_TRANSPOSED)))) return false;
+    if (bn == 128 && (bm != 256 || !d.x3 || d.conv != 1 || splitk > 1 || d.N % 256 == 0 || d.N % 320 == 0 || (d.flags & (FFN_IG_GEGLU | FFN_IG_OUT_PAIR | FFN_IG_OUT_KV64 | FFN_IG_OUT_TRANSPOSED | FFN_IG_OUT_GNSTATS)))) return false;
     if (d.x3) {
         if (d.x3 != 2 || d.K % 96 != 0 || d.a_lo != 32) return false;
     } else if (d.K % 64 != 0) return false;
@@ -60,12 +60,12 @@
         if (!can_split(d) || nkt % splitk != 0 || nkt / splitk < 2 || (long)splitk * d.M * d.N * 4 > d.ws_bytes || (long)splitk * d.M * d.N * 4 >= lim) return false;
     } else {
         const int act_ok = (!d.residual && !d.x3 && !d.f8 && !(d.flags & FFN_IG_GEGLU)) ? (FFN_IG_OUT_GELU | FFN_IG_OUT_RELU) : 0;
-        if ((d.alpha != 1.0f && !d.f8) || (d.flags & ~(FFN_IG_GEGLU | act_ok | (d.x3 ? (FFN_IG_OUT_F32 | FFN_IG_OUT_PAIR | FFN_IG_OUT_KV64) : 0)))) return false;
+        if ((d.alpha != 1.0f && !d.f8) || (d.flags & ~(FFN_IG_GEGLU | act_ok | (d.x3 ? (FFN_IG_OUT_F32 | FFN_IG_OUT_PAIR | FFN_IG_OUT_KV64 | FFN_IG_OUT_GNSTATS) : 0)))) return false;
         if (d.f8 && (!d.conv || (d.flags & FFN_IG_GEGLU))) return false;
         if (d.x3 && (d.flags & FFN_IG_GEGLU) && !(d.flags & FFN_IG_OUT_PAIR)) return false;
         if ((d.flags & FFN_IG_OUT_PAIR) && !(d.flags & FFN_IG_GEGLU) && (d.N % 32 != 0 || (d.ldo / 2) % 32 != 0 || (d.flags & FFN_IG_OUT_TRANSPOSED))) return false;
         if ((d.flags & FFN_IG_GEGLU) && bn != 256) return false;
-        if (d.rowbias && d.rows_per_batch < 128) return false;
+        if ((d.rowbias || (d.flags & FFN_IG_OUT_GNSTATS)) && d.rows_per_batch < 128) return false;
     }
     long a_bytes;
     if (d.conv) {
@@ -162,6 +162,12 @@
     if ((long)((d.M + d.rows_per_batch - 1) / d.rows_per_batch) * d.N * d.ldo * (d.x3 ? 4 : 2) >= lim) return false;
     return (*bm = pp_tile_height(d, *bn, {256, 192}, 0, true)) != 0;
 }
+static bool gnstats_tile(const ffn_igemm_desc& d, int* bm, int* bn, int min_fill4 = 0) {
+    if (!d.x3 || d.splitk > 1 || d.conv == 2) return false;
+    for (int n : {320, 256})
+        if ((*bm = pp_tile_height(d, n, {256, 192}, min_fill4))) { *bn = n; return true; }
+    return false;
+}
 static IgChoice rule_choice(int dtype, const ffn_igemm_desc& d) {
     int bm, bn, sk;
     igemm_rule_for(dtype, d, &bm, &bn, &sk);
@@ -175,6 +181,7 @@
 static IgChoice heuristic_choice(const ffn_igemm_desc& d) {
     int bm, bn;
     if (d.conv == 2 && conv2_tile(d, &bm, &bn)) return IgChoice{pp_cfg(bm, bn), 1};
+    if (d.flags & FFN_IG_OUT_GNSTATS) return IgChoice{gnstats_tile(d, &bm, &bn) ? pp_cfg(bm, bn) : -1, 1};
     if (d.splitk <= 1) {
         for (int n : {320, 256})
             if ((bm = pp_tile_height(d, n, {256, 192}, 3))) return IgChoice{pp_cfg(bm, n), 1};
@@ -228,7 +235,7 @@
     for (int cfg = 0; cfg < CFG_COUNT; ++cfg) {
         const IgCfgInfo& c = kCfg[cfg];
         if ((d.x3 || d.f8) && !x3_cfg(cfg)) continue;
-        if (d.conv == 2 && !is_pp_cfg(cfg)) continue;
+        if ((d.conv == 2 || (d.flags & FFN_IG_OUT_GNSTATS)) && !is_pp_cfg(cfg)) continue;
         if ((cfg == CFG_128x320 || cfg == CFG_128x160 || cfg == CFG_192x320) && (d.flags & FFN_IG_GEGLU)) continue;
         if (is_halo_cfg(cfg)) {
             const int hb = halo_bytes_for(d, c.bm);
@@ -315,6 +322,7 @@
     int bm, bn, amode, nwm, nwn;
     bool swap, fastk, x3, f8;
     bool res, geglu, split;
+    bool stats;
     int splitk, halo_bytes, lds;
     bool reduce_f32;
     dim3 grid, block;
@@ -370,6 +378,8 @@
         p->split = p->splitk > 1;
         p->res = !p->split && d.residual;
         p->geglu = !p->split && !d.conv && (d.flags & FFN_IG_GEGLU);
+        p->stats = d.flags & FFN_IG_OUT_GNSTATS;
+        REQUIRE(!p->stats || (p->x3 && !p->split && !p->geglu && p->bn != 128), "igemm: no statistics epilogue on this ping-pong tile");
         [[fallthrough]];
     case IG_PP_TRANS: {
         p->lds = 2 * (p->bm + p->bn) * 128 + 12288;
@@ -414,6 +424,19 @@
 template <int AMODE, bool X3 = false, bool F8 = false>
 static int launch_pp(const IgemmPlan& p, hipStream_t s, const ffn_igemm_desc& d) {
     const bool trans = p.kind == IG_PP_TRANS;
+    if constexpr (X3) {
+        if (p.stats) {
+#define FFN_PPS(BM_, BN_)                                                                                                          \
+    if (p.bm == BM_ && p.bn == BN_) return p.res ? igemm_launch(p, igemm_pp_gnstats_kernel<BM_, BN_, AMODE, true>, s, d, p.splitk) \
+                                                 : igemm_launch(p, igemm_pp_gnstats_kernel<BM_, BN_, AMODE, false>, s, d, p.splitk)
+            FFN_PPS(256, 320);
+            FFN_PPS(256, 256);
+            FFN_PPS(192, 320);
+            FFN_PPS(192, 256);
+#undef FFN_PPS
+            return fail(FFN_EINVAL, "igemm: no %d x %d ping-pong tile with the statistics epilogue", p.bm, p.bn);
+        }
+    }
 #define FFN_PP(BM_, BN_, RES_, GEGLU_, SPLIT_, TRANS_)                                                                       \
     if (p.bm == BM_ && p.bn == BN_ && p.res == RES_ && p.geglu == GEGLU_ && p.split == SPLIT_ && trans == TRANS_) \
         return igemm_launch(p, igemm_pp_kernel<BM_, BN_, AMODE, RES_, GEGLU_, SPLIT_, TRANS_, X3, F8>, s, d, p.splitk)
@@ -610,6 +633,15 @@
         else REQUIRE(d.kv64_from >= 0 && d.kv64_from < d.N && d.kv64_from % 64 == 0 && d.N % 64 == 0 && d.ldo % 4 == 0,
                      "igemm: KV64 output needs kv64_from and N %% 64 == 0 (kv64_from=%d, N=%d)", d.kv64_from, d.N);
     }
+    if (d.flags & FFN_IG_OUT_GNSTATS) {
+        REQUIRE(dtype == FFN_BF16X3 && d.x3 == 2 && d.splitk <= 1 && d.conv != 2 &&
+                    !(d.flags & (FFN_IG_GEGLU | FFN_IG_OUT_PAIR | FFN_IG_OUT_KV64 | FFN_IG_OUT_TRANSPOSED | FFN_IG_OUT_SILU | FFN_IG_OUT_GELU | FFN_IG_OUT_RELU | FFN_IG_OUT_QGELU)),
+                "igemm: FFN_IG_OUT_GNSTATS needs FFN_BF16X3 with blocked operands, a plain / row-bias / residual epilogue and no forced split-K");
+        REQUIRE(d.rows_per_batch >= 128, "igemm: GNSTATS needs rows_per_batch >= 128, the rows of a wave (rows_per_batch=%d): at most two images meet there", d.rows_per_batch);
+        const long need = ffn_igemm_gnstats_floats(dtype, &d, 1);
+        REQUIRE(need > 0, "igemm: GNSTATS: no unsplit ping-pong tile takes M=%d N=%d K=%d", d.M, d.N, d.K);
+        REQUIRE(d.gn_ws && aligned16(d.gn_ws) && d.gn_ws_floats >= need && d.gn_ws_floats * 4 < (1l << 31), "igemm: GNSTATS workspace of %ld floats, %ld needed (16-byte aligned)", d.gn_ws_floats, need);
+    }
     if (d.flags & FFN_IG_OUT_TRANSPOSED) {
         REQUIRE(!d.conv, "igemm: transposed output is only supported for dense A");
         REQUIRE(d.ldo % 4 == 0, "igemm: transposed ldo=%d must be a multiple of 4", d.ldo);
@@ -643,6 +675,14 @@
     }
     if (d.residual) REQUIRE(d.ldr >= d.N, "igemm: ldr=%d must be >= N=%d", d.ldr, d.N);
     return FFN_OK;
+}
+extern "C" long ffn_igemm_gnstats_floats(int dtype, const ffn_igemm_desc* d0, int any_size) {
+    if (!d0 || dtype != FFN_BF16X3 || d0->x3 != 2 || d0->M <= 0 || d0->N <= 0 || d0->rows_per_batch < 128) return 0;
+    ffn_igemm_desc d = igemm_view(dtype, *d0);
+    d.flags |= FFN_IG_OUT_GNSTATS;
+    int bm, bn;
+    if (!gnstats_tile(d, &bm, &bn, any_size ? 0 : 3)) return 0;
+    return 4 + 16l * d.N * ((d.M + 191) / 192);
 }
 static bool tuned_family(int dtype, const ffn_igemm_desc& d) { return dtype != FFN_F32 && !(d.flags & FFN_IG_OUT_TRANSPOSED); }
 extern "C" int ffn_igemm_kernel_name(int dtype, const ffn_igemm_desc* d0, char* buf, int len) {
@@ -663,6 +703,10 @@
     case IG_HALO: snprintf(buf, len, "void igemm_halo_kernel<bf16, %d, %d, %d, %d>(ffn_igemm_desc, int)", p.bm, p.bn, p.nwm, p.nwn); break;
     case IG_PP:
     case IG_PP_TRANS:
+        if (p.stats) {
+            snprintf(buf, len, "void igemm_pp_gnstats_kernel<%d, %d, %d, %s>(ffn_igemm_desc, int)", p.bm, p.bn, p.amode, b(p.res));
+            break;
+        }
         snprintf(buf, len, "void igemm_pp_kernel<%d, %d, %d, %s, %s, %s, %s, %s, %s>(ffn_igemm_desc, int)", p.bm, p.bn, p.amode, b(p.res), b(p.geglu), b(p.split),
                  b(p.kind == IG_PP_TRANS), b(p.x3), b(p.f8));
         break;
diff --git a/freefine_amd/csrc/igemm_p8.h b/freefine_amd/csrc/igemm_p8.h
--- a/freefine_amd/csrc/igemm_p8.h
+++ b/freefine_amd/csrc/igemm_p8.h
@@ -17,6 +17,13 @@
 __device__ __forceinline__ void pp_wait_vmcnt() {
     if (PP_ABL != 2) asm volatile("s_waitcnt vmcnt(%0)" ::"n"(N) : "memory");
 }
+__device__ __forceinline__ float dpp_rowsum16(float v) {
+    v += __builtin_bit_cast(float, __builtin_amdgcn_update_dpp(0, __builtin_bit_cast(int, v), 0xB1, 0xF, 0xF, true));
+    v += __builtin_bit_cast(float, __builtin_amdgcn_update_dpp(0, __builtin_bit_cast(int, v), 0x4E, 0xF, 0xF, true));
+    v += __builtin_bit_cast(float, __builtin_amdgcn_update_dpp(0, __builtin_bit_cast(int, v), 0x141, 0xF, 0xF, true));
+    v += __builtin_bit_cast(float, __builtin_amdgcn_update_dpp(0, __builtin_bit_cast(int, v), 0x140, 0xF, 0xF, true));
+    return v;
+}
 __device__ __forceinline__ void pp_barrier() {
     asm volatile("" ::: "memory");
     __builtin_amdgcn_s_barrier();
@@ -26,8 +33,8 @@
 #ifdef PP_TRACE
 __device__ unsigned long long pp_trace[256 * 64];
 #endif
-template <int BM, int BN, int AMODE, bool RES, bool GEGLU, bool SPLIT = false, bool TRANS = false, bool X3 = false, bool F8 = false>
-__global__ __launch_bounds__(512) void igemm_pp_kernel(const IgemmParams p, int splitk = 1) {
+template <int BM, int BN, int AMODE, bool RES, bool GEGLU, bool SPLIT, bool TRANS, bool X3, bool F8, bool STATS>
+__device__ __forceinline__ void igemm_pp_body(const IgemmParams& p, int splitk) {
     typedef bf16 T;
     constexpr int HM = BM / 2;
     constexpr int FM = HM / 16;
@@ -385,6 +392,45 @@
         }
         if constexpr (X3) {
             const int voff = (pr * p.ldo + 4 * pg) * 4;
+            if constexpr (STATS) {
+                {
+                    const int sl = ln & 15, sg = ln >> 4;
+                    const int E = (m0 / p.rows_per_batch + 1) * p.rows_per_batch - m0;
+                    const int r0 = i0 * 16, r1 = min(r0 + FH * 16, p.M - m0);
+                    const int q = (m0 + r0) / (FH * 16);
+                    const __amdgpu_buffer_rsrc_t rsrcGn = __builtin_amdgcn_make_buffer_rsrc(p.gn_ws, 0, (int)(p.gn_ws_floats * 4), 0x00020000);
+                    if (q == 0 && wc == 0)
+                        __builtin_amdgcn_raw_buffer_store_b128(__builtin_bit_cast(u32x4, f32x4{(float)(FH * 16), 0.f, 0.f, 0.f}), rsrcGn, ln == 0 ? 0 : OOB, 0, 0);
+#pragma unroll 1
+                    for (int slot = 0; slot < 2; ++slot) {
+                        const int lo = slot ? max(E, r0) : r0, hi = slot ? r1 : min(E, r1);
+                        if (hi <= lo) continue;
+                        const float inv_n = 1.0f / (float)(hi - lo);
+                        const int rl = r0 + sl - lo, rn = hi - lo;
+                        const int gvo = sl < 2 ? (sl * p.N + 4 * sg) * 4 : OOB;
+#pragma unroll
+                        for (int j = 0; j < FN; ++j) {
+                            f32x4 pv, sm = f32x4{0.f, 0.f, 0.f, 0.f}, m2 = f32x4{0.f, 0.f, 0.f, 0.f};
+#pragma unroll
+                            for (int r = 0; r < 4; ++r) pv[r] = __builtin_bit_cast(float, __builtin_amdgcn_ds_bpermute((ln & 48) * 4, __builtin_bit_cast(int, acc[i0][j][r])));
+#pragma unroll
+                            for (int i = 0; i < FH; ++i) sm += (acc[i0 + i][j] - pv) * ((unsigned)(rl + 16 * i) < (unsigned)rn ? 1.f : 0.f);
+#pragma unroll
+                            for (int r = 0; r < 4; ++r) sm[r] = dpp_rowsum16(sm[r]) * inv_n;
+#pragma unroll
+                            for (int i = 0; i < FH; ++i) {
+                                const f32x4 dv = ((acc[i0 + i][j] - pv) - sm) * ((unsigned)(rl + 16 * i) < (unsigned)rn ? 1.f : 0.f);
+                                m2 += dv * dv;
+                            }
+#pragma unroll
+                            for (int r = 0; r < 4; ++r) m2[r] = dpp_rowsum16(m2[r]);
+                            const f32x4 v = (sl & 1) ? m2 : pv + sm;
+                            __builtin_amdgcn_raw_buffer_store_b128(__builtin_bit_cast(u32x4, v), rsrcGn, gvo, (4 + (2 * q + slot) * 2 * p.N + n0 + j * 16) * 4, 0);
+                        }
+                    }
+                    __builtin_amdgcn_sched_barrier(0);
+                }
+            }
 #pragma unroll
             for (int i = i0; i < i0 + FH; ++i) {
                 const int vo = m0 + i * 16 + pr < p.M ? voff : OOB;
@@ -785,3 +831,11 @@
     if (blockIdx.x == 7) pp_stamp_out[tid] = *reinterpret_cast<const unsigned long long*>(smem + CV + 12288 + tid * 8);
 #endif
 }
+template <int BM, int BN, int AMODE, bool RES, bool GEGLU, bool SPLIT = false, bool TRANS = false, bool X3 = false, bool F8 = false>
+__global__ __launch_bounds__(512) void igemm_pp_kernel(const IgemmParams p, int splitk = 1) {
+    igemm_pp_body<BM, BN, AMODE, RES, GEGLU, SPLIT, TRANS, X3, F8, false>(p, splitk);
+}
+template <int BM, int BN, int AMODE, bool RES>
+__global__ __launch_bounds__(512) void igemm_pp_gnstats_kernel(const IgemmParams p, int splitk = 1) {
+    igemm_pp_body<BM, BN, AMODE, RES, false, false, false, true, false, true>(p, splitk);
+}
diff --git a/freefine_amd/csrc/norms.h b/freefine_amd/csrc/norms.h
--- a/freefine_amd/csrc/norms.h
+++ b/freefine_amd/csrc/norms.h
@@ -108,6 +108,52 @@
     const double mean = s / n;
     const double m2 = fmax(sq - s * mean, 0.0);
     const float rstd = (float)(1.0 / sqrt(m2 / n + (double)eps));
+    for (int i = lane; i < cg; i += 64) {
+        const int c = g * cg + i;
+        const float sc = rstd * gamma[c];
+        scale[(long)b * C + c] = sc;
+        shift[(long)b * C + c] = (float)((double)beta[c] - mean * (double)sc);
+    }
+}
+
+struct GnMoments { double n, mean, m2; };
+__device__ __forceinline__ GnMoments gn_merge(const GnMoments a, const GnMoments b) {
+    if (b.n == 0.0) return a;
+    if (a.n == 0.0) return b;
+    const double n = a.n + b.n, d = b.mean - a.mean;
+    return GnMoments{n, a.mean + d * (b.n / n), a.m2 + b.m2 + d * d * (a.n * b.n / n)};
+}
+__global__ __launch_bounds__(64) void gn_finalize_tiles_kernel(const float* __restrict__ wa, int Ca, const float* __restrict__ wb, int Cb, const float* __restrict__ gamma,
+                                                               const float* __restrict__ beta, float* __restrict__ scale, float* __restrict__ shift, int B, int HW, int G,
+                                                               float eps) {
+    const int g = blockIdx.x, b = blockIdx.y, lane = threadIdx.x;
+    const int C = Ca + Cb, cg = C / G, M = B * HW;
+    const int lo_b = b * HW, hi_b = lo_b + HW;
+    GnMoments acc{0.0, 0.0, 0.0};
+    for (int ci = 0; ci < cg; ++ci) {
+        const int c = g * cg + ci;
+        const bool second = c >= Ca;
+        const float* ws = second ? wb : wa;
+        const int N = second ? Cb : Ca, cc = second ? c - Ca : c;
+        const int R = (int)ws[0];
+        if (R != 48 && R != 64) {
+            acc = GnMoments{1.0, __builtin_nan(""), 0.0};
+            break;
+        }
+        for (int q = lo_b / R + lane; q * R < hi_b; q += 64) {
+            const int slot = b - ((q >> 1) * 2 * R) / HW;
+            const int lo = max(q * R, lo_b), hi = min(min((q + 1) * R, hi_b), M);
+            if (hi <= lo) continue;
+            const float* src = ws + 4 + (long)(2 * q + slot) * 2 * N + cc;
+            acc = gn_merge(acc, GnMoments{(double)(hi - lo), (double)src[0], (double)src[N]});
+        }
+    }
+    for (int off = 32; off > 0; off >>= 1) {
+        const GnMoments o{__shfl_down(acc.n, off), __shfl_down(acc.mean, off), __shfl_down(acc.m2, off)};
+        acc = gn_merge(acc, o);
+    }
+    const double mean = __shfl(acc.mean, 0), var = __shfl(acc.m2, 0) / __shfl(acc.n, 0);
+    const float rstd = (float)(1.0 / sqrt(var + (double)eps));
     for (int i = lane; i < cg; i += 64) {
         const int c = g * cg + i;
         const float sc = rstd * gamma[c];
diff --git a/freefine_amd/ops.py b/freefine_amd/ops.py
--- a/freefine_amd/ops.py
+++ b/freefine_amd/ops.py
@@ -289,6 +289,46 @@
         ws = _WS[key] = torch.empty(WS_BYTES // 4, dtype=torch.float32, device=device)
     return ws
 
+GN_EPILOGUE = os.environ.get("FFN_GN_EPILOGUE", "0") == "1"
+GN_EPILOGUE_ANY_SIZE = False
+
+
+def _gnstats_request(lib, dcode, d, want, device):
+    if not (want and GN_EPILOGUE) or _invariant():
+        return None
+    n = lib.ffn_igemm_gnstats_floats(dcode, CT.byref(d), 1 if GN_EPILOGUE_ANY_SIZE else 0)
+    if n <= 0:
+        return None
+    ws = torch.empty(n, dtype=torch.float32, device=device)
+    d.flags |= L.IG_OUT_GNSTATS
+    d.gn_ws, d.gn_ws_floats = ws.data_ptr(), n
+    return ws
+
+
+def _gnstats_attach(out, ws, d):
+    if ws is not None:
+        out._ffn_gnstats = (ws, out.data_ptr(), d.M, d.N, d.rows_per_batch)
+    elif hasattr(out, "_ffn_gnstats"):
+        del out._ffn_gnstats
+
+
+def gn_stats_of(x):
+    st = getattr(x, "_ffn_gnstats", None)
+    if st is None or not GN_EPILOGUE or x.ndim != 3 or not x.is_contiguous() or x.dtype != torch.float32:
+        return None
+    ws, ptr, M, N, rpb = st
+    B, HW, Cc = x.shape
+    return ws if (ptr, M, N, rpb) == (x.data_ptr(), B * HW, Cc, HW) else None
+
+
+def _gn_tables_from_tiles(lib, x, st, gamma, beta, G, eps, ws):
+    B, HW, Cc = x.shape
+    scale, shift = ws[1:] if ws is not None else (torch.empty(B, Cc, dtype=torch.float32, device=x.device), torch.empty(B, Cc, dtype=torch.float32, device=x.device))
+    call = lambda: lib.ffn_gn_finalize_tiles(_stream(), st.data_ptr(), Cc, 0, 0, gamma.data_ptr(), beta.data_ptr(), B, HW, G, eps, scale.data_ptr(), shift.data_ptr())
+    L.check(call() if _PROF is None else _timed("gn_finalize_tiles_kernel", 0.0, 4.0 * st.numel(), call), "ffn_gn_finalize_tiles")
+    return scale, shift
+
+
 _TLS = threading.local()
 
 
@@ -306,7 +346,7 @@
 
 
 def linear(x, w, bias=None, *, K=None, out=None, residual=None, rowbias=None, rows_per_batch=None, silu=False,
-           geglu=False, out_f32=False, transposed_ld=None, alpha=1.0, splitk=0, out_pair=False, gelu=False, relu=False, kv64_from=None, qgelu=False):
+           geglu=False, out_f32=False, transposed_ld=None, alpha=1.0, splitk=0, out_pair=False, gelu=False, relu=False, kv64_from=None, qgelu=False, gn_stats=False):
     lib = L.load()
     K = K if K is not None else x.shape[-1]
     M = x.numel() // x.shape[-1]
@@ -372,17 +412,19 @@
     if splitk == 0 and _invariant():
         splitk = 1
     d.splitk, d.ws, d.ws_bytes = splitk, _workspace(x.device).data_ptr(), WS_BYTES
+    gws = _gnstats_request(lib, dcode, d, gn_stats, x.device)
     if _PROF is None:
         L.check(lib.ffn_igemm(_stream(), dcode, CT.byref(d)), "ffn_igemm")
     else:
         esz = x.element_size()
         L.check(_timed(_igemm_name(lib, dcode, d), 2.0 * M * N * K, esz * (M * K + N * K + M * n_out),
                        lambda: lib.ffn_igemm(_stream(), dcode, CT.byref(d))), "ffn_igemm")
+    _gnstats_attach(out, gws, d)
     return out
 
 
 def conv3x3(x, w, bias, B, Hin, Win, Cin, *, stride=1, pad=1, upsample=False, out=None, residual=None, rowbias=None,
-            rowbias_ld=None, out_f32=False, Hout=None, Wout=None, splitk=0, relu=False):
+            rowbias_ld=None, out_f32=False, Hout=None, Wout=None, splitk=0, relu=False, gn_stats=False):
     lib = L.load()
     He, We = (Hin * 2, Win * 2) if upsample else (Hin, Win)
     if Hout is None:
@@ -423,6 +465,7 @@
     if splitk == 0 and _invariant():
         splitk = 1
     d.splitk, d.ws, d.ws_bytes = splitk, _workspace(x.device).data_ptr(), WS_BYTES
+    gws = _gnstats_request(lib, dcode, d, gn_stats, x.device)
     if _PROF is None:
         L.check(lib.ffn_igemm(_stream(), dcode, CT.byref(d)), "ffn_igemm(conv)")
     else:
@@ -430,6 +473,7 @@
         k_real = 9 * getattr(x, "_ffn_f8_act", Cin)
         L.check(_timed(_igemm_name(lib, dcode, d), 2.0 * d.M * N * k_real, esz * (x.numel() + N * d.K + d.M * N),
                        lambda: lib.ffn_igemm(_stream(), dcode, CT.byref(d))), "ffn_igemm(conv)")
+    _gnstats_attach(out, gws, d)
     return out
 
 
@@ -593,6 +637,13 @@
         out = _mark_pair(torch.empty(B, HW, 2 * Cc, dtype=torch.bfloat16, device=x.device), Cc)
     if out is None:
         out = torch.empty_like(x)
+    st = None if _invariant() else gn_stats_of(x)
+    if st is not None:
+        scale, shift = _gn_tables_from_tiles(lib, x, st, gamma, beta, G, eps, ws)
+        fl = (L.NORM_SILU if silu else 0) | (L.NORM_OUT_PAIR if pair else 0)
+        call = lambda: lib.ffn_gn_apply(_stream(), _dt(x), x.data_ptr(), out.data_ptr(), scale.data_ptr(), shift.data_ptr(), B, HW, Cc, fl)
+        L.check(call() if _PROF is None else _timed(f"gn_apply<{_tname(x)}> (statistics from the producer)", 0.0, 2.0 * x.numel() * x.element_size(), call), "ffn_gn_apply")
+        return out
     nb = B
     if _invariant() and lib.ffn_gn_fused(1, HW, Cc, G) and not lib.ffn_gn_fused(B, HW, Cc, G):
         while not lib.ffn_gn_fused(nb, HW, Cc, G):
@@ -622,11 +673,17 @@
 def groupnorm_pair_raw(x, gamma, beta, G, eps, silu=False, ws=None):
     lib = L.load()
     B, HW, Cc = x.shape
-    if Cc % 8 != 0 or lib.ffn_gn_fused(1 if _invariant() else B, HW, Cc, G) or not x.is_contiguous():
+    st = None if _invariant() else gn_stats_of(x)
+    if Cc % 8 != 0 or Cc % G != 0 or (Cc // G) % 2 != 0 or (st is None and lib.ffn_gn_fused(1 if _invariant() else B, HW, Cc, G)) or not x.is_contiguous():
         return groupnorm(x, gamma, beta, G, eps, silu=silu, pair=True, ws=ws), split_pair(x, Cc)
     assert x.dtype == torch.float32
     y = _mark_pair(torch.empty(B, HW, 2 * Cc, dtype=torch.bfloat16, device=x.device), Cc)
     yr = _mark_pair(torch.empty(B, HW, 2 * Cc, dtype=torch.bfloat16, device=x.device), Cc)
+    if st is not None:
+        scale, shift = _gn_tables_from_tiles(lib, x, st, gamma, beta, G, eps, ws)
+        call = lambda: lib.ffn_gn_apply_pair_raw(_stream(), x.data_ptr(), y.data_ptr(), yr.data_ptr(), scale.data_ptr(), shift.data_ptr(), B, HW, Cc, L.NORM_SILU if silu else 0)
+        L.check(call() if _PROF is None else _timed("gn_apply<float> (+ raw pair; statistics from the producer)", 0.0, 3.0 * x.numel() * x.element_size(), call), "ffn_gn_apply_pair_raw")
+        return y, yr
     partial, scale, shift = ws if ws is not None else gn_workspace(B, HW, Cc, x.device)
     call = lambda: lib.ffn_groupnorm_pair_raw(_stream(), x.data_ptr(), y.data_ptr(), yr.data_ptr(), gamma.data_ptr(), beta.data_ptr(), B, HW, Cc, G, eps,
                                               L.NORM_SILU if silu else 0, _p(partial), _p(scale), _p(shift))
diff --git a/freefine_amd/unet.py b/freefine_amd/unet.py
--- a/freefine_amd/unet.py
+++ b/freefine_amd/unet.py
@@ -515,18 +515,18 @@
             return ops.groupnorm_f8(x, gb[0], gb[1], self.cfg.norm_num_groups, self.cfg.norm_eps, w._ffn_f8[0], silu=True)
         return self._gn(x, gb, self.cfg.norm_eps, True)
 
-    def _resblock(self, r, x, B, H, W, temb_all, out=None):
+    def _resblock(self, r, x, B, H, W, temb_all, out=None, gn_next=False):
         cin = x.shape[-1]
         if r.sc is not None and self.x3 and not ops.is_f8(r.c1[0]) and ops.pair_width(x) is None and x.dtype == torch.float32:
             h, x = ops.groupnorm_pair_raw(x, r.n1[0], r.n1[1], self.cfg.norm_num_groups, self.cfg.norm_eps, silu=True)
         else:
             h = self._gn_conv_in(x, r.n1, r.c1[0])
         rb = temb_all[:, r.temb_off:r.temb_off + r.cout]
-        h = ops.conv3x3(h, r.c1[0], r.c1[1], B, H, W, cin, rowbias=rb, rowbias_ld=temb_all.shape[1])
+        h = ops.conv3x3(h, r.c1[0], r.c1[1], B, H, W, cin, rowbias=rb, rowbias_ld=temb_all.shape[1], gn_stats=self.x3)
         h = self._gn_conv_in(h, r.n2, r.c2[0])
         if r.sc is not None:
             x = ops.linear(x, r.sc[0], r.sc[1], K=cin)
-        return ops.conv3x3(h, r.c2[0], r.c2[1], B, H, W, r.cout, residual=x, out=out)
+        return ops.conv3x3(h, r.c2[0], r.c2[1], B, H, W, r.cout, residual=x, out=out, gn_stats=self.x3 and gn_next)
 
     def _without_ref_queries(self, plan, B):
         keep = self._reuse["idx_a_list"]
@@ -580,7 +580,7 @@
             ru["static"] += [qk[B:, :, C:], vt[B:]]
         return qk, vt
 
-    def _transformer_block(self, t, x, B, H, W, place, kv_text, out=None, drop=None, tb=0):
+    def _transformer_block(self, t, x, B, H, W, place, kv_text, out=None, drop=None, tb=0, gn_next=False):
         S, C = H * W, t.C
         res0 = x
         ru = self._reuse
@@ -618,7 +618,7 @@
         y = ops.layernorm(h, *t.ln[2], pair=self.x3)
         y = ops.linear(y, t.ff1[0], t.ff1[1], K=C, geglu=True, out_pair=self.x3)
         h = ops.linear(y, t.ff2[0], t.ff2[1], K=4 * C, residual=h, out_pair=self.x3 and C % 32 == 0)
-        return ops.linear(h, t.proj_out[0], t.proj_out[1], K=C, residual=res0, out=out)
+        return ops.linear(h, t.proj_out[0], t.proj_out[1], K=C, residual=res0, out=out, rows_per_batch=S if self.x3 and gn_next else None, gn_stats=self.x3 and gn_next)
 
     def _run(self, sample, text_kv, stop_up=None):
         cfg = self.cfg
@@ -650,23 +650,24 @@
         temb_full = temb_all
         temb_all = temb_all[:B]
         x = ops.pack_nchw(sample, list(range(B)), self.cin_pad, dt)
-        x = ops.conv3x3(x, self.conv_in[0], self.conv_in[1], B, H, W, self.cin_pad)
+        x = ops.conv3x3(x, self.conv_in[0], self.conv_in[1], B, H, W, self.cin_pad, gn_stats=self.x3)
         skips = [(x, H, W)]
         n = len(self.down)
         for i, blk in enumerate(self.down):
             for j, r in enumerate(blk.res):
-                x = self._resblock(r, x, B, H, W, temb_all)
+                to_norm1 = j + 1 < len(blk.res) or blk.down is None
+                x = self._resblock(r, x, B, H, W, temb_all, gn_next=bool(blk.attn) or to_norm1)
                 if blk.attn:
-                    x = self._transformer_block(blk.attn[j], x, B, H, W, "down", next(ti), tb=tb)
+                    x = self._transformer_block(blk.attn[j], x, B, H, W, "down", next(ti), tb=tb, gn_next=to_norm1)
                     tb += 1
                 skips.append((x, H, W))
             if blk.down is not None:
                 C = x.shape[-1]
-                x = ops.conv3x3(x, blk.down[0], blk.down[1], B, H, W, C, stride=2)
+                x = ops.conv3x3(x, blk.down[0], blk.down[1], B, H, W, C, stride=2, gn_stats=self.x3)
                 H, W = (H + 1) // 2, (W + 1) // 2
                 skips.append((x, H, W))
-        x = self._resblock(self.mid.res[0], x, B, H, W, temb_all)
-        x = self._transformer_block(self.mid.attn[0], x, B, H, W, "mid", next(ti), tb=tb)
+        x = self._resblock(self.mid.res[0], x, B, H, W, temb_all, gn_next=True)
+        x = self._transformer_block(self.mid.attn[0], x, B, H, W, "mid", next(ti), tb=tb, gn_next=True)
         tb += 1
         def cat_dst(C1, HW):
             return ops.cat_dst((B, HW), C1, skips[-1][0].shape[-1], dt, x.device) if skips else None
@@ -688,11 +689,12 @@
                 assert (sh, sw) == (H, W)
                 x = ops.concat(x, s)
                 dst = cat_dst(r.cout, H * W) if j + 1 < len(blk.res) else None
-                x = self._resblock(r, x, B, H, W, temb_all, out=None if blk.attn else dst)
+                closes = i == len(self.up) - 1 and j == len(blk.res) - 1 and blk.up is None and stop_up is None
+                x = self._resblock(r, x, B, H, W, temb_all, out=None if blk.attn else dst, gn_next=bool(blk.attn) or closes)
                 if blk.attn:
                     last = replay and bool(ru.get("drop_tail")) and blk.attn[j] is self.transformers[-1]
                     drop = (ru["idx_a"], ru["text_kv_a"][-1]) if last else None
-                    x = self._transformer_block(blk.attn[j], x, B, H, W, "up", next(ti), out=dst, drop=drop, tb=tb)
+                    x = self._transformer_block(blk.attn[j], x, B, H, W, "up", next(ti), out=dst, drop=drop, tb=tb, gn_next=closes)
                     tb += 1
                     if last:
                         assert dst is None and i == len(self.up) - 1 and j == len(blk.res) - 1, "the last transformer block closes the network"
diff --git a/include/freefine_hip.h b/include/freefine_hip.h
--- a/include/freefine_hip.h
+++ b/include/freefine_hip.h
@@ -23,7 +23,8 @@
     FFN_IG_OUT_GELU = 1 << 5,
     FFN_IG_OUT_KV64 = 1 << 7,
     FFN_IG_OUT_RELU = 1 << 6,
-    FFN_IG_OUT_QGELU = 1 << 8
+    FFN_IG_OUT_QGELU = 1 << 8,
+    FFN_IG_OUT_GNSTATS = 1 << 9
 };
 typedef struct ffn_igemm_desc {
     const void* A;
@@ -46,8 +47,11 @@
     int x3;
     int f8;
     int kv64_from;
+    float* gn_ws;
+    long gn_ws_floats;
 } ffn_igemm_desc;
 int ffn_igemm(void* stream, int dtype, const ffn_igemm_desc* d);
+long ffn_igemm_gnstats_floats(int dtype, const ffn_igemm_desc* d, int any_size);
 int ffn_split_pair(void* stream, const float* src, void* dst, long rows, int C, int ld_src);
 int ffn_conv3x3_n4(void* stream, int dtype, const void* x, const float* w, const float* bias, float* out, int B, int H, int W, int Cin);
 int ffn_groupnorm_f8(void* stream, const void* x_bf16, void* y_e4m3, const float* gamma, const float* beta, int B, int HW, int C, int Cp,
@@ -127,6 +131,9 @@
                   float eps, int silu, float* partial_ws, float* scale, float* shift);
 int ffn_groupnorm_pair_raw(void* stream, const void* x, void* y_pair, void* yraw_pair, const float* gamma, const float* beta, int B, int HW, int C, int G,
                            float eps, int silu, float* partial_ws, float* scale, float* shift);
+int ffn_gn_apply_pair_raw(void* stream, const void* x, void* y_pair, void* yraw_pair, const float* scale, const float* shift, int B, int HW, int C, int silu);
+int ffn_gn_finalize_tiles(void* stream, const float* ws_a, int Ca, const float* ws_b, int Cb, const float* gamma, const float* beta, int B, int HW, int G, float eps,
+                          float* scale, float* shift);
 int ffn_layernorm(void* stream, int dtype, const void* x, void* y, const float* gamma, const float* beta, int M, int C,
                   float eps);
 int ffn_layernorm_pair(void* stream, const float* x, void* y, const float* gamma, const float* beta, int M, int C, float eps);
```
